# Critical-Infrastructure-Systems-Lab/ldsr

Hardware: NVIDIA B200
Metric: EM fits/sec (T~400, restarts x CV folds) (higher is better)
Workload: dtype f64

## Files before the change

### ldsr_b200/csrc/em_split_kernel.cuh

```cuda
#pragma once
#include "em_kernel.cuh"

namespace ldsr {

constexpr int SPLIT_NCH = 10;

template <int PQ> __host__ __device__ constexpr int split_nstat() { return 11 + 3 * PQ; }

__host__ __device__ constexpr bool split_w_in_smem(int pq) { return pq <= 4; }
__host__ __device__ inline size_t split_smem_bytes(int pq, int nw, int max_units, int max_uunits) {
    size_t b = 0;
    b += (size_t)max_units * 3 * 32 * 8;
    b += (size_t)2 * nw * 4 * 32 * 8;
    const bool pair = nw % 2 == 0 && nw * (11 + 3 * pq) > 2 * nw * SPLIT_NCH;
    const size_t ch = (size_t)2 * nw * SPLIT_NCH * 32 * 8, st = (size_t)(pair ? nw / 2 : nw) * (11 + 3 * pq) * 32 * 8;
    b += ch > st ? ch : st;
    b += ((size_t)max_units * 4 + 15) & ~size_t(15);
    b += 128;
    b += (size_t)8 * 32 * 8;
    if (split_w_in_smem(pq)) b += (size_t)max_uunits * pq * 32 * 8;
    if (theta_bd_in_smem(pq)) b += (size_t)2 * pq * 32 * 8;
    return b;
}

constexpr int UNIT_M = 1 << 30, UNIT_M1 = 1 << 29, UNIT_US = 1 << 28, UNIT_T0 = UNIT_US - 1;

template <class F> __host__ __device__ inline void split_window_units(int t0, int T, int mseg, int uw, F f) {
    const int end = T < t0 + uw ? T : t0 + uw;
    int t = t0;
    while (t < end) {
        if (t + mseg <= T - 1 && t + mseg <= end) {
            f(t, false);
            t += mseg;
        } else {
            f(t, true);
            t += 1;
        }
    }
}

inline int split_units_upper_bound(const double *y, int T, int mseg, int uw) {
    int n = 0;
    for (int t0 = 0; t0 < T; t0 += uw) {
        bool any = false;
        for (int t = t0; t < T && t < t0 + uw; t++) any = any || (y[t] == y[t]);
        const bool inside = t0 + uw <= T - 1;
        if (!any && inside)
            n += 1;
        else
            split_window_units(t0, T, mseg, uw, [&](int, bool) { n++; });
    }
    return n;
}

template <int N> __device__ __forceinline__ void load_vec(const double *__restrict__ p, double (&dst)[N]) {
    if constexpr (N % 2 == 0) {
        const double2 *__restrict__ p2 = reinterpret_cast<const double2 *>(p);
#pragma unroll
        for (int i = 0; i < N / 2; i++) {
            const double2 t = p2[i];
            dst[2 * i] = t.x;
            dst[2 * i + 1] = t.y;
        }
    } else {
#pragma unroll
        for (int i = 0; i < N; i++) dst[i] = p[i];
    }
}

__device__ __forceinline__ void rescale4(double &a, double &b, double &c, double &d) {
    const int e = ((__double2hiint(a + b + c + d) >> 20) & 0x7ff) - 1023;
    const double sc = __hiloint2double((1023 - e) << 20, 0);
    a *= sc;
    b *= sc;
    c *= sc;
    d *= sc;
}

template <int PQ, int UW> struct SplitConst {
    static_assert(UW == 16 || UW == 32, "U unit is 16 or 32 steps");
    double A, A2, Q;
    double A8, A16;
    double aVW, bVW;
    MixedConst<PQ> mc;
    __device__ __forceinline__ double AW() const { return UW == 32 ? A16 * A16 : A16; }
    __device__ __forceinline__ void set(const Theta<PQ> &th) {
        A = th.A;
        A2 = A * A;
        Q = th.Q;
        const double A4 = A2 * A2;
        A8 = A4 * A4;
        A16 = A8 * A8;
        const double aw = AW();
        aVW = aw * aw;
        const double sv = ((1.0 + A2) * (1.0 + A4)) * (1.0 + A8);
        double s = sv * (1.0 + A16);
        if (UW == 32) s *= 1.0 + A16 * A16;
        bVW = Q * s;
        mc.set(th, A2);
    }
};

template <int PQ, int UW, int N>
__device__ __forceinline__ void compose_var_unit(const Theta<PQ> &th, const SplitConst<PQ, UW> &k, unsigned bits,
                                                 double &m11, double &m12, double &m21, double &m22) {
#pragma unroll
    for (int j = 0; j < N; j++) {
        const bool obs = (bits >> j) & 1u;
        const double s11 = obs ? k.mc.a11 : k.A2, s12 = obs ? k.mc.a12 : k.Q;
        const double s21 = obs ? k.mc.C2 : 0.0, s22 = obs ? th.R : 1.0;
        const double n11 = fma(s11, m11, s12 * m21), n12 = fma(s11, m12, s12 * m22);
        const double n21 = fma(s21, m11, s22 * m21), n22 = fma(s21, m12, s22 * m22);
        m11 = n11;
        m12 = n12;
        m21 = n21;
        m22 = n22;
    }
    rescale4(m11, m12, m21, m22);
}

template <int N> struct UnitGains {
    double K[N], rS[N], alpha[N], J[N], L[N];
    double Vnext;
    double dend;
};
template <int PQ, int UW, int N>
__device__ __forceinline__ void unit_gains(const Theta<PQ> &th, const SplitConst<PQ, UW> &k, unsigned bits, double Vq,
                                           UnitGains<N> &G) {
    double nj[N], dj[N], nn[N], dd[N];
    double n = Vq, d = 1.0;
#pragma unroll
    for (int j = 0; j < N; j++) {
        const bool obs = (bits >> j) & 1u;
        const double m11 = obs ? k.mc.a11 : k.A2, m12 = obs ? k.mc.a12 : k.Q;
        const double m21 = obs ? k.mc.C2 : 0.0, m22 = obs ? th.R : 1.0;
        nj[j] = n;
        dj[j] = d;
        nn[j] = fma(m11, n, m12 * d);
        dd[j] = fma(m21, n, m22 * d);
        n = nn[j];
        d = dd[j];
    }
    double rho[N], rn[N];
#pragma unroll
    for (int j = 0; j < N; j++) {
        rho[j] = fast_rcp(dd[j]);
        rn[j] = fast_rcp(nn[j]);
    }
#pragma unroll
    for (int j = 0; j < N; j++) {
        const bool obs = (bits >> j) & 1u;
        const double K = obs ? th.C * nj[j] * rho[j] : 0.0;
        const double nu = obs ? th.R * nj[j] : nj[j];
        const double vu = nu * rho[j];
        const double J = k.A * nu * rn[j];
        G.K[j] = K;
        G.rS[j] = obs ? dj[j] * rho[j] : 0.0;
        G.alpha[j] = fma(-k.mc.AC, K, k.A);
        G.J[j] = J;
        G.L[j] = vu * fma(-k.A, J, 1.0);
    }
    G.Vnext = nn[N - 1] * rho[N - 1];
    G.dend = d;
}

template <int PQ, int N>
__device__ __forceinline__ void unit_inputs(const Theta<PQ> &th, unsigned bits, const double *__restrict__ yseg,
                                            const double *__restrict__ useg, const double *__restrict__ vseg,
                                            double (&Bu)[N], double (&ymd)[N], double (&yo)[N],
                                            double (&ur)[N * PQ], double (&vr)[N * PQ]) {
    double yr[N];
    load_vec<N * PQ>(useg, ur);
    load_vec<N * PQ>(vseg, vr);
    load_vec<N>(yseg, yr);
#pragma unroll
    for (int j = 0; j < N; j++) {
        double b = 0.0, dv = 0.0;
#pragma unroll
        for (int i = 0; i < PQ; i++) {
            b = fma(th.b(i), ur[j * PQ + i], b);
            dv = fma(th.d(i), vr[j * PQ + i], dv);
        }
        const bool obs = (bits >> j) & 1u;
        yo[j] = obs ? yr[j] : 0.0;
        Bu[j] = b;
        ymd[j] = yo[j] - dv;
    }
}

struct PieceFwd {
    double Vq, P, q;
    double l0, l1, l2;
    double dprod;
    int shift;
    double PJ, PJ2, G0, GG, Lc;
};

template <int PQ, int UW, int N>
__device__ __forceinline__ void forward_unit_basis(const Theta<PQ> &th, const SplitConst<PQ, UW> &k, unsigned bits,
                                                   const double *__restrict__ yseg, const double *__restrict__ useg,
                                                   const double *__restrict__ vseg, PieceFwd &c) {
    double Bu[N], ymd[N], yo[N];
    {
        double ur[N * PQ], vr[N * PQ];
        unit_inputs<PQ, N>(th, bits, yseg, useg, vseg, Bu, ymd, yo, ur, vr);
    }
    UnitGains<N> G;
    unit_gains<PQ, UW, N>(th, k, bits, c.Vq, G);
    double q[N + 1], P[N + 1];
    q[0] = c.q;
    P[0] = c.P;
#pragma unroll
    for (int j = 0; j < N; j++) {
        const double beta = fma(k.A * G.K[j], ymd[j], Bu[j]);
        q[j + 1] = fma(G.alpha[j], q[j], beta);
        P[j + 1] = G.alpha[j] * P[j];
    }
    double g0[N], gP[N];
#pragma unroll
    for (int j = 0; j < N; j++) {
        const double d0 = fma(-th.C, q[j], ymd[j]);
        const double w0 = G.rS[j] * d0;
        c.l0 = fma(w0, d0, c.l0);
        c.l1 = fma(w0, P[j], c.l1);
        c.l2 = fma(G.rS[j] * P[j], P[j], c.l2);
        const double xu0 = fma(G.K[j], d0, q[j]);
        const double xuP = P[j] * fma(-G.K[j], th.C, 1.0);
        g0[j] = fma(-G.J[j], q[j + 1], xu0);
        gP[j] = fma(-G.J[j], P[j + 1], xuP);
    }
    double pj = c.PJ, pj2 = c.PJ2;
#pragma unroll
    for (int j = 0; j < N; j++) {
        c.G0 = fma(pj, g0[j], c.G0);
        c.GG = fma(pj, gP[j], c.GG);
        c.Lc = fma(pj2, G.L[j], c.Lc);
        pj *= G.J[j];
        pj2 *= G.J[j] * G.J[j];
    }
    c.PJ = pj;
    c.PJ2 = pj2;
    c.q = q[N];
    c.P = P[N];
    c.Vq = G.Vnext;
    c.dprod *= G.dend;
    {
        const int e = ((__double2hiint(c.dprod) >> 20) & 0x7ff) - 1023;
        c.dprod *= __hiloint2double((1023 - e) << 20, 0);
        c.shift += e;
    }
}

template <int PQ, int UW>
__device__ __forceinline__ void forward_word_basis(const Theta<PQ> &th, const SplitConst<PQ, UW> &k,
                                                   const double *__restrict__ useg, double *__restrict__ wk,
                                                   PieceFwd &c) {
    constexpr bool KEEP_W = split_w_in_smem(PQ);
    const double A4 = k.A2 * k.A2;
    double hh = 0.0;
    double W[KEEP_W ? PQ : 1];
    if (KEEP_W) {
#pragma unroll
        for (int i = 0; i < PQ; i++) W[i] = 0.0;
    }
#pragma unroll 1
    for (int b = 0; b < UW / 8; b++) {
        double ur[8 * PQ];
        load_vec<8 * PQ>(useg + b * 8 * PQ, ur);
        if (KEEP_W) {
#pragma unroll
            for (int i = 0; i < PQ; i++) {
                double lo = ur[i], hi = ur[4 * PQ + i];
#pragma unroll
                for (int j = 1; j < 4; j++) {
                    lo = fma(k.A, lo, ur[j * PQ + i]);
                    hi = fma(k.A, hi, ur[(4 + j) * PQ + i]);
                }
                W[i] = fma(W[i], k.A8, fma(lo, A4, hi));
            }
        } else {
            double Bu[8];
#pragma unroll
            for (int j = 0; j < 8; j++) {
                double acc = 0.0;
#pragma unroll
                for (int i = 0; i < PQ; i++) acc = fma(th.b(i), ur[j * PQ + i], acc);
                Bu[j] = acc;
            }
            double lo = Bu[0], hi = Bu[4];
#pragma unroll
            for (int j = 1; j < 4; j++) {
                lo = fma(k.A, lo, Bu[j]);
                hi = fma(k.A, hi, Bu[4 + j]);
            }
            hh = fma(hh, k.A8, fma(lo, A4, hi));
        }
    }
    if (KEEP_W) {
#pragma unroll
        for (int i = 0; i < PQ; i++) {
            hh = fma(th.b(i), W[i], hh);
            wk[i * 32] = W[i];
        }
    }
    const double AW = k.AW();
    const double qn = fma(AW, c.q, hh);
    const double Pn = AW * c.P;
    const double Vn = fma(k.aVW, c.Vq, k.bVW);
    const double Jc = AW * c.Vq * fast_rcp(Vn);
    const double g0 = fma(-Jc, qn, c.q);
    const double gP = fma(-Jc, Pn, c.P);
    const double L = c.Vq * fma(-AW, Jc, 1.0);
    c.G0 = fma(c.PJ, g0, c.G0);
    c.GG = fma(c.PJ, gP, c.GG);
    c.Lc = fma(c.PJ2, L, c.Lc);
    c.PJ *= Jc;
    c.PJ2 *= Jc * Jc;
    c.q = qn;
    c.P = Pn;
    c.Vq = Vn;
}

template <int PQ, int UW, int N>
__device__ __forceinline__ void smooth_unit(const Theta<PQ> &th, const SplitConst<PQ, UW> &k, unsigned bits, bool last,
                                            const double *__restrict__ yseg, const double *__restrict__ useg,
                                            const double *__restrict__ vseg, double Xq, double Vq, double &Xs1,
                                            double &Vs1, Stats<PQ> &st) {
    constexpr bool KEEP_ROWS = N * PQ <= 16;
    double Bu[N], ymd[N], yo[N];
    double ur[N * PQ], vr[N * PQ];
    unit_inputs<PQ, N>(th, bits, yseg, useg, vseg, Bu, ymd, yo, ur, vr);
    UnitGains<N> G;
    unit_gains<PQ, UW, N>(th, k, bits, Vq, G);
    double xq[N + 1], g[N];
    xq[0] = Xq;
#pragma unroll
    for (int j = 0; j < N; j++) xq[j + 1] = fma(G.alpha[j], xq[j], fma(k.A * G.K[j], ymd[j], Bu[j]));
#pragma unroll
    for (int j = 0; j < N; j++) {
        const double delta = fma(-th.C, xq[j], ymd[j]);
        const double xu = fma(G.K[j], delta, xq[j]);
        g[j] = fma(-G.J[j], xq[j + 1], xu);
    }
    double Xs[N + 1], Vs[N + 1];
    Xs[N] = Xs1;
    Vs[N] = Vs1;
#pragma unroll
    for (int j = N - 1; j >= 0; j--) {
        Xs[j] = fma(G.J[j], Xs[j + 1], g[j]);
        Vs[j] = fma(G.J[j] * G.J[j], Vs[j + 1], G.L[j]);
    }
    if (!KEEP_ROWS) {
        load_vec<N * PQ>(useg, ur);
        load_vec<N * PQ>(vseg, vr);
    }
#pragma unroll
    for (int j = 0; j < N; j++) {
        if (N == 1 && last) {
            st.XT = Xs[j];
            st.VT = Vs[j];
        } else {
            st.Tx1x = fma(Xs[j + 1], Xs[j], st.Tx1x);
            st.Tx1xv = fma(Vs[j + 1], G.J[j], st.Tx1xv);
            st.Txx = fma(Xs[j], Xs[j], st.Txx);
            st.Txxv += Vs[j];
#pragma unroll
            for (int i = 0; i < PQ; i++) {
                st.Tx1u[i] = fma(Xs[j + 1], ur[j * PQ + i], st.Tx1u[i]);
                st.Tux[i] = fma(ur[j * PQ + i], Xs[j], st.Tux[i]);
            }
        }
        const bool obs = (bits >> j) & 1u;
        const double xo = obs ? Xs[j] : 0.0;
        st.Syx = fma(yo[j], xo, st.Syx);
        st.Sxx = fma(xo, xo, st.Sxx);
        st.Sxxv += obs ? Vs[j] : 0.0;
#pragma unroll
        for (int i = 0; i < PQ; i++) st.Sxv[i] = fma(xo, vr[j * PQ + i], st.Sxv[i]);
    }
    Xs1 = Xs[0];
    Vs1 = Vs[0];
}

template <int N> struct ShortConst {
    double AN, aV, bV;
    __device__ __forceinline__ ShortConst(double A, double A2, double Q) {
        double an = 1.0, av = 1.0, sv = 0.0;
#pragma unroll
        for (int j = 0; j < N; j++) {
            an *= A;
            sv = fma(sv, A2, 1.0);
            av *= A2;
        }
        AN = an;
        aV = av;
        bV = Q * sv;
    }
};
template <int PQ, int N>
__device__ __forceinline__ void forward_short_basis(const Theta<PQ> &th, double A, double A2, double Q,
                                                    const double *__restrict__ useg, PieceFwd &c) {
    const ShortConst<N> sc(A, A2, Q);
    double hh = 0.0;
#pragma unroll
    for (int j = 0; j < N; j++) {
        double bu = 0.0;
#pragma unroll
        for (int i = 0; i < PQ; i++) bu = fma(th.b(i), useg[j * PQ + i], bu);
        hh = fma(A, hh, bu);
    }
    const double qn = fma(sc.AN, c.q, hh), Pn = sc.AN * c.P, Vn = fma(sc.aV, c.Vq, sc.bV);
    const double Jc = sc.AN * c.Vq * fast_rcp(Vn);
    const double g0 = fma(-Jc, qn, c.q), gP = fma(-Jc, Pn, c.P), L = c.Vq * fma(-sc.AN, Jc, 1.0);
    c.G0 = fma(c.PJ, g0, c.G0);
    c.GG = fma(c.PJ, gP, c.GG);
    c.Lc = fma(c.PJ2, L, c.Lc);
    c.PJ *= Jc;
    c.PJ2 *= Jc * Jc;
    c.q = qn;
    c.P = Pn;
    c.Vq = Vn;
}
template <int PQ, int N>
__device__ __forceinline__ void smooth_short(const Theta<PQ> &th, double A, double A2, double Q,
                                             const double *__restrict__ useg, double Xq, double Vq, double &cG,
                                             double &cH, double &Xs1, double &Vs1, Stats<PQ> &st) {
    double Gs[N], Hs[N];
    Gs[N - 1] = Q * cG;
    Hs[N - 1] = cH;
#pragma unroll
    for (int j = N - 2; j >= 0; j--) {
        Gs[j] = A * Gs[j + 1];
        Hs[j] = A2 * Hs[j + 1];
    }
    const ShortConst<N> sc(A, A2, Q);
    const double G0 = sc.AN * cG, H0 = sc.aV * cH;
    double Xn[N + 1], vp[N + 1], Vn[N + 1];
    Xn[0] = fma(Vq, G0, Xq);
    vp[0] = Vq;
    Vn[0] = fma(Vq, Vq * H0, Vq);
    double tv = 0.0;
#pragma unroll
    for (int j = 0; j < N; j++) {
        double inp = Gs[j];
#pragma unroll
        for (int i = 0; i < PQ; i++) inp = fma(th.b(i), useg[j * PQ + i], inp);
        Xn[j + 1] = fma(A, Xn[j], inp);
        vp[j + 1] = fma(A2, vp[j], Q);
        const double t1 = vp[j + 1] * Hs[j];
        Vn[j + 1] = fma(vp[j + 1], t1, vp[j + 1]);
        st.Tx1x = fma(Xn[j + 1], Xn[j], st.Tx1x);
        st.Txx = fma(Xn[j], Xn[j], st.Txx);
        st.Txxv += Vn[j];
        tv = fma(vp[j], 1.0 + t1, tv);
#pragma unroll
        for (int i = 0; i < PQ; i++) {
            st.Tx1u[i] = fma(Xn[j + 1], useg[j * PQ + i], st.Tx1u[i]);
            st.Tux[i] = fma(useg[j * PQ + i], Xn[j], st.Tux[i]);
        }
    }
    st.Tx1xv = fma(A, tv, st.Tx1xv);
    Xs1 = Xn[0];
    Vs1 = Vn[0];
    cG = G0;
    cH = H0;
}

constexpr int SPLIT_NUV = 7;
template <int UW> __device__ __forceinline__ void uvar_constants(double a, double Q, double aW, double *o) {
    double sig = 0.0, b1 = 0.0, W = 0.0, Z = 0.0, pw = 1.0, pw_prev = 1.0;
#pragma unroll 4
    for (int s = 0; s < UW; s++) {
        const double sn = fma(a, sig, 1.0);
        b1 += sig;
        W = fma(a, W, sig * sig);
        Z = fma(a, Z, sig * sn);
        sig = sn;
        pw_prev = pw;
        pw *= a;
    }
    const double Q2 = Q * Q;
    o[0 * 32] = sig;
    o[1 * 32] = Q * b1;
    o[2 * 32] = aW * sig;
    o[3 * 32] = 2.0 * Q * aW * b1;
    o[4 * 32] = Q2 * (a * W);
    o[5 * 32] = Q * fma(pw_prev, b1 + sig, aW * b1);
    o[6 * 32] = Q2 * Z;
}

template <int PQ, int UW>
__device__ __forceinline__ void smooth_word(const Theta<PQ> &th, const SplitConst<PQ, UW> &k,
                                            const double *__restrict__ useg, const double *__restrict__ uv,
                                            const double *__restrict__ wk, const double *__restrict__ tuu_w,
                                            double Xq, double Vq, double &cG, double &cH, double &Xs1, double &Vs1,
                                            Stats<PQ> &st) {
    constexpr int NB = UW / 8;
    constexpr bool KEEP_W = split_w_in_smem(PQ);
    const double qg0 = k.Q * cG;
    const double g1 = k.A8 * qg0, g2 = k.A16 * qg0, g3 = k.A8 * g2;
    const double G0 = (NB == 4 ? k.A8 * k.A16 * k.A8 : k.A16) * cG;
    const double H0 = k.aVW * cH;
    const double Xfirst = fma(Vq, G0, Xq), Vfirst = fma(Vq, Vq * H0, Vq);
    {
        const double sumVp = fma(uv[0 * 32], Vq, uv[1 * 32]);
        const double qa = uv[2 * 32] * Vq;
        st.Txxv += fma(cH, fma(Vq, qa + uv[3 * 32], uv[4 * 32]), sumVp);
        st.Tx1xv = fma(k.A, fma(cH, fma(Vq, qa + uv[5 * 32], uv[6 * 32]), sumVp), st.Tx1xv);
    }
    double Xs = Xfirst;
    double tux[KEEP_W ? PQ : 1];
    if (KEEP_W) {
#pragma unroll
        for (int i = 0; i < PQ; i++) tux[i] = 0.0;
    }
#pragma unroll 1
    for (int b = 0; b < NB; b++) {
        const int r = NB - 1 - b;
        const double Gb = r == 0 ? qg0 : (r == 1 ? g1 : (r == 2 ? g2 : g3));
        const double *__restrict__ blk = useg + b * 8 * PQ;
        constexpr bool KEEP_U = PQ <= 4;
        double uk[8 * PQ];
        load_vec<8 * PQ>(blk, uk);
        double Gs[8];
        Gs[7] = Gb;
#pragma unroll
        for (int j = 6; j >= 0; j--) Gs[j] = k.A * Gs[j + 1];
        double inp[8];
#pragma unroll
        for (int j = 0; j < 8; j++) {
            double acc = Gs[j];
#pragma unroll
            for (int i = 0; i < PQ; i++) acc = fma(th.b(i), uk[j * PQ + i], acc);
            inp[j] = acc;
        }
        double Xn[9];
        Xn[0] = Xs;
#pragma unroll
        for (int j = 0; j < 8; j++) Xn[j + 1] = fma(k.A, Xn[j], inp[j]);
        if (!KEEP_U) load_vec<8 * PQ>(blk, uk);
#pragma unroll
        for (int j = 0; j < 8; j++) {
            st.Tx1x = fma(Xn[j + 1], Xn[j], st.Tx1x);
            st.Txx = fma(Xn[j], Xn[j], st.Txx);
#pragma unroll
            for (int i = 0; i < PQ; i++) {
                if (KEEP_W) {
                    tux[i] = fma(uk[j * PQ + i], Xn[j], tux[i]);
                } else {
                    st.Tx1u[i] = fma(Xn[j + 1], uk[j * PQ + i], st.Tx1u[i]);
                    st.Tux[i] = fma(uk[j * PQ + i], Xn[j], st.Tux[i]);
                }
            }
        }
        Xs = Xn[8];
    }
    if (KEEP_W) {
#pragma unroll
        for (int i = 0; i < PQ; i++) {
            double acc = fma(qg0, wk[i * 32], k.A * tux[i]);
#pragma unroll
            for (int j = 0; j < PQ; j++) acc = fma(th.b(j), tuu_w[j * PQ + i], acc);
            st.Tx1u[i] += acc;
            st.Tux[i] += tux[i];
        }
    }
    Xs1 = Xfirst;
    Vs1 = Vfirst;
    cG = G0;
    cH = H0;
}

template <int PQ> __device__ __forceinline__ void stats_store(const Stats<PQ> &st, double *o) {
    o[0 * 32] = st.Syx;
    o[1 * 32] = st.Sxx;
    o[2 * 32] = st.Sxxv;
    o[3 * 32] = st.Tx1x;
    o[4 * 32] = st.Tx1xv;
    o[5 * 32] = st.Txx;
    o[6 * 32] = st.Txxv;
    o[7 * 32] = st.X0;
    o[8 * 32] = st.V0;
    o[9 * 32] = st.XT;
    o[10 * 32] = st.VT;
#pragma unroll
    for (int i = 0; i < PQ; i++) {
        o[(11 + i) * 32] = st.Sxv[i];
        o[(11 + PQ + i) * 32] = st.Tx1u[i];
        o[(11 + 2 * PQ + i) * 32] = st.Tux[i];
    }
}
template <int PQ> __device__ __forceinline__ void stats_add(Stats<PQ> &st, const double *o) {
    st.Syx += o[0 * 32];
    st.Sxx += o[1 * 32];
    st.Sxxv += o[2 * 32];
    st.Tx1x += o[3 * 32];
    st.Tx1xv += o[4 * 32];
    st.Txx += o[5 * 32];
    st.Txxv += o[6 * 32];
    st.X0 += o[7 * 32];
    st.V0 += o[8 * 32];
    st.XT += o[9 * 32];
    st.VT += o[10 * 32];
#pragma unroll
    for (int i = 0; i < PQ; i++) {
        st.Sxv[i] += o[(11 + i) * 32];
        st.Tx1u[i] += o[(11 + PQ + i) * 32];
        st.Tux[i] += o[(11 + 2 * PQ + i) * 32];
    }
}
template <int PQ, int NW> __host__ __device__ constexpr bool split_pairwise() {
    return NW % 2 == 0 && NW * (11 + 3 * PQ) > 2 * NW * SPLIT_NCH;
}
template <int PQ, int NW> __host__ __device__ constexpr int split_st_slots() {
    return split_pairwise<PQ, NW>() ? NW / 2 : NW;
}

struct SplitParams {
    EmParams em;
    int max_units;
    int max_uunits;
    int blob_smem;
    int cost_u, cost_m;
    int *flags;
    int epoch;
    int *ctl;
    const int *order;
    int n_sm;
#ifdef LDSR_PHASE_CLOCKS
    long long *clk;
#endif
};
#ifdef LDSR_PHASE_CLOCKS
#define LDSR_PHASE_MARK(kk)                       \
    do {                                          \
        const long long c_ = clock64();           \
        pc[kk] += c_ - tprev;                     \
        tprev = c_;                               \
    } while (0)
#define LDSR_UNIT_BEGIN() const long long ub_ = clock64()
#define LDSR_UNIT_END(base, u0) pc[(base) + (((u0) & UNIT_M) ? 1 : ((u0) & UNIT_M1) ? 2 : ((u0) & UNIT_US) ? 3 : 0)] += clock64() - ub_
#else
#define LDSR_PHASE_MARK(kk) \
    do {                    \
    } while (0)
#define LDSR_UNIT_BEGIN() \
    do {                  \
    } while (0)
#define LDSR_UNIT_END(base, u0) \
    do {                        \
    } while (0)
#endif

__device__ __forceinline__ int unit_cost(int u, int cost_u, int cost_m, int mseg) {
    if (u & UNIT_US) return cost_m / 5;
    return (u & UNIT_M) ? cost_m : ((u & UNIT_M1) ? (3 * cost_m) / (2 * mseg) : cost_u);
}
template <int NW>
__device__ inline void split_range(const int *units, int a, int b, int cost_u, int cost_m, int mseg, int *bounds) {
    long long total = 0;
    for (int i = a; i < b; ++i) total += unit_cost(units[i], cost_u, cost_m, mseg);
    bounds[0] = a;
    long long acc = 0;
    int kq = a;
    for (int w = 1; w < NW; ++w) {
        const long long target = (total * w + NW / 2) / NW;
        while (kq < b) {
            const int cu = unit_cost(units[kq], cost_u, cost_m, mseg);
            if (acc + cu / 2 >= target) break;
            acc += cu;
            kq++;
        }
        bounds[w] = kq;
    }
    bounds[NW] = b;
}

template <int PQ, int NW, int MINB, int MSEG, int UW>
__global__ void __launch_bounds__(NW * 32, MINB) em_split_kernel(const SplitParams SP) {
    static_assert(MSEG == 4 || MSEG == 8, "M unit is 4 or 8 steps");
    const EmParams &P = SP.em;
    LDSR_DYN_SMEM(smem_raw);
    LDSR_STATIC_SMEM(__align__(8) uint64_t, bar);
    constexpr int NST = split_nstat<PQ>();
    constexpr int NP = 2 * NW;
    constexpr bool PAIR = split_pairwise<PQ, NW>();
    constexpr int ST_SLOTS = split_st_slots<PQ, NW>();
    constexpr size_t CH_DOUBLES = (size_t)NP * SPLIT_NCH * 32, ST_DOUBLES = (size_t)ST_SLOTS * NST * 32;

    const int lane = threadIdx.x & 31, warp = threadIdx.x >> 5;
    if (threadIdx.x == 0) {
        mbar_init(&bar, 1);
        fence_mbar_init();
    }
    __syncthreads();
    const int n_tasks = *P.n_tasks;
    unsigned phase = 0;
    int w_lo = 0;
    const auto slot_len = [&]() -> int {
        const int W = n_tasks * P.chunk, M = (W + (int)gridDim.x - 1) / (int)gridDim.x;
        return M < P.chunk ? P.chunk : M;
    };
    if (SP.flags) w_lo = (int)blockIdx.x * slot_len();
    const bool ranked = SP.ctl != nullptr && n_tasks <= (int)gridDim.x;
    LDSR_STATIC_SMEM(int, s_ti);
    LDSR_STATIC_SMEM(int, s_more);
    LDSR_STATIC_SMEM(int, s_on_sm);
    for (int seg = 0;; ++seg, phase ^= 1u) {
    int ti, n_it = P.chunk;
    bool wait_first = false;
    if (ranked) {
        if (seg > 0) break;
        if (threadIdx.x == 0) {
            const unsigned sm = sm_id(2);
            if (sm >= (unsigned)SHARE_MAX_SMID) share_trap();
            const int local = atomicAdd(SP.ctl + SHARE_CTL_SLOT + sm, 1);
            int r;
            if (local == 0) {
                r = atomicAdd(SP.ctl + SHARE_CTL_SMS, 1);
                flag_raise(SP.ctl + SHARE_CTL_RANK + sm, r + 1);
            } else {
                while ((r = ld_acquire(SP.ctl + SHARE_CTL_RANK + sm)) == 0) {
                }
                r -= 1;
            }
            if (local >= 2 || r >= SP.n_sm) share_trap();
            const int x = n_tasks > SP.n_sm ? n_tasks - SP.n_sm : 0;
            int qi = -1;
            if (local < 2 && r < SP.n_sm) qi = r < x ? 2 * r + local : (local == 0 ? x + r : -1);
            s_ti = (qi >= 0 && qi < n_tasks) ? SP.order[qi] : -1;
            s_on_sm = r < x ? 2 : 1;
            s_more = 1;
        }
        __syncthreads();
        ti = s_ti;
        if (ti < 0) break;
    } else if (SP.flags) {
        const int W = n_tasks * P.chunk, hi = ((int)blockIdx.x + 1) * slot_len(), w_hi = hi < W ? hi : W;
        if (w_lo >= w_hi) break;
        ti = w_lo / P.chunk;
        const int t_end = (ti + 1) * P.chunk, end = t_end < w_hi ? t_end : w_hi;
        n_it = end - w_lo;
        wait_first = w_lo == ti * P.chunk && end < t_end;
    } else {
        ti = (int)blockIdx.x + seg * (int)gridDim.x;
        if (ti >= n_tasks) break;
    }
    LDSR_CHECK(ti >= 0 && ti < n_tasks && n_it >= 1 && n_it <= P.chunk);
    if (seg > 0) __syncthreads();
    if (wait_first) {
        if (threadIdx.x == 0) flag_wait(SP.flags + ti, SP.epoch);
        __syncthreads();
    }
    const int4 task = P.tasks[ti];
    const SeriesDev S = P.series[task.x];
    const int T = S.T;
    if (threadIdx.x == 0) stage_blob(smem_raw, P.blobs + S.blob_off, (unsigned)S.blob_doubles * 8u, &bar);

    const double *__restrict__ ser = reinterpret_cast<const double *>(smem_raw);
    const double *__restrict__ ys = ser + S.y_off;
    const double *__restrict__ us = ser + S.u_off;
    const double *__restrict__ vs = ser + S.v_off;
    double *const ck = reinterpret_cast<double *>(smem_raw + SP.blob_smem) + lane;
    double *const MC = ck + (size_t)SP.max_units * 96;
    double *const CH = MC + (size_t)NP * 4 * 32;
    double *const ST = CH;
    int *const units =
        reinterpret_cast<int *>(CH - lane + (CH_DOUBLES > ST_DOUBLES ? CH_DOUBLES : ST_DOUBLES));
    int *const pbound = units + ((SP.max_units + 3) & ~3);
    double *const UV = reinterpret_cast<double *>(pbound + 32) + lane;
    double *const WK = UV + 8 * 32;
    double *const TB = WK + (split_w_in_smem(PQ) ? (size_t)SP.max_uunits * PQ * 32 : 0);
    double *const TD = TB + PQ * 32;
    constexpr bool BD_SMEM = theta_bd_in_smem(PQ);

    const bool valid = lane < task.z;
    const int fit = P.active[task.y + (valid ? lane : 0)];
    const int grp = P.f_group[fit];
    const unsigned *__restrict__ mw = P.masks + P.g_mask_off[grp];
    const double *__restrict__ gc = P.gconst + (size_t)grp * gconst_stride(PQ);
    const double *__restrict__ tuu_inv = P.sconst + S.sconst_off;
    const double n_obs = gc[1], inv_n_obs = 1.0 / n_obs;
    constexpr int TL = theta_pad_len<PQ>();
    Theta<PQ> th;
    {
        double g[TL];
#pragma unroll
        for (int i = 0; i < TL; i++) g[i] = ld_l2(P.theta + (size_t)fit * TL + i);
        load_theta<PQ>(th, g);
    }
    th.sb = TB;
    th.sd = TD;
    if (BD_SMEM && warp == 0) {
#pragma unroll
        for (int i = 0; i < PQ; i++) {
            TB[i * 32] = th.B[i];
            TD[i * 32] = th.D[i];
        }
    }
    double l1 = ld_l2(P.l1 + fit), l2 = ld_l2(P.l2 + fit), lik = ld_l2(P.lik + fit);
    int ne = ld_l2(P.ne + fit);
    bool live = valid && (ld_l2(P.done + fit) == 0);
    if (live && P.g_status[grp] != 0) {
        live = false;
        lik = __longlong_as_double(0x7ff8000000000000ULL);
    }

    if (warp == 0) {
        mbar_wait(&bar, phase);
        auto any_finite = [&](int t0, int n) -> bool {
            const int t = t0 + lane;
            const double yt = (lane < n && t < T) ? ys[t] : __longlong_as_double(0x7ff8000000000000ULL);
            return __any_sync(FULL, yt == yt);
        };
        int nu = 0;
        for (int t0 = 0; t0 < T; t0 += UW) {
            const bool any = any_finite(t0, UW);
            const bool inside = t0 + UW <= T - 1;
            if (!any && inside) {
                if (lane == 0) units[nu] = t0;
                nu++;
            } else {
                split_window_units(t0, T, MSEG, UW, [&](int t, bool single) {
                    int type = single ? UNIT_M1 : UNIT_M;
#ifndef LDSR_NO_US
                    if (!single && !any_finite(t, MSEG)) type = UNIT_US;
#endif
                    if (lane == 0) units[nu] = t | type;
                    nu++;
                });
            }
        }
        __syncwarp();
        if (lane == 0) {
            int nM = 0;
            for (int i = 0; i < nu; ++i) nM += (units[i] & (UNIT_M | UNIT_M1)) ? 1 : 0;
            int best = nu / 2, best_mis = 1 << 30, mb = 0;
            for (int s = 0; s <= nu; ++s) {
                const int ub = s - mb, ma = nM - mb, uaft = (nu - s) - ma;
                int mis = min(mb + uaft, ub + ma);
                if (s == 0 || s == nu) mis = 1 << 29;
                if (mis < best_mis || (mis == best_mis && abs(2 * s - nu) < abs(2 * best - nu))) {
                    best_mis = mis;
                    best = s;
                }
                if (s < nu && (units[s] & (UNIT_M | UNIT_M1))) mb++;
            }
            split_range<NW>(units, 0, best, SP.cost_u, SP.cost_m, MSEG, pbound);
            split_range<NW>(units, best, nu, SP.cost_u, SP.cost_m, MSEG, pbound + NW);
            LDSR_CHECK(nu <= SP.max_units && (T + UW - 1) / UW <= SP.max_uunits);
            for (int w = 0; w < 2 * NW; ++w) LDSR_CHECK(pbound[w] >= 0 && pbound[w] <= pbound[w + 1] && pbound[w + 1] <= nu);
        }
    }
    mbar_wait(&bar, phase);
    __syncthreads();

#ifdef LDSR_PHASE_CLOCKS
    long long pc[21] = {0, 0, 0, 0, 0, 0, 0, 0, 0, 0, 0, 0, 0, 0, 0, 0, 0, 0, 0, 0, 0}, tprev = clock64();
#endif
    bool counted = false;
    for (int it = 0;; ++it) {
        if (it >= n_it) {
            if (!ranked) break;
            if (!counted) {
                if (threadIdx.x == 0) {
                    atomicAdd(SP.ctl + SHARE_CTL_FINISHED, 1);
                    if (atomicAdd(SP.ctl + SHARE_CTL_DONE + sm_id(2), 1) + 1 < s_on_sm) s_more = 0;
                }
                counted = true;
                __syncthreads();
            }
            if (!s_more) break;
        }
        if (!__any_sync(FULL, live)) break;
        SplitConst<PQ, UW> k;
        k.set(th);

        if (warp == NW - 1) uvar_constants<UW>(k.A2, k.Q, k.aVW, UV);
        LDSR_PHASE_MARK(9);
#pragma unroll 1
        for (int h = 0; h < 2; ++h) {
            const int pj = h * NW + warp;
            if (pj == NP - 1) break;
            double m11 = 1.0, m12 = 0.0, m21 = 0.0, m22 = 1.0;
            const int ua = pbound[pj], ue = pbound[pj + 1];
            for (int un = ua; un < ue; ++un) {
                const int u0 = units[un];
                const int t0 = u0 & UNIT_T0;
                if (u0 & UNIT_M) {
                    compose_var_unit<PQ, UW, MSEG>(th, k, seg_bits(mw, t0, MSEG), m11, m12, m21, m22);
                } else if (u0 & UNIT_M1) {
                    compose_var_unit<PQ, UW, 1>(th, k, seg_bits(mw, t0, 1), m11, m12, m21, m22);
                } else if (u0 & UNIT_US) {
                    const ShortConst<MSEG> sc(k.A, k.A2, k.Q);
                    m11 = fma(sc.aV, m11, sc.bV * m21);
                    m12 = fma(sc.aV, m12, sc.bV * m22);
                } else {
                    m11 = fma(k.aVW, m11, k.bVW * m21);
                    m12 = fma(k.aVW, m12, k.bVW * m22);
                }
            }
            MC[(pj * 4 + 0) * 32] = m11;
            MC[(pj * 4 + 1) * 32] = m12;
            MC[(pj * 4 + 2) * 32] = m21;
            MC[(pj * 4 + 3) * 32] = m22;
        }
        LDSR_PHASE_MARK(0);
        __syncthreads();
        LDSR_PHASE_MARK(1);
        double VinA = th.V1, VinB = th.V1;
        {
            double n = th.V1, d = 1.0;
#pragma unroll
            for (int pj = 0; pj < NP - 1; ++pj) {
                const double m11 = MC[(pj * 4 + 0) * 32], m12 = MC[(pj * 4 + 1) * 32];
                const double m21 = MC[(pj * 4 + 2) * 32], m22 = MC[(pj * 4 + 3) * 32];
                const double nn = fma(m11, n, m12 * d), dd = fma(m21, n, m22 * d);
                n = nn;
                d = dd;
                if (pj + 1 == warp) VinA = n * fast_rcp(d);
                if (pj + 1 == NW + warp) VinB = n * fast_rcp(d);
            }
        }

        LDSR_PHASE_MARK(10);
#pragma unroll 1
        for (int h = 0; h < 2; ++h) {
            const int pj = h * NW + warp;
            const int ua = pbound[pj], ue = pbound[pj + 1];
            PieceFwd c;
            c.Vq = h ? VinB : VinA;
            c.P = 1.0;
            c.q = 0.0;
            c.l0 = c.l1 = c.l2 = 0.0;
            c.dprod = 1.0;
            c.shift = 0;
            c.PJ = c.PJ2 = 1.0;
            c.G0 = c.GG = c.Lc = 0.0;
            bool any_m = false;
            for (int un = ua; un < ue; ++un) {
                const int u0 = units[un];
                const int t0 = u0 & UNIT_T0;
                ck[(un * 3 + 0) * 32] = c.Vq;
                ck[(un * 3 + 1) * 32] = c.q;
                ck[(un * 3 + 2) * 32] = c.P;
                LDSR_UNIT_BEGIN();
                if (u0 & UNIT_M) {
                    any_m = true;
                    forward_unit_basis<PQ, UW, MSEG>(th, k, seg_bits(mw, t0, MSEG), ys + t0, us + t0 * PQ,
                                                     vs + t0 * PQ, c);
                } else if (u0 & UNIT_M1) {
                    any_m = true;
                    forward_unit_basis<PQ, UW, 1>(th, k, seg_bits(mw, t0, 1), ys + t0, us + t0 * PQ, vs + t0 * PQ, c);
                } else if (u0 & UNIT_US) {
                    forward_short_basis<PQ, MSEG>(th, k.A, k.A2, k.Q, us + t0 * PQ, c);
                } else {
                    forward_word_basis<PQ, UW>(th, k, us + t0 * PQ, WK + (size_t)(t0 / UW) * PQ * 32, c);
                }
                LDSR_UNIT_END(13, u0);
            }
            double ld = 0.0;
            if (any_m) ld = fma((double)c.shift, 0.693147180559945309417, log(c.dprod));
            double *o = CH + (size_t)pj * SPLIT_NCH * 32;
            o[0 * 32] = c.P;
            o[1 * 32] = c.q;
            o[2 * 32] = c.l0 + ld;
            o[3 * 32] = c.l1;
            o[4 * 32] = c.l2;
            o[5 * 32] = c.PJ;
            o[6 * 32] = c.G0;
            o[7 * 32] = c.GG;
            o[8 * 32] = c.Lc;
            o[9 * 32] = c.Vq;
        }
        LDSR_PHASE_MARK(2);
        __syncthreads();
        LDSR_PHASE_MARK(3);

        double gk[NP];
        double xinA = 0.0, xinB = 0.0;
        double XrA = 0.0, XrB = 0.0, VrA = 0.0, VrB = 0.0;
        double acc = 0.0;
        double x = th.mu1;
        double vend = th.V1;
        {
#pragma unroll
            for (int pj = 0; pj < NP; ++pj) {
                const double *o = CH + (size_t)pj * SPLIT_NCH * 32;
                if (pj == warp) xinA = x;
                if (pj == NW + warp) xinB = x;
                gk[pj] = fma(o[7 * 32], x, o[6 * 32]);
                const double tC = th.C * x;
                acc += fma(tC, fma(tC, o[4 * 32], -2.0 * o[3 * 32]), o[2 * 32]);
                x = fma(o[0 * 32], x, o[1 * 32]);
                vend = o[9 * 32];
                if (pj == warp) {
                    XrA = x;
                    VrA = vend;
                }
                if (pj == NW + warp) {
                    XrB = x;
                    VrB = vend;
                }
            }
        }
        const double lik_new = (-0.5 * n_obs * LOG_2PI - 0.5 * acc) * inv_n_obs;

        if (live) {
            lik = lik_new;
            ne += 1;
            if (warp == 0 && P.liks) P.liks[(size_t)P.f_user[fit] * P.niter + (ne - 1)] = lik_new;
            const bool conv = (ne >= 3) && (fabs(lik_new - l1) < P.tol) && (fabs(l1 - l2) < P.tol);
            if (conv || ne >= P.niter) live = false;
        }
        if (!__any_sync(FULL, live)) break;

        double Xs1A = 0.0, Vs1A = 0.0, Xs1B = 0.0, Vs1B = 0.0;
        {
            double Xs = x, Vs = vend;
#pragma unroll
            for (int pj = NP - 1; pj >= 0; --pj) {
                if (pj == NW + warp) {
                    Xs1B = Xs;
                    Vs1B = Vs;
                }
                if (pj == warp) {
                    Xs1A = Xs;
                    Vs1A = Vs;
                }
                const double *o = CH + (size_t)pj * SPLIT_NCH * 32;
                const double pjv = o[5 * 32];
                Xs = fma(pjv, Xs, gk[pj]);
                Vs = fma(pjv * pjv, Vs, o[8 * 32]);
            }
        }
        LDSR_PHASE_MARK(4);
        __syncthreads();
        LDSR_PHASE_MARK(5);

        Stats<PQ> st;
        st.zero();
#pragma unroll 1
        for (int h = 1; h >= 0; --h) {
            const int pj = h * NW + warp;
            const int ua = pbound[pj], ue = pbound[pj + 1];
            const double xin = h ? xinB : xinA;
            double Xs1 = h ? Xs1B : Xs1A, Vs1 = h ? Vs1B : Vs1A;
            double Xr = h ? XrB : XrA, Vr = h ? VrB : VrA;
            double cG = 0.0, cH = 0.0;
            bool in_run = false;
            for (int un = ue - 1; un >= ua; --un) {
                const int u0 = units[un];
                const int t0 = u0 & UNIT_T0;
                const double Vq = ck[(un * 3 + 0) * 32];
                const double Xq = fma(ck[(un * 3 + 2) * 32], xin, ck[(un * 3 + 1) * 32]);
                LDSR_UNIT_BEGIN();
                if (u0 & UNIT_M) {
                    smooth_unit<PQ, UW, MSEG>(th, k, seg_bits(mw, t0, MSEG), false, ys + t0, us + t0 * PQ,
                                              vs + t0 * PQ, Xq, Vq, Xs1, Vs1, st);
                    in_run = false;
                } else if (u0 & UNIT_M1) {
                    smooth_unit<PQ, UW, 1>(th, k, seg_bits(mw, t0, 1), t0 == T - 1, ys + t0, us + t0 * PQ,
                                           vs + t0 * PQ, Xq, Vq, Xs1, Vs1, st);
                    in_run = false;
                } else {
                    if (!in_run) {
                        const double rv = fast_rcp(Vr);
                        cG = (Xs1 - Xr) * rv;
                        cH = (Vs1 - Vr) * rv * rv;
                        in_run = true;
                    }
                    if (u0 & UNIT_US)
                        smooth_short<PQ, MSEG>(th, k.A, k.A2, k.Q, us + t0 * PQ, Xq, Vq, cG, cH, Xs1, Vs1, st);
                    else
                    smooth_word<PQ, UW>(th, k, us + t0 * PQ, UV, WK + (size_t)(t0 / UW) * PQ * 32,
                                        P.uwin + S.uwin_off + (size_t)(t0 / UW) * PQ * PQ, Xq, Vq, cG, cH, Xs1, Vs1, st);
                }
                LDSR_UNIT_END(17, u0);
                Xr = Xq;
                Vr = Vq;
            }
            if (ua == 0 && ue > 0) {
                st.X0 = Xs1;
                st.V0 = Vs1;
            }
        }
        LDSR_PHASE_MARK(6);
        if (ranked && it + 1 >= n_it && threadIdx.x == 0)
            s_more = ld_relaxed(SP.ctl + SHARE_CTL_FINISHED) + (counted ? 0 : 1) < n_tasks;
        if (!PAIR) {
            stats_store<PQ>(st, ST + (size_t)warp * NST * 32);
            __syncthreads();
            LDSR_PHASE_MARK(7);
            st.zero();
#pragma unroll
            for (int w = 0; w < NW; ++w) stats_add<PQ>(st, ST + (size_t)w * NST * 32);
        } else {
            if (warp >= NW / 2) stats_store<PQ>(st, ST + (size_t)(warp - NW / 2) * NST * 32);
            __syncthreads();
            if (warp < NW / 2) {
                stats_add<PQ>(st, ST + (size_t)warp * NST * 32);
                stats_store<PQ>(st, ST + (size_t)warp * NST * 32);
            }
            __syncthreads();
            if (warp == 0) {
                st.zero();
#pragma unroll
                for (int w = 0; w < NW / 2; ++w) stats_add<PQ>(st, ST + (size_t)w * NST * 32);
            }
        }
        LDSR_PHASE_MARK(11);
        if (!PAIR) {
            if (live) mstep_from_stats<PQ, true>(st, gc, tuu_inv, T, th);
        } else {
            double g[TL];
            if (warp == 0) {
                if (BD_SMEM) {
#pragma unroll
                    for (int i = 0; i < PQ; i++) {
                        th.B[i] = TB[i * 32];
                        th.D[i] = TD[i * 32];
                    }
                }
                if (live) mstep_from_stats<PQ, true>(st, gc, tuu_inv, T, th);
                if (BD_SMEM) {
#pragma unroll
                    for (int i = 0; i < PQ; i++) {
                        TB[i * 32] = th.B[i];
                        TD[i * 32] = th.D[i];
                    }
                }
                store_theta<PQ>(th, g);
#pragma unroll
                for (int i = 0; i < TL; i++) ST[i * 32] = g[i];
            }
            __syncthreads();
            if (warp != 0) {
#pragma unroll
                for (int i = 0; i < TL; i++) g[i] = ST[i * 32];
                load_theta<PQ>(th, g);
            }
        }
        if (live) {
            l2 = l1;
            l1 = lik;
        }
        LDSR_PHASE_MARK(8);
    }
#ifdef LDSR_PHASE_CLOCKS
    if (lane == 0 && SP.clk)
        for (int i = 0; i < 21; i++) SP.clk[((size_t)blockIdx.x * NW + warp) * 21 + i] = pc[i];
#endif

    if (ranked && !counted && threadIdx.x == 0) {
        atomicAdd(SP.ctl + SHARE_CTL_FINISHED, 1);
        atomicAdd(SP.ctl + SHARE_CTL_DONE + sm_id(2), 1);
    }
    if (BD_SMEM && warp == 0) {
#pragma unroll
        for (int i = 0; i < PQ; i++) {
            th.B[i] = TB[i * 32];
            th.D[i] = TD[i * 32];
        }
    }
    if (warp == 0 && valid) {
        store_theta<PQ>(th, P.theta + (size_t)fit * TL);
        P.l1[fit] = l1;
        P.l2[fit] = l2;
        P.lik[fit] = lik;
        P.ne[fit] = ne;
        P.done[fit] = live ? 0 : 1;
    }
    if (SP.flags) {
        if (w_lo % P.chunk != 0 && warp == 0) {
            __threadfence();
            __syncwarp();
            if (lane == 0) flag_raise(SP.flags + w_lo / P.chunk, SP.epoch);
        }
        w_lo += n_it;
    }
    }
}

}
```

### ldsr_b200/csrc/ldsr_abi.cu

```cuda
#include "../../include/ldsr_b200.h"
#include "generic_kernels.cuh"
#include "kernel_table.h"
#include "r_rng.cuh"
#include "scan_kernels.cuh"

#include <algorithm>
#include <atomic>
#include <chrono>
#include <condition_variable>
#include <cmath>
#include <cstdarg>
#include <cstdio>
#include <cstdlib>
#include <cstring>
#include <memory>
#include <mutex>
#include <numeric>
#include <string>
#include <thread>
#include <vector>

namespace ldsr {

#define LDSR_DECL(n) const KernelTable *kernel_table_pq##n() __attribute__((weak));
#define LDSR_PQ_LIST(X) X(1) X(2) X(3) X(4) X(5) X(6) X(7) X(8) X(10) X(12) X(16) X(24) X(32)
LDSR_PQ_LIST(LDSR_DECL)
const KernelTable *kernel_table_for(int need) {
#define LDSR_PICK(n) \
    if (need <= n && kernel_table_pq##n) return kernel_table_pq##n();
    LDSR_PQ_LIST(LDSR_PICK)
    return nullptr;
}

struct Err {
    int code = LDSR_OK;
    std::string msg;
    bool ok() const { return code == LDSR_OK; }
};
static Err fail(int code, const char *fmt, ...) {
    char buf[512];
    va_list ap;
    va_start(ap, fmt);
    vsnprintf(buf, sizeof buf, fmt, ap);
    va_end(ap);
    Err e;
    e.code = code;
    e.msg = buf;
    return e;
}
static int report(const Err &e, char *errbuf, int errlen) {
    if (errbuf && errlen > 0) snprintf(errbuf, errlen, "%s", e.msg.c_str());
    return e.code;
}
#define CU(call)                                                                                    \
    do {                                                                                            \
        cudaError_t _e = (call);                                                                    \
        if (_e != cudaSuccess) return fail(LDSR_ERR_CUDA, "%s: %s", #call, cudaGetErrorString(_e)); \
    } while (0)

class DevicePool {
  public:
    explicit DevicePool(int device) : device_(device) {}
    ~DevicePool() {
        cudaSetDevice(device_);
        for (auto &b : blocks_) cudaFree(b.ptr);
        for (auto &b : pinned_) cudaFreeHost(b.ptr);
        for (cudaStream_t s : streams_) cudaStreamDestroy(s);
    }
    cudaError_t alloc_pinned(size_t bytes, void **out) {
        bytes = std::max<size_t>((bytes + 255) & ~size_t(255), 256);
        std::lock_guard<std::mutex> lk(mu_);
        for (auto &b : pinned_)
            if (!b.used && b.size >= bytes) {
                b.used = true;
                *out = b.ptr;
                return cudaSuccess;
            }
        void *p = nullptr;
        cudaError_t e = cudaMallocHost(&p, bytes);
        if (e != cudaSuccess) return e;
        pinned_.push_back({p, bytes, true});
        *out = p;
        return cudaSuccess;
    }
    void release_pinned(void *p) {
        std::lock_guard<std::mutex> lk(mu_);
        for (auto &b : pinned_)
            if (b.ptr == p) b.used = false;
    }
    cudaError_t get_stream(cudaStream_t *out) {
        std::lock_guard<std::mutex> lk(mu_);
        if (!streams_.empty()) {
            *out = streams_.back();
            streams_.pop_back();
            return cudaSuccess;
        }
        return cudaStreamCreateWithFlags(out, cudaStreamNonBlocking);
    }
    void put_stream(cudaStream_t s) {
        std::lock_guard<std::mutex> lk(mu_);
        streams_.push_back(s);
    }
    cudaError_t alloc(size_t bytes, void **out) {
        bytes = std::max<size_t>((bytes + 255) & ~size_t(255), 256);
        std::lock_guard<std::mutex> lk(mu_);
        int best = -1;
        for (int i = 0; i < (int)blocks_.size(); i++)
            if (!blocks_[i].used && blocks_[i].size >= bytes && blocks_[i].size <= 2 * bytes + 4096 &&
                (best < 0 || blocks_[i].size < blocks_[best].size))
                best = i;
        if (best >= 0) {
            blocks_[best].used = true;
            *out = blocks_[best].ptr;
            return cudaSuccess;
        }
        void *p = nullptr;
        cudaError_t e = cudaMalloc(&p, bytes);
        if (e == cudaErrorMemoryAllocation) {
            cudaGetLastError();
            trim_locked();
            e = cudaMalloc(&p, bytes);
        }
        if (e != cudaSuccess) return e;
        blocks_.push_back({p, bytes, true});
        *out = p;
        return cudaSuccess;
    }
    void release(void *p) {
        std::lock_guard<std::mutex> lk(mu_);
        for (auto &b : blocks_)
            if (b.ptr == p) b.used = false;
    }
    size_t trim() {
        std::lock_guard<std::mutex> lk(mu_);
        return trim_locked();
    }
    size_t cached_bytes() {
        std::lock_guard<std::mutex> lk(mu_);
        size_t n = 0;
        for (auto &b : blocks_) n += b.size;
        return n;
    }
    int device() const { return device_; }

  private:
    struct Block {
        void *ptr;
        size_t size;
        bool used;
    };
    size_t trim_locked() {
        int prev = -1;
        cudaGetDevice(&prev);
        cudaSetDevice(device_);
        size_t freed = 0;
        auto drop = [&](std::vector<Block> &v, bool pinned) {
            size_t keep = 0;
            for (auto &b : v) {
                if (b.used) {
                    v[keep++] = b;
                    continue;
                }
                if (pinned)
                    cudaFreeHost(b.ptr);
                else {
                    cudaFree(b.ptr);
                    freed += b.size;
                }
            }
            v.resize(keep);
        };
        drop(blocks_, false);
        drop(pinned_, true);
        if (prev >= 0) cudaSetDevice(prev);
        return freed;
    }
    int device_;
    std::mutex mu_;
    std::vector<Block> blocks_, pinned_;
    std::vector<cudaStream_t> streams_;
};

}

using namespace ldsr;

struct ldsr_ctx {
    std::vector<int> devices;
    std::vector<std::unique_ptr<DevicePool>> pools;
};

constexpr int SCAN_MAX_FITS = 1500;
inline int scan_auto_fits(int pq) { return pq <= 4 ? 1200 : 900; }
constexpr size_t COUNTS_CAP = 256;
struct ldsr_plan {
    int device = 0;
    int n_sm = 148;
    DevicePool *pool = nullptr;
    std::unique_ptr<DevicePool> own_pool;
    cudaStream_t stream = nullptr;
    const KernelTable *kt = nullptr;
    int PQ = 0, TL = 0;
    int n_series = 0, n_groups = 0, n_fits = 0, theta_stride = 0;
    int max_T = 0, max_seg = 0;
    int max_units = 0;
    int wide_units = 0, wide_msteps = 0;
    size_t max_blob_bytes = 0;
    bool blob_in_smem = true;
    int last_niter = 0;
    std::vector<SeriesDev> h_series;
    std::vector<int> g_user, f_user, h_g_series, h_g_fit_ptr, h_f_group;
    std::vector<int> s_p, s_q, s_T;
    std::vector<int> user_fit_series;
    std::vector<long long> h_traj_ptr_user;
    long long traj_total = 0;
    std::vector<void *> allocs;
    SeriesDev *d_series = nullptr;
    double *d_blobs = nullptr, *d_sconst = nullptr, *d_gconst = nullptr, *d_uwin = nullptr;
    int *d_g_series = nullptr, *d_g_status = nullptr, *d_g_nobs = nullptr, *d_g_fit_ptr = nullptr;
    int *d_held_ptr = nullptr, *d_held_idx = nullptr;
    unsigned *d_masks = nullptr;
    long long *d_g_mask_off = nullptr;
    int *d_f_group = nullptr, *d_f_user = nullptr;
    double *d_theta0 = nullptr, *d_theta = nullptr, *d_l1 = nullptr, *d_l2 = nullptr, *d_lik = nullptr;
    int *d_ne = nullptr, *d_done = nullptr, *d_status = nullptr;
    double *d_liks = nullptr;
    size_t liks_cap = 0;
    int *d_active = nullptr, *d_task_off = nullptr, *d_n_live = nullptr, *d_counts = nullptr;
    size_t counts_cap = COUNTS_CAP;
    int4 *d_tasks = nullptr;
    int max_tasks = 0;
    unsigned long long *d_sum = nullptr;
    unsigned *d_ticket = nullptr;
    int *d_share_flags = nullptr;
    int *d_share_ctl = nullptr, *d_share_order = nullptr, *d_share_key = nullptr;
    int share_epoch = 0;
    double *d_ckpt = nullptr;
    size_t ckpt_cap = 0;
    int *d_best = nullptr;
    double *d_X = nullptr, *d_Y = nullptr, *d_V = nullptr, *d_J = nullptr;
    double *d_res = nullptr, *h_res = nullptr;
    size_t res_head = 0, res_total = 0;
    int *d_g_user = nullptr;
    bool same_width = true;
    int *d_job_group = nullptr, *d_job_theta = nullptr;
    long long *d_job_row = nullptr;
    int *h_counts = nullptr;
    bool em_done = false;

    template <class T> Err dalloc(T **out, size_t n) {
        void *p = nullptr;
        cudaError_t e = pool->alloc(std::max<size_t>(n, 1) * sizeof(T), &p);
        if (e != cudaSuccess) return fail(LDSR_ERR_CUDA, "device allocation of %zu bytes failed: %s", n * sizeof(T),
                                          cudaGetErrorString(e));
        allocs.push_back(p);
        *out = static_cast<T *>(p);
        return Err();
    }
    template <class T> Err drealloc(T **ptr, size_t n) {
        if (*ptr) {
            allocs.erase(std::remove(allocs.begin(), allocs.end(), static_cast<void *>(*ptr)), allocs.end());
            pool->release(*ptr);
            *ptr = nullptr;
        }
        return dalloc(ptr, n);
    }
    template <class T> Err upload(T **out, const std::vector<T> &h) {
        Err e = dalloc(out, h.size());
        if (!e.ok()) return e;
        if (!h.empty()) CU(cudaMemcpyAsync(*out, h.data(), h.size() * sizeof(T), cudaMemcpyHostToDevice, stream));
        return Err();
    }
    ~ldsr_plan() {
        cudaSetDevice(device);
        if (stream) cudaStreamSynchronize(stream);
        for (void *p : allocs) pool->release(p);
        if (h_counts) pool->release_pinned(h_counts);
        if (h_res) pool->release_pinned(h_res);
        if (stream) pool->put_stream(stream);
    }
};

namespace ldsr {

static void pad_theta(const double *src, int p, int q, bool has_u, bool has_v, int PQ, double *dst) {
    std::fill(dst, dst + 2 * PQ + 6, 0.0);
    dst[0] = src[0];
    if (has_u)
        for (int j = 0; j < p; j++) dst[1 + j] = src[1 + j];
    dst[1 + PQ] = src[1 + p];
    if (has_v)
        for (int j = 0; j < q; j++) dst[2 + PQ + j] = src[2 + p + j];
    for (int k = 0; k < 4; k++) dst[2 + 2 * PQ + k] = src[2 + p + q + k];
}
static void unpad_theta(const double *src, int p, int q, bool has_u, bool has_v, int PQ, double *dst) {
    dst[0] = src[0];
    for (int j = 0; j < p; j++) dst[1 + j] = has_u ? src[1 + j] : 0.0;
    dst[1 + p] = src[1 + PQ];
    for (int j = 0; j < q; j++) dst[2 + p + j] = has_v ? src[2 + PQ + j] : 0.0;
    for (int k = 0; k < 4; k++) dst[2 + p + q + k] = src[2 + 2 * PQ + k];
}

static Err validate(const ldsr_batch *b) {
    if (!b) return fail(LDSR_ERR_ARG, "batch is NULL");
    if (b->n_series < 1 || b->n_groups < 1 || b->n_fits < 1)
        return fail(LDSR_ERR_ARG, "n_series, n_groups and n_fits must all be >= 1");
    if (!b->T || !b->p || !b->q || !b->y || !b->group_series || !b->fit_group || !b->theta0)
        return fail(LDSR_ERR_ARG, "a required table pointer is NULL");
    for (int s = 0; s < b->n_series; s++) {
        if (b->T[s] < 2) return fail(LDSR_ERR_ARG, "series %d: T=%d, need T >= 2", s, b->T[s]);
        if (b->p[s] < 0 || b->q[s] < 0) return fail(LDSR_ERR_ARG, "series %d: negative p or q", s);
        if (b->p[s] > LDSR_MAX_PQ || b->q[s] > LDSR_MAX_PQ)
            return fail(LDSR_ERR_UNSUPPORTED, "series %d: p=%d q=%d exceeds LDSR_MAX_PQ=%d", s, b->p[s], b->q[s],
                        LDSR_MAX_PQ);
        if (!b->y[s]) return fail(LDSR_ERR_ARG, "series %d: y is NULL", s);
        if (b->u && b->u[s] && b->p[s] < 1) return fail(LDSR_ERR_ARG, "series %d: u given but p=0", s);
        if (b->v && b->v[s] && b->q[s] < 1) return fail(LDSR_ERR_ARG, "series %d: v given but q=0", s);
        if (b->theta_stride < b->p[s] + b->q[s] + 6)
            return fail(LDSR_ERR_ARG, "theta_stride=%d < p+q+6=%d (series %d)", b->theta_stride,
                        b->p[s] + b->q[s] + 6, s);
        for (int t = 0; t < b->T[s]; t++)
            if (std::isinf(b->y[s][t])) return fail(LDSR_ERR_ARG, "series %d: y[%d] is +-Inf", s, t);
    }
    for (int g = 0; g < b->n_groups; g++) {
        const int s = b->group_series[g];
        if (s < 0 || s >= b->n_series) return fail(LDSR_ERR_ARG, "group %d: series id %d out of range", g, s);
        if (b->held_ptr) {
            if (b->held_ptr[g + 1] < b->held_ptr[g]) return fail(LDSR_ERR_ARG, "held_ptr not monotone at group %d", g);
            for (int k = b->held_ptr[g]; k < b->held_ptr[g + 1]; k++)
                if (b->held_idx[k] < 0 || b->held_idx[k] >= b->T[s])
                    return fail(LDSR_ERR_ARG, "group %d: held-out step %d outside 0..%d", g, b->held_idx[k],
                                b->T[s] - 1);
        }
    }
    for (int f = 0; f < b->n_fits; f++) {
        const int g = b->fit_group[f];
        if (g < 0 || g >= b->n_groups) return fail(LDSR_ERR_ARG, "fit %d: group id %d out of range", f, g);
        if (f > 0 && g < b->fit_group[f - 1])
            return fail(LDSR_ERR_ARG, "fit_group must be non-decreasing (fit %d)", f);
    }
    return Err();
}

static Err plan_build(const ldsr_batch *b, int device, DevicePool *pool, ldsr_plan **out) {
    Err e = validate(b);
    if (!e.ok()) return e;
    int ndev = 0;
    if (cudaGetDeviceCount(&ndev) != cudaSuccess || ndev < 1)
        return fail(LDSR_ERR_CUDA, "no CUDA device available (this library has no CPU path)");
    if (device < 0 || device >= ndev) return fail(LDSR_ERR_ARG, "device %d out of range (have %d)", device, ndev);
    CU(cudaSetDevice(device));

    std::unique_ptr<ldsr_plan> P(new ldsr_plan());
    P->device = device;
    if (pool)
        P->pool = pool;
    else {
        P->own_pool.reset(new DevicePool(device));
        P->pool = P->own_pool.get();
    }
    CU(P->pool->get_stream(&P->stream));
    {
        void *hp = nullptr;
        CU(P->pool->alloc_pinned(COUNTS_CAP * sizeof(int), &hp));
        P->h_counts = static_cast<int *>(hp);
    }
    CU(cudaDeviceGetAttribute(&P->n_sm, cudaDevAttrMultiProcessorCount, device));

    const int ns = b->n_series, ng = b->n_groups, nf = b->n_fits;
    P->n_series = ns;
    P->n_groups = ng;
    P->n_fits = nf;
    P->theta_stride = b->theta_stride;
    int need = 1;
    for (int s = 0; s < ns; s++) {
        const bool hu = b->u && b->u[s], hv = b->v && b->v[s];
        if (hu) need = std::max(need, b->p[s]);
        if (hv) need = std::max(need, b->q[s]);
    }
    P->kt = kernel_table_for(need);
    if (!P->kt) return fail(LDSR_ERR_UNSUPPORTED, "input width %d has no kernel instantiation", need);
    const int PQ = P->PQ = P->kt->pq;
    P->TL = 2 * PQ + 6;
    P->s_p.assign(b->p, b->p + ns);
    P->s_q.assign(b->q, b->q + ns);
    P->s_T.assign(b->T, b->T + ns);

    std::vector<int> fit_lo(ng, -1), fit_hi(ng, -1);
    for (int f = 0; f < nf; f++) {
        const int g = b->fit_group[f];
        if (fit_lo[g] < 0) fit_lo[g] = f;
        fit_hi[g] = f + 1;
    }
    P->g_user.resize(ng);
    std::iota(P->g_user.begin(), P->g_user.end(), 0);
    std::stable_sort(P->g_user.begin(), P->g_user.end(),
                     [&](int a, int c) { return b->group_series[a] < b->group_series[c]; });
    P->h_g_series.resize(ng);
    P->h_g_fit_ptr.assign(ng + 1, 0);
    P->f_user.clear();
    P->h_f_group.clear();
    for (int gi = 0; gi < ng; gi++) {
        const int gu = P->g_user[gi];
        P->h_g_series[gi] = b->group_series[gu];
        P->h_g_fit_ptr[gi] = (int)P->f_user.size();
        if (fit_lo[gu] >= 0)
            for (int f = fit_lo[gu]; f < fit_hi[gu]; f++) {
                P->f_user.push_back(f);
                P->h_f_group.push_back(gi);
            }
    }
    P->h_g_fit_ptr[ng] = (int)P->f_user.size();

    P->h_series.resize(ns);
    std::vector<double> blobs, uwin;
    long long sconst_off = 0;
    for (int s = 0; s < ns; s++) {
        SeriesDev &S = P->h_series[s];
        std::memset(&S, 0, sizeof S);
        const int T = b->T[s], p = b->p[s], q = b->q[s];
        const double *u = b->u ? b->u[s] : nullptr, *v = b->v ? b->v[s] : nullptr;
        S.T = T;
        S.p = p;
        S.q = q;
        S.has_u = u != nullptr;
        S.has_v = v != nullptr;
        S.same_uv = (u && v && p == q && (u == v || std::memcmp(u, v, sizeof(double) * (size_t)p * T) == 0)) ||
                    (!u && !v);
        const int Ty = (T + 1) & ~1;
        const int nuv = T * PQ;
        S.y_off = 0;
        S.u_off = Ty;
        S.v_off = S.same_uv ? S.u_off : ((S.u_off + nuv + 1) & ~1);
        S.blob_doubles = ((S.v_off + nuv) + 1) & ~1;
        S.blob_off = (long long)blobs.size();
        S.sconst_off = sconst_off;
        sconst_off += PQ * PQ + 1;
        blobs.resize(blobs.size() + S.blob_doubles, 0.0);
        double *B = blobs.data() + S.blob_off;
        for (int t = 0; t < T; t++) {
            B[t] = b->y[s][t];
            if (u)
                for (int j = 0; j < p; j++) B[S.u_off + (size_t)t * PQ + j] = u[(size_t)t * p + j];
            if (v && !S.same_uv)
                for (int j = 0; j < q; j++) B[S.v_off + (size_t)t * PQ + j] = v[(size_t)t * q + j];
        }
        P->max_T = std::max(P->max_T, T);
        P->max_units = std::max(P->max_units, split_units_upper_bound(b->y[s], T, P->kt->split_mseg, P->kt->split_uw));
        if (P->kt->wide_nw > 0) {
            int nu = 0, nm = 0;
            wide_count_units(b->y[s], T, P->kt->wide_mseg, P->kt->split_uw, &nu, &nm);
            P->wide_units = std::max(P->wide_units, nu);
            P->wide_msteps = std::max(P->wide_msteps, nm);
        }
        {
            const int UWn = P->kt->split_uw, nwin = (T + UWn - 1) / UWn;
            S.uwin_off = (int)uwin.size();
            uwin.resize(uwin.size() + (size_t)nwin * PQ * PQ, 0.0);
            if (u)
                for (int t = 0; t < T; t++) {
                    double *G = uwin.data() + S.uwin_off + (size_t)(t / UWn) * PQ * PQ;
                    for (int a = 0; a < p; a++)
                        for (int c = 0; c < p; c++) G[a * PQ + c] += u[(size_t)t * p + a] * u[(size_t)t * p + c];
                }
        }
        P->max_blob_bytes = std::max(P->max_blob_bytes, (size_t)S.blob_doubles * 8);
    }
    {
        int f = 0;
        for (int s = 0; s < ns; s++) {
            P->h_series[s].fit_begin = f;
            while (f < (int)P->h_f_group.size() && P->h_g_series[P->h_f_group[f]] == s) f++;
            P->h_series[s].fit_end = f;
        }
    }
    P->max_seg = (P->max_T + EM_SEG - 1) / EM_SEG;
    P->blob_in_smem = P->max_blob_bytes <= 200 * 1024;

    std::vector<long long> mask_off(ng);
    long long nwords = 0;
    std::vector<int> held_ptr(ng + 1, 0), held_idx;
    for (int gi = 0; gi < ng; gi++) {
        const int gu = P->g_user[gi];
        mask_off[gi] = nwords;
        nwords += (b->T[P->h_g_series[gi]] + 31) / 32;
        if (b->held_ptr)
            for (int k = b->held_ptr[gu]; k < b->held_ptr[gu + 1]; k++) held_idx.push_back(b->held_idx[k]);
        held_ptr[gi + 1] = (int)held_idx.size();
    }
    P->h_traj_ptr_user.resize(ng + 1);
    P->h_traj_ptr_user[0] = 0;
    for (int g = 0; g < ng; g++) P->h_traj_ptr_user[g + 1] = P->h_traj_ptr_user[g] + b->T[b->group_series[g]];
    P->traj_total = P->h_traj_ptr_user[ng];

    std::vector<double> th0((size_t)nf * P->TL);
    for (int fi = 0; fi < nf; fi++) {
        const int s = P->h_g_series[P->h_f_group[fi]];
        pad_theta(b->theta0 + (size_t)P->f_user[fi] * b->theta_stride, b->p[s], b->q[s], P->h_series[s].has_u != 0,
                  P->h_series[s].has_v != 0, PQ, &th0[(size_t)fi * P->TL]);
    }

    if (!(e = P->upload(&P->d_series, P->h_series)).ok()) return e;
    if (!(e = P->upload(&P->d_blobs, blobs)).ok()) return e;
    if (uwin.empty()) uwin.push_back(0.0);
    if (!(e = P->upload(&P->d_uwin, uwin)).ok()) return e;
    if (!(e = P->upload(&P->d_g_series, P->h_g_series)).ok()) return e;
    if (!(e = P->upload(&P->d_g_fit_ptr, P->h_g_fit_ptr)).ok()) return e;
    if (!(e = P->upload(&P->d_g_mask_off, mask_off)).ok()) return e;
    if (!(e = P->upload(&P->d_held_ptr, held_ptr)).ok()) return e;
    if (held_idx.empty()) held_idx.push_back(0);
    if (!(e = P->upload(&P->d_held_idx, held_idx)).ok()) return e;
    if (!(e = P->upload(&P->d_f_group, P->h_f_group)).ok()) return e;
    if (!(e = P->upload(&P->d_f_user, P->f_user)).ok()) return e;
    if (!(e = P->upload(&P->d_g_user, P->g_user)).ok()) return e;
    for (int s = 0; s < ns; s++) P->same_width = P->same_width && b->p[s] + b->q[s] + 6 == b->theta_stride;
    if (!P->same_width) {
        P->user_fit_series.resize(nf);
        for (int f = 0; f < nf; f++) P->user_fit_series[f] = b->group_series[b->fit_group[f]];
    }
    P->res_head = (size_t)nf * b->theta_stride + nf + ((size_t)2 * nf + ng + 1) / 2;
    P->res_total = P->res_head + 4 * (size_t)P->traj_total;
    if (!(e = P->upload(&P->d_theta0, th0)).ok()) return e;
    if (!(e = P->dalloc(&P->d_masks, (size_t)nwords)).ok()) return e;
    if (!(e = P->dalloc(&P->d_sconst, (size_t)sconst_off)).ok()) return e;
    if (!(e = P->dalloc(&P->d_gconst, (size_t)ng * gconst_stride(PQ))).ok()) return e;
    if (!(e = P->dalloc(&P->d_g_status, ng)).ok()) return e;
    if (!(e = P->dalloc(&P->d_g_nobs, ng)).ok()) return e;
    if (!(e = P->dalloc(&P->d_theta, (size_t)nf * P->TL)).ok()) return e;
    if (!(e = P->dalloc(&P->d_l1, nf)).ok()) return e;
    if (!(e = P->dalloc(&P->d_l2, nf)).ok()) return e;
    if (!(e = P->dalloc(&P->d_lik, nf)).ok()) return e;
    if (!(e = P->dalloc(&P->d_ne, nf)).ok()) return e;
    if (!(e = P->dalloc(&P->d_done, nf)).ok()) return e;
    if (!(e = P->dalloc(&P->d_status, nf)).ok()) return e;
    if (!(e = P->dalloc(&P->d_active, nf)).ok()) return e;
    if (!(e = P->dalloc(&P->d_n_live, ns)).ok()) return e;
    if (!(e = P->dalloc(&P->d_task_off, ns + 1)).ok()) return e;
    if (!(e = P->dalloc(&P->d_counts, COUNTS_CAP)).ok()) return e;
    if (!(e = P->dalloc(&P->d_sum, 1)).ok()) return e;
    if (!(e = P->dalloc(&P->d_ticket, 1)).ok()) return e;
    CU(cudaMemsetAsync(P->d_ticket, 0, sizeof(unsigned), P->stream));
    P->max_tasks = std::max(nf / 32, std::min(nf, SCAN_MAX_FITS)) + ns + 1;
    if (!(e = P->dalloc(&P->d_tasks, P->max_tasks)).ok()) return e;
    if (!(e = P->dalloc(&P->d_share_flags, P->max_tasks)).ok()) return e;
    CU(cudaMemsetAsync(P->d_share_flags, 0, (size_t)P->max_tasks * sizeof(int), P->stream));
    if (!(e = P->dalloc(&P->d_share_ctl, SHARE_CTL_LEN)).ok()) return e;
    if (!(e = P->dalloc(&P->d_share_order, P->max_tasks)).ok()) return e;
    if (!(e = P->dalloc(&P->d_share_key, P->max_tasks)).ok()) return e;
    if (!(e = P->dalloc(&P->d_best, ng)).ok()) return e;

    SetupParams sp;
    sp.series = P->d_series;
    sp.blobs = P->d_blobs;
    sp.n_series = ns;
    sp.n_groups = ng;
    sp.g_series = P->d_g_series;
    sp.held_ptr = P->d_held_ptr;
    sp.held_idx = P->d_held_idx;
    sp.masks = P->d_masks;
    sp.g_mask_off = P->d_g_mask_off;
    sp.gconst = P->d_gconst;
    sp.sconst = P->d_sconst;
    sp.g_status = P->d_g_status;
    sp.g_nobs = P->d_g_nobs;
    sp.pq = PQ;
    const size_t sh = (size_t)(2 * PQ * PQ + 2 * PQ + 4) * sizeof(double);
    setup_kernel<<<ng + ns, 128, sh, P->stream>>>(sp);
    CU(cudaGetLastError());
    merge_status_kernel<<<(ng + 127) / 128, 128, 0, P->stream>>>(P->d_series, P->d_sconst, P->d_g_series, ng, PQ,
                                                                 P->d_g_status);
    CU(cudaGetLastError());
    *out = P.release();
    return Err();
}

#ifdef LDSR_PHASE_CLOCKS
static long long *sp_clk_last = nullptr;
#endif
static Err plan_em(ldsr_plan *P, int niter, double tol, const ldsr_options *opt, cudaStream_t st, bool want_liks,
                   std::atomic<int> *abort_flag, long long *stats) {
    if (niter < 2) return fail(LDSR_ERR_ARG, "niter=%d: the reference requires niter >= 2 (EM.cpp:247,256)", niter);
    if (!(tol == tol)) return fail(LDSR_ERR_ARG, "tol is NaN");
    CU(cudaSetDevice(P->device));
    if (!st) st = P->stream;
    if (st != P->stream) {
        cudaEvent_t ready = nullptr;
        CU(cudaEventCreateWithFlags(&ready, cudaEventDisableTiming));
        cudaError_t e1 = cudaEventRecord(ready, P->stream);
        if (e1 == cudaSuccess) e1 = cudaStreamWaitEvent(st, ready, 0);
        cudaEventDestroy(ready);
        CU(e1);
    }
    const int nf = P->n_fits, ns = P->n_series, ng = P->n_groups;
    int chunk = (opt && opt->chunk_iters > 0) ? opt->chunk_iters : 100;
    long long launches = 0, chunks = 0;
    double em_ms = 0.0;
    P->last_niter = niter;
    P->em_done = false;

    if (want_liks) {
        const size_t need = (size_t)nf * niter;
        if (P->liks_cap < need) {
            P->liks_cap = 0;
            Err e = P->drealloc(&P->d_liks, need);
            if (!e.ok()) return e;
            P->liks_cap = need;
        }
        fill_nan_kernel<<<(unsigned)((need + 255) / 256), 256, 0, st>>>(P->d_liks, need);
        launches++;
    }
    {
        const int n = nf * P->TL;
        init_state_kernel<<<(n + 255) / 256, 256, 0, st>>>(nf, P->TL, P->d_theta0, P->d_theta, P->d_l1, P->d_l2,
                                                           P->d_lik, P->d_ne, P->d_done);
        CU(cudaGetLastError());
        launches++;
    }
    const size_t blob_sm = (P->max_blob_bytes + 127) & ~size_t(127);
    const size_t ck_sm = (size_t)EM_WARPS * P->max_seg * 64 * sizeof(double);
    int mode = 0;
    size_t smem = 0;
    if (P->blob_in_smem) {
        mode = 1;
        smem = blob_sm;
        if (blob_sm + ck_sm <= 220 * 1024 && !(opt && opt->variant == 1)) {
            mode = 2;
            smem = blob_sm + ck_sm;
        }
    }
    const bool no_scan = opt && opt->variant == 6;
    const int variant = (opt && !no_scan) ? opt->variant : 0;
    const int max_uunits = (P->max_T + P->kt->split_uw - 1) / P->kt->split_uw;
    const size_t split_sm = blob_sm + split_smem_bytes(P->PQ, P->kt->split_nw, P->max_units, max_uunits);
    const size_t wide_blob_sm = wide_blob_smem(P->max_blob_bytes, P->max_T);
    const size_t wide_sm = P->kt->wide_nw > 0
                               ? wide_blob_sm + wide_smem_bytes(P->PQ, P->kt->wide_nw, P->max_T, P->wide_units, P->wide_msteps)
                               : ~size_t(0);
    const bool use_wide = P->kt->wide_nw > 0 && P->blob_in_smem && wide_sm <= 227 * 1024 && (variant == 0 || variant == 4);
    if (variant == 4 && !use_wide)
        return fail(LDSR_ERR_UNSUPPORTED, "variant 4 (wide-input kernel) needs width >= 5 and %zu bytes of shared memory",
                    wide_sm);
    int scan_steps = P->PQ <= 4 ? 4 : 2;
    if (const char *ev = std::getenv("LDSR_SCAN_L"))
        if (std::atoi(ev) == 2 && P->max_T <= 2 * 32 * SCAN_MAX_WARPS) scan_steps = 2;
    bool scan_uv_ok = true;
    if (P->PQ >= SCAN_SHARE_UV_FROM)
        for (const SeriesDev &S : P->h_series) scan_uv_ok = scan_uv_ok && S.same_uv != 0 && S.has_u != 0;
    const bool scan_ok = P->kt->scan_l > 0 && scan_uv_ok && P->max_T <= scan_steps * 32 * SCAN_MAX_WARPS;
    const bool use_scan = scan_ok && !no_scan &&
                          ((variant == 0 && nf <= scan_auto_fits(P->PQ)) || (variant == 5 && nf <= SCAN_MAX_FITS));
    if (variant == 5 && !use_scan)
        return fail(LDSR_ERR_UNSUPPORTED,
                    "variant 5 (scan kernel) needs input width <= %d, T <= %d (%d and v == u for width > 4) and at most %d fits",
                    SCAN_MAX_PQ, 32 * SCAN_L * SCAN_MAX_WARPS, 32 * 2 * SCAN_MAX_WARPS, SCAN_MAX_FITS);
    bool use_split = !use_scan && !use_wide && P->blob_in_smem && split_sm <= 227 * 1024 && (variant == 0 || variant == 3);
    if (variant == 3 && !use_split)
        return fail(LDSR_ERR_UNSUPPORTED, "variant 3 (time-split kernel) needs %zu bytes of shared memory", split_sm);
    if (use_scan) {
        smem = 0;
    } else if (use_wide) {
        smem = wide_sm;
        CU(P->kt->em_wide_prepare(smem));
    } else if (use_split) {
        smem = split_sm;
        CU(P->kt->em_split_prepare(smem));
    } else {
        CU(P->kt->em_prepare(std::max<size_t>(smem, 1024)));
    }
    const int fits_per_cta = use_scan ? 1 : ((use_split || use_wide) ? 32 : 32 * EM_WARPS);

    EmParams ep;
    ep.series = P->d_series;
    ep.blobs = P->d_blobs;
    ep.sconst = P->d_sconst;
    ep.uwin = P->d_uwin;
    ep.g_series = P->d_g_series;
    ep.masks = P->d_masks;
    ep.g_mask_off = P->d_g_mask_off;
    ep.gconst = P->d_gconst;
    ep.g_status = P->d_g_status;
    ep.f_group = P->d_f_group;
    ep.theta = P->d_theta;
    ep.l1 = P->d_l1;
    ep.l2 = P->d_l2;
    ep.lik = P->d_lik;
    ep.ne = P->d_ne;
    ep.done = P->d_done;
    ep.liks = want_liks ? P->d_liks : nullptr;
    ep.f_user = P->d_f_user;
    ep.active = P->d_active;
    ep.tasks = P->d_tasks;
    ep.max_seg = P->max_seg;
    ep.niter = niter;
    if (use_scan && !(opt && opt->chunk_iters > 0) && !(opt && opt->poll) && abort_flag == nullptr) chunk = niter;
    ep.chunk = chunk;
    ep.tol = tol;
    ep.mode = mode;
    ep.ckpt_smem_off = (int)blob_sm;
    ep.ckpt = nullptr;

    const int max_chunks = (niter + chunk - 1) / chunk;
    const bool sync_each = (opt && opt->poll) || abort_flag != nullptr;
    int grid0 = 0;
    for (int s = 0; s < ns; s++)
        grid0 += (P->h_series[s].fit_end - P->h_series[s].fit_begin + fits_per_cta - 1) / fits_per_cta;
    int share_slots = 0;
    bool share_ranked = false;
    if (use_split && P->kt->em_split_resident) {
        static const bool no_share = std::getenv("LDSR_NO_SHARE") != nullptr;
        int coop = 0, dev = 0;
        CU(cudaGetDevice(&dev));
        CU(cudaDeviceGetAttribute(&coop, cudaDevAttrCooperativeLaunch, dev));
        const int slots = P->kt->em_split_resident(smem) * P->n_sm;
        if (!no_share && !std::getenv("LDSR_MAX_GRID") && coop && slots > 0 && grid0 > P->n_sm && grid0 <= 4 * slots &&
            (long long)(grid0 + 1) * chunk < (1ll << 31))
            share_slots = slots;
        static const bool no_rank = std::getenv("LDSR_NO_RANK") != nullptr;
        share_ranked = share_slots == 2 * P->n_sm && share_slots <= 1024 && !no_rank;
    }
    if ((int)P->counts_cap < 2 * max_chunks) {
        Err e = P->drealloc(&P->d_counts, (size_t)2 * max_chunks);
        if (!e.ok()) return e;
        P->counts_cap = 2 * max_chunks;
        if (P->h_counts) P->pool->release_pinned(P->h_counts);
        P->h_counts = nullptr;
        void *hp = nullptr;
        CU(P->pool->alloc_pinned((size_t)2 * max_chunks * sizeof(int), &hp));
        P->h_counts = static_cast<int *>(hp);
    }
    const size_t ck_need = (mode == 2 || use_split || use_wide || use_scan) ? 0 : (size_t)grid0 * EM_WARPS * P->max_seg * 64;
    if (P->ckpt_cap < ck_need) {
        P->ckpt_cap = 0;
        Err e = P->drealloc(&P->d_ckpt, ck_need);
        if (!e.ok()) return e;
        P->ckpt_cap = ck_need;
    }
    ep.ckpt = P->d_ckpt;
    std::vector<cudaEvent_t> evs;
    struct EvVecGuard {
        std::vector<cudaEvent_t> &v;
        ~EvVecGuard() {
            for (cudaEvent_t e : v) cudaEventDestroy(e);
        }
    } evs_guard{evs};
    int enq = 0;
    for (int c = 0; c < max_chunks; ++c) {
        int *cnt = P->d_counts + 2 * c;
        compact_kernel<<<ns, 1024, 0, st>>>(P->d_series, ns, P->d_done, P->d_active, P->d_n_live, fits_per_cta,
                                            P->d_tasks, P->d_task_off, cnt, P->d_ticket, P->d_ne,
                                            share_ranked ? P->d_share_ctl : nullptr, P->d_share_order, P->d_share_key);
        launches++;
        int grid = (c == 0 || grid0 > 3 * P->n_sm) ? grid0 : std::min(grid0, 2 * P->n_sm);
        if (use_wide || use_scan) grid = grid0;
        int plain_grid = grid;
        if (share_slots > 0) grid = share_slots;
        static const int grid_cap = std::getenv("LDSR_MAX_GRID") ? std::atoi(std::getenv("LDSR_MAX_GRID")) : 0;
        if (grid_cap > 0) grid = std::min(grid, grid_cap);
        if (sync_each) {
            CU(cudaMemcpyAsync(P->h_counts + 2 * c, cnt, 2 * sizeof(int), cudaMemcpyDeviceToHost, st));
            CU(cudaStreamSynchronize(st));
            grid = plain_grid = std::max(1, P->h_counts[2 * c]);
            if (share_slots > 0) grid = share_ranked ? share_slots : std::min(grid, share_slots);
            if (P->h_counts[2 * c + 1] == 0) break;
            if (abort_flag) {
                if (abort_flag->load()) return fail(LDSR_ERR_INTERRUPTED, "interrupted");
            } else if (opt->poll(opt->poll_arg)) {
                return fail(LDSR_ERR_INTERRUPTED, "interrupted by the poll callback");
            }
        }
        ep.n_tasks = cnt;
        if (stats) {
            cudaEvent_t a = nullptr, b = nullptr;
            CU(cudaEventCreate(&a));
            evs.push_back(a);
            CU(cudaEventCreate(&b));
            evs.push_back(b);
            CU(cudaEventRecord(a, st));
        }
        if (use_scan) {
            ep.max_seg = P->max_T;
            ep.mode = nf > 2 * P->n_sm ? 1 : 0;
            CU(P->kt->em_scan(ep, grid, scan_steps, st));
        } else if (use_wide) {
            WideParams wp;
            wp.em = ep;
            wp.max_units = P->wide_units;
            wp.max_msteps = P->wide_msteps;
            wp.max_T = P->max_T;
            wp.blob_smem = (int)wide_blob_sm;
            wp.cost_u = P->kt->split_uw * 17 / 2;
            wp.cost_m = P->kt->wide_mseg * 90;
            if (const char *ev = std::getenv("LDSR_WIDE_COST_M")) wp.cost_m = std::atoi(ev);
#ifdef LDSR_PHASE_CLOCKS
            if (!sp_clk_last) cudaMalloc(&sp_clk_last, sizeof(long long) * 4096 * 21 * 8);
            wp.clk = (c == 1 && grid <= 2048) ? sp_clk_last : nullptr;
#endif
            CU(P->kt->em_wide(wp, grid, smem, st));
#ifdef LDSR_PHASE_CLOCKS
            if (c == 1 && grid <= 2048) {
                const int nw = P->kt->wide_nw;
                std::vector<long long> h((size_t)grid * nw * 21);
                cudaStreamSynchronize(st);
                cudaMemcpy(h.data(), sp_clk_last, h.size() * sizeof(long long), cudaMemcpyDeviceToHost);
                static const char *names[21] = {"P1", "B1 wait", "prefix+P2", "B2 wait", "P4", "B3 wait", "-",
                                                "B4 wait", "store sums", "B5 wait", "totals", "B5b wait", "matvec rows",
                                                "B5c wait", "M-step scalars", "B6 wait", "phase A", "chain+stop", "phase C", "-", "-"};
                std::fprintf(stderr, "[ldsr] wide kernel, phase clocks of launch 1 (cycles per iteration, mean over %d CTAs), per warp:\n", grid);
                for (int i = 0; i < 19; i++) {
                    std::fprintf(stderr, "[ldsr]   %-14s", names[i]);
                    for (int w = 0; w < nw; w++) {
                        double sum = 0;
                        for (int b = 0; b < grid; b++) sum += (double)h[((size_t)b * nw + w) * 21 + i];
                        std::fprintf(stderr, " %8.0f", sum / grid / chunk);
                    }
                    std::fprintf(stderr, "\n");
                }
            }
#endif
        } else if (use_split) {
            SplitParams sp;
            sp.em = ep;
            sp.max_units = P->max_units;
            sp.max_uunits = max_uunits;
            sp.blob_smem = (int)blob_sm;
            sp.cost_u = P->kt->split_uw * 22;
            sp.cost_m = P->kt->split_mseg * 168;
#ifdef LDSR_PHASE_CLOCKS
            if (!sp_clk_last) cudaMalloc(&sp_clk_last, sizeof(long long) * 4096 * 21 * 8);
            sp.clk = (c == 1 && grid <= 4096) ? sp_clk_last : nullptr;
#endif
            sp.flags = share_slots > 0 ? P->d_share_flags : nullptr;
            sp.epoch = ++P->share_epoch;
            sp.ctl = share_ranked ? P->d_share_ctl : nullptr;
            sp.order = P->d_share_order;
            sp.n_sm = P->n_sm;
            cudaError_t le = (grid <= 2 * P->n_sm || sp.flags) ? P->kt->em_split_wide(sp, grid, smem, st)
                                                               : P->kt->em_split(sp, grid, smem, st);
            if (le == cudaErrorCooperativeLaunchTooLarge && sp.flags) {
                cudaGetLastError();
                share_slots = 0;
                share_ranked = false;
                sp.flags = nullptr;
                sp.ctl = nullptr;
                grid = plain_grid;
                le = grid <= 2 * P->n_sm ? P->kt->em_split_wide(sp, grid, smem, st) : P->kt->em_split(sp, grid, smem, st);
            }
            CU(le);
        } else {
            CU(P->kt->em_chunk(ep, grid, smem, st));
        }
        if (stats) CU(cudaEventRecord(evs.back(), st));
#ifdef LDSR_PHASE_CLOCKS
        if (use_split && c == 1 && grid <= 4096) {
            const int nw = P->kt->split_nw;
            std::vector<long long> h((size_t)grid * nw * 21);
            cudaStreamSynchronize(st);
            cudaMemcpy(h.data(), sp_clk_last, h.size() * sizeof(long long), cudaMemcpyDeviceToHost);
            static const char *names[21] = {"P1 loops", "B1 wait", "P2", "B2 wait", "chain+stop", "B2' wait",
                                            "P4", "B3 wait", "M-step", "constants", "prefix", "reduce",
                                            "-", "P2 U words", "P2 M units", "P2 M1 units",
                                            "P2 US units", "P4 U words", "P4 M units", "P4 M1 units", "P4 US units"};
            std::fprintf(stderr, "[ldsr] phase clocks of launch 1 (cycles per iteration, mean over %d CTAs), per warp:\n", grid);
            for (int i = 0; i < 21; i++) {
                std::fprintf(stderr, "[ldsr]   %-14s", names[i]);
                for (int w = 0; w < nw; w++) {
                    double sum = 0;
                    for (int b = 0; b < grid; b++) sum += (double)h[((size_t)b * nw + w) * 21 + i];
                    std::fprintf(stderr, " %9.0f", sum / grid / chunk);
                }
                std::fprintf(stderr, "\n");
            }
        }
#endif
        launches++;
        enq++;
    }
    if (!sync_each) {
        CU(cudaMemcpyAsync(P->h_counts, P->d_counts, (size_t)2 * max_chunks * sizeof(int), cudaMemcpyDeviceToHost, st));
        CU(cudaStreamSynchronize(st));
        if (abort_flag && abort_flag->load()) return fail(LDSR_ERR_INTERRUPTED, "interrupted");
    } else {
        CU(cudaStreamSynchronize(st));
    }
    static const bool trace_chunks = std::getenv("LDSR_TIMING") != nullptr;
    for (int c = 0; c < enq; ++c) {
        if (P->h_counts[2 * c + 1] > 0) chunks++;
        if (stats) {
            float ms = 0.f;
            CU(cudaEventElapsedTime(&ms, evs[2 * c], evs[2 * c + 1]));
            if (P->h_counts[2 * c + 1] > 0) em_ms += ms;
            if (trace_chunks)
                std::fprintf(stderr, "[ldsr] chunk %d: %d tasks, %d live fits, %.3f ms\n", c, P->h_counts[2 * c],
                             P->h_counts[2 * c + 1], ms);
        }
    }
    cudaEvent_t tail_a = nullptr, tail_b = nullptr;
    if (trace_chunks && stats) {
        cudaEventCreate(&tail_a);
        cudaEventCreate(&tail_b);
        cudaEventRecord(tail_a, st);
    }
    select_kernel<<<(ng + 3) / 4, 128, 0, st>>>(ng, P->d_g_fit_ptr, P->d_theta, P->TL, 1 + P->PQ, P->d_lik,
                                                    P->d_g_status, P->d_best, P->d_status);
    CU(cudaGetLastError());
    launches++;
    if (!P->d_X) {
        Err e;
        if (!(e = P->dalloc(&P->d_res, P->res_total)).ok()) return e;
        P->d_X = P->d_res + P->res_head;
        P->d_Y = P->d_X + P->traj_total;
        P->d_V = P->d_Y + P->traj_total;
        P->d_J = P->d_V + P->traj_total;
        std::vector<int> jg(ng);
        std::vector<long long> jr(ng);
        for (int gi = 0; gi < ng; gi++) {
            jg[gi] = gi;
            jr[gi] = P->h_traj_ptr_user[P->g_user[gi]];
        }
        cudaStream_t keep = P->stream;
        P->stream = st;
        if (!(e = P->upload(&P->d_job_group, jg)).ok()) return e;
        if (!(e = P->upload(&P->d_job_row, jr)).ok()) return e;
        P->stream = keep;
    }
    SmootherParams sp;
    sp.series = P->d_series;
    sp.blobs = P->d_blobs;
    sp.g_series = P->d_g_series;
    sp.masks = P->d_masks;
    sp.g_mask_off = P->d_g_mask_off;
    sp.g_nobs = P->d_g_nobs;
    sp.n_jobs = ng;
    sp.job_group = P->d_job_group;
    sp.job_theta = P->d_best;
    sp.job_row = P->d_job_row;
    sp.theta = P->d_theta;
    sp.X = P->d_X;
    sp.Y = P->d_Y;
    sp.V = P->d_V;
    sp.J = P->d_J;
    sp.lik = nullptr;
    sp.stdlik = 1;
    sp.aux = nullptr;
    static const bool seq_traj = std::getenv("LDSR_SEQ_TRAJ") != nullptr;
    if (scan_ok && !seq_traj) {
        EmParams tp = ep;
        tp.max_seg = P->max_T;
        tp.n_jobs = ng;
        tp.job_group = sp.job_group;
        tp.job_theta = sp.job_theta;
        tp.job_row = sp.job_row;
        tp.tX = sp.X;
        tp.tY = sp.Y;
        tp.tV = sp.V;
        tp.tJ = sp.J;
        CU(P->kt->em_scan_traj(tp, scan_steps, st));
    } else {
        CU(P->kt->smoother(sp, st));
    }
    launches++;
    if (tail_a) cudaEventRecord(tail_b, st);
    CU(cudaMemsetAsync(P->d_sum, 0, sizeof(unsigned long long), st));
    sum_int_kernel<<<64, 256, 0, st>>>(P->d_ne, nf, P->d_sum);
    launches++;
    unsigned long long total = 0;
    CU(cudaMemcpyAsync(&total, P->d_sum, sizeof total, cudaMemcpyDeviceToHost, st));
    CU(cudaStreamSynchronize(st));
    CU(cudaGetLastError());
    P->em_done = true;
    if (tail_a) {
        float ms = 0.f, all = 0.f;
        cudaEventElapsedTime(&ms, tail_a, tail_b);
        if (!evs.empty()) cudaEventElapsedTime(&all, evs.front(), tail_b);
        std::fprintf(stderr, "[ldsr] selection + winners' smoother %.3f ms; first chunk start -> end %.3f ms\n", ms, all);
        cudaEventDestroy(tail_a);
        cudaEventDestroy(tail_b);
    }
    if (stats) {
        stats[0] = launches;
        stats[1] = chunks;
        stats[2] = (long long)total;
        stats[3] = (long long)(em_ms * 1e6);
        stats[4] = use_scan ? 3 : (use_wide ? 2 : (use_split ? 1 : 0));
        stats[5] = share_slots;
        stats[6] = stats[7] = 0;
    }
    return Err();
}

struct FetchMap {
    const int *fits, *groups;
    const long long *traj_ptr;
    int niter;
};

static Err plan_fetch(ldsr_plan *P, ldsr_em_result *out, const FetchMap *map = nullptr) {
    if (!P->em_done) return fail(LDSR_ERR_ARG, "ldsr_plan_fetch before a successful ldsr_plan_em");
    if (!out) return fail(LDSR_ERR_ARG, "result struct is NULL");
    CU(cudaSetDevice(P->device));
    const int nf = P->n_fits, ng = P->n_groups, stride = P->theta_stride;
    cudaStream_t st = P->stream;
    double *d_theta_u = P->d_res, *d_lik_u = d_theta_u + (size_t)nf * stride;
    int *d_int = reinterpret_cast<int *>(d_lik_u + nf);
    PackParams pk;
    pk.n_fits = nf;
    pk.n_groups = ng;
    pk.theta_len = P->TL;
    pk.pq = P->PQ;
    pk.stride = stride;
    pk.series = P->d_series;
    pk.g_series = P->d_g_series;
    pk.f_group = P->d_f_group;
    pk.f_user = P->d_f_user;
    pk.g_user = P->d_g_user;
    pk.theta = P->d_theta;
    pk.lik = P->d_lik;
    pk.iters = P->d_ne;
    pk.status = P->d_status;
    pk.best = P->d_best;
    pk.theta_u = d_theta_u;
    pk.lik_u = d_lik_u;
    pk.iters_u = d_int;
    pk.status_u = d_int + nf;
    pk.best_u = d_int + 2 * (size_t)nf;
    pack_results_kernel<<<(std::max(nf, ng) + 255) / 256, 256, 0, st>>>(pk);
    CU(cudaGetLastError());
    if (!P->h_res) {
        void *hp = nullptr;
        CU(P->pool->alloc_pinned(P->res_total * sizeof(double), &hp));
        P->h_res = static_cast<double *>(hp);
    }
    const bool traj = out->X || out->Y || out->V || out->J;
    CU(cudaMemcpyAsync(P->h_res, P->d_res, (traj ? P->res_total : P->res_head) * sizeof(double),
                       cudaMemcpyDeviceToHost, st));
    std::vector<double> liks_tmp;
    if (out->liks) {
        if (!P->d_liks) return fail(LDSR_ERR_ARG, "liks requested at fetch but not at ldsr_plan_em time");
        double *dst = out->liks;
        if (map) {
            liks_tmp.resize((size_t)nf * P->last_niter);
            dst = liks_tmp.data();
        }
        CU(cudaMemcpyAsync(dst, P->d_liks, (size_t)nf * P->last_niter * sizeof(double), cudaMemcpyDeviceToHost, st));
    }
    CU(cudaStreamSynchronize(st));
    const double *h_theta = P->h_res, *h_lik = h_theta + (size_t)nf * stride;
    const int *h_int = reinterpret_cast<const int *>(h_lik + nf);
    if (map) {
        const int *h_it = h_int, *h_st = h_int + nf, *h_best = h_int + 2 * (size_t)nf;
        for (int i = 0; i < nf; i++) {
            const int f = map->fits[i];
            if (out->theta) {
                int w = stride;
                if (!P->same_width) {
                    const int s = P->user_fit_series[i];
                    w = P->s_p[s] + P->s_q[s] + 6;
                }
                std::memcpy(out->theta + (size_t)f * stride, h_theta + (size_t)i * stride, sizeof(double) * w);
            }
            if (out->lik) out->lik[f] = h_lik[i];
            if (out->iters) out->iters[f] = h_it[i];
            if (out->status) out->status[f] = h_st[i];
            if (out->liks)
                std::memcpy(out->liks + (size_t)f * map->niter, &liks_tmp[(size_t)i * P->last_niter],
                            sizeof(double) * P->last_niter);
        }
        const size_t tt = (size_t)P->traj_total;
        const double *h_traj = P->h_res + P->res_head;
        for (int gl = 0; gl < ng; gl++) {
            const int g = map->groups[gl];
            if (out->best) out->best[g] = h_best[gl] < 0 ? -1 : map->fits[h_best[gl]];
            const size_t n = (size_t)(P->h_traj_ptr_user[gl + 1] - P->h_traj_ptr_user[gl]) * sizeof(double);
            const size_t src = (size_t)P->h_traj_ptr_user[gl], dst = (size_t)map->traj_ptr[g];
            if (out->X) std::memcpy(out->X + dst, h_traj + src, n);
            if (out->Y) std::memcpy(out->Y + dst, h_traj + tt + src, n);
            if (out->V) std::memcpy(out->V + dst, h_traj + 2 * tt + src, n);
            if (out->J) std::memcpy(out->J + dst, h_traj + 3 * tt + src, n);
        }
        return Err();
    }
    if (out->theta) {
        if (P->same_width)
            std::memcpy(out->theta, h_theta, sizeof(double) * (size_t)nf * stride);
        else
            for (int fi = 0; fi < nf; fi++) {
                const int s = P->h_g_series[P->h_f_group[fi]];
                const size_t row = (size_t)P->f_user[fi] * stride;
                std::memcpy(out->theta + row, h_theta + row, sizeof(double) * (P->s_p[s] + P->s_q[s] + 6));
            }
    }
    if (out->lik) std::memcpy(out->lik, h_lik, sizeof(double) * nf);
    if (out->iters) std::memcpy(out->iters, h_int, sizeof(int) * nf);
    if (out->status) std::memcpy(out->status, h_int + nf, sizeof(int) * nf);
    if (out->best) std::memcpy(out->best, h_int + 2 * (size_t)nf, sizeof(int) * ng);
    const size_t tt = (size_t)P->traj_total, tb = tt * sizeof(double);
    const double *h_traj = P->h_res + P->res_head;
    if (out->X) std::memcpy(out->X, h_traj, tb);
    if (out->Y) std::memcpy(out->Y, h_traj + tt, tb);
    if (out->V) std::memcpy(out->V, h_traj + 2 * tt, tb);
    if (out->J) std::memcpy(out->J, h_traj + 3 * tt, tb);
    return Err();
}

struct SubBatch {
    ldsr_batch b;
    std::vector<int> groups;
    std::vector<int> group_series, held_ptr, held_idx, fit_group, fits;
    std::vector<double> theta0;
    std::vector<long long> traj_ptr;
};

static void make_sub(const ldsr_batch *b, const std::vector<int> &groups, const std::vector<int> &fit_lo,
                     const std::vector<int> &fit_hi, SubBatch &sb) {
    sb.groups = groups;
    sb.b = *b;
    sb.held_ptr.assign(1, 0);
    sb.traj_ptr.assign(1, 0);
    for (int gl = 0; gl < (int)groups.size(); gl++) {
        const int g = groups[gl];
        sb.group_series.push_back(b->group_series[g]);
        if (b->held_ptr)
            for (int k = b->held_ptr[g]; k < b->held_ptr[g + 1]; k++) sb.held_idx.push_back(b->held_idx[k]);
        sb.held_ptr.push_back((int)sb.held_idx.size());
        sb.traj_ptr.push_back(sb.traj_ptr.back() + b->T[b->group_series[g]]);
        for (int f = fit_lo[g]; f >= 0 && f < fit_hi[g]; f++) {
            sb.fits.push_back(f);
            sb.fit_group.push_back(gl);
        }
    }
    sb.theta0.resize(sb.fits.size() * (size_t)b->theta_stride);
    for (size_t i = 0; i < sb.fits.size(); i++)
        std::memcpy(&sb.theta0[i * b->theta_stride], b->theta0 + (size_t)sb.fits[i] * b->theta_stride,
                    sizeof(double) * b->theta_stride);
    if (sb.held_idx.empty()) sb.held_idx.push_back(0);
    sb.b.n_groups = (int)groups.size();
    sb.b.group_series = sb.group_series.data();
    sb.b.held_ptr = sb.held_ptr.data();
    sb.b.held_idx = sb.held_idx.data();
    sb.b.n_fits = (int)sb.fits.size();
    sb.b.fit_group = sb.fit_group.data();
    sb.b.theta0 = sb.theta0.data();
}

static void shard_groups(const ldsr_batch *b, int n_shards, int *group_shard) {
    const int ng = b->n_groups;
    std::vector<double> cost(ng, 0.0);
    for (int f = 0; f < b->n_fits; f++) {
        const int g = b->fit_group[f], s = b->group_series[g];
        cost[g] += (double)b->T[s] * (b->p[s] + b->q[s] + 8);
    }
    std::vector<int> order(ng);
    std::iota(order.begin(), order.end(), 0);
    std::stable_sort(order.begin(), order.end(), [&](int a, int c) { return cost[a] > cost[c]; });
    std::vector<double> load(n_shards, 0.0);
    for (int g : order) {
        const int d = (int)(std::min_element(load.begin(), load.end()) - load.begin());
        group_shard[g] = d;
        load[d] += cost[g];
    }
}

static Err em_batch(ldsr_ctx *ctx, const ldsr_batch *b, int niter, double tol, const ldsr_options *opt,
                    ldsr_em_result *out) {
    Err e = validate(b);
    if (!e.ok()) return e;
    if (!out) return fail(LDSR_ERR_ARG, "result struct is NULL");
    std::unique_ptr<ldsr_ctx> tmp_ctx;
    if (!ctx) {
        ldsr_ctx *c = nullptr;
        char buf[256];
        int rc = ldsr_ctx_create(opt ? opt->n_devices : 0, opt ? opt->devices : nullptr, &c, buf, sizeof buf);
        if (rc != LDSR_OK) return fail(rc, "%s", buf);
        tmp_ctx.reset(c);
        ctx = c;
    }
    int nd = (int)ctx->devices.size();
    if (opt && opt->n_devices > 0) nd = std::min(nd, opt->n_devices);
    nd = std::max(1, std::min(nd, b->n_groups));
    const bool want_liks = out->liks != nullptr;

    if (nd == 1) {
        static const bool timing = std::getenv("LDSR_TIMING") != nullptr;
        auto now = [] { return std::chrono::steady_clock::now(); };
        auto ms = [](std::chrono::steady_clock::time_point a, std::chrono::steady_clock::time_point c) {
            return std::chrono::duration<double, std::milli>(c - a).count();
        };
        const auto t0 = now();
        ldsr_plan *P = nullptr;
        e = plan_build(b, ctx->devices[0], ctx->pools[0].get(), &P);
        if (!e.ok()) return e;
        const auto t1 = now();
        {
            std::unique_ptr<ldsr_plan> guard(P);
            e = plan_em(P, niter, tol, opt, nullptr, want_liks, nullptr, nullptr);
            if (!e.ok()) return e;
            const auto t2 = now();
            e = plan_fetch(P, out);
            const auto t3 = now();
            guard.reset();
            if (timing)
                std::fprintf(stderr, "ldsr_em_batch: build %.3f ms, em %.3f ms, fetch %.3f ms, destroy %.3f ms\n",
                             ms(t0, t1), ms(t1, t2), ms(t2, t3), ms(t3, now()));
        }
        return e;
    }

    const int ng = b->n_groups;
    std::vector<int> fit_lo(ng, -1), fit_hi(ng, -1);
    for (int f = 0; f < b->n_fits; f++) {
        const int g = b->fit_group[f];
        if (fit_lo[g] < 0) fit_lo[g] = f;
        fit_hi[g] = f + 1;
    }
    {
        int nonempty = 0;
        for (int g = 0; g < ng; g++) nonempty += fit_lo[g] >= 0 ? 1 : 0;
        nd = std::max(1, std::min(nd, nonempty));
    }
    std::vector<int> shard(ng);
    shard_groups(b, nd, shard.data());
    std::vector<std::vector<int>> dev_groups(nd);
    for (int g = 0; g < ng; g++) dev_groups[shard[g]].push_back(g);
    std::vector<long long> traj_ptr(ng + 1, 0);
    for (int g = 0; g < ng; g++) traj_ptr[g + 1] = traj_ptr[g] + b->T[b->group_series[g]];

    ldsr_options wopt;
    std::memset(&wopt, 0, sizeof wopt);
    if (opt) wopt = *opt;
    wopt.poll = nullptr;
    wopt.poll_arg = nullptr;
    if (wopt.variant == 0) {
        int width = 1;
        for (int s = 0; s < b->n_series; s++) {
            if (b->u && b->u[s]) width = std::max(width, b->p[s]);
            if (b->v && b->v[s]) width = std::max(width, b->q[s]);
        }
        const KernelTable *kt_all = kernel_table_for(width);
        if (kt_all && b->n_fits > scan_auto_fits(kt_all->pq)) wopt.variant = 6;
    }
    const bool caller_polls = opt && opt->poll;
    std::vector<SubBatch> subs(nd);
    std::vector<Err> errs(nd);
    std::atomic<int> abort_flag(0);
    std::mutex mu;
    std::condition_variable cv;
    int running = nd;
    static const bool timing = std::getenv("LDSR_TIMING") != nullptr;
    std::vector<double> dev_ms(nd, 0.0);
    std::vector<std::thread> workers;
    for (int d = 0; d < nd; d++) {
        workers.emplace_back([&, d]() {
            const auto t0 = std::chrono::steady_clock::now();
            SubBatch &sb = subs[d];
            make_sub(b, dev_groups[d], fit_lo, fit_hi, sb);
            Err er;
            if (sb.fits.empty()) {
                const double nan = std::nan("");
                for (int g : sb.groups) {
                    if (out->best) out->best[g] = -1;
                    for (double *rowp : {out->X, out->Y, out->V, out->J})
                        if (rowp) std::fill(rowp + traj_ptr[g], rowp + traj_ptr[g + 1], nan);
                }
            } else {
                ldsr_plan *P = nullptr;
                er = plan_build(&sb.b, ctx->devices[d], ctx->pools[d].get(), &P);
                if (er.ok()) {
                    std::unique_ptr<ldsr_plan> guard(P);
                    er = plan_em(P, niter, tol, &wopt, nullptr, want_liks, caller_polls ? &abort_flag : nullptr, nullptr);
                    if (er.ok()) {
                        FetchMap map{sb.fits.data(), sb.groups.data(), traj_ptr.data(), niter};
                        er = plan_fetch(P, out, &map);
                    }
                }
            }
            if (!er.ok()) abort_flag.store(1);
            errs[d] = er;
            dev_ms[d] = std::chrono::duration<double, std::milli>(std::chrono::steady_clock::now() - t0).count();
            {
                std::lock_guard<std::mutex> lk(mu);
                running--;
            }
            cv.notify_all();
        });
    }
    bool interrupted = false;
    {
        std::unique_lock<std::mutex> lk(mu);
        while (running > 0) {
            if (!caller_polls) {
                cv.wait(lk);
                continue;
            }
            cv.wait_for(lk, std::chrono::milliseconds(20));
            if (running > 0 && !interrupted) {
                lk.unlock();
                const bool stop = opt->poll(opt->poll_arg) != 0;
                lk.lock();
                if (stop) {
                    interrupted = true;
                    abort_flag.store(1);
                }
            }
        }
    }
    for (auto &w : workers) w.join();
    if (timing)
        for (int d = 0; d < nd; d++)
            std::fprintf(stderr, "ldsr_em_batch: device %d: %zu groups, %zu fits, %.3f ms\n", ctx->devices[d],
                         subs[d].groups.size(), subs[d].fits.size(), dev_ms[d]);
    if (interrupted) return fail(LDSR_ERR_INTERRUPTED, "interrupted by the poll callback");
    for (int d = 0; d < nd; d++)
        if (!errs[d].ok() && errs[d].code != LDSR_ERR_INTERRUPTED) return errs[d];
    for (int d = 0; d < nd; d++)
        if (!errs[d].ok()) return errs[d];
    return Err();
}

static thread_local double g_last_device_ms = 0.0;

enum class StepKind { Smoother, Propagate };

static Err step_batch(ldsr_ctx *ctx, const ldsr_batch *b, StepKind kind, int stdlik, double *X, double *Y, double *V,
                      double *J, double *lik, double *aux = nullptr, bool rows_to_host = true) {
    std::unique_ptr<ldsr_ctx> tmp_ctx;
    if (!ctx) {
        ldsr_ctx *c = nullptr;
        char buf[256];
        int rc = ldsr_ctx_create(1, nullptr, &c, buf, sizeof buf);
        if (rc != LDSR_OK) return fail(rc, "%s", buf);
        tmp_ctx.reset(c);
        ctx = c;
    }
    if (rows_to_host && (!X || !Y || !V)) return fail(LDSR_ERR_ARG, "X, Y and V outputs are required");
    ldsr_plan *P = nullptr;
    Err e = plan_build(b, ctx->devices[0], ctx->pools[0].get(), &P);
    if (!e.ok()) return e;
    std::unique_ptr<ldsr_plan> guard(P);
    const int nf = P->n_fits;
    std::vector<long long> row_user(nf + 1, 0);
    for (int f = 0; f < nf; f++) row_user[f + 1] = row_user[f] + b->T[b->group_series[b->fit_group[f]]];
    std::vector<long long> jr(nf);
    std::vector<int> jt(nf);
    for (int fi = 0; fi < nf; fi++) {
        jr[fi] = row_user[P->f_user[fi]];
        jt[fi] = fi;
    }
    const size_t tot = (size_t)row_user[nf];
    double *dX, *dY, *dV, *dJ = nullptr, *dlik, *daux = nullptr;
    int *d_jt;
    long long *d_jr;
    if (!(e = P->dalloc(&dX, tot)).ok()) return e;
    if (!(e = P->dalloc(&dY, tot)).ok()) return e;
    if (!(e = P->dalloc(&dV, tot)).ok()) return e;
    if (J && !(e = P->dalloc(&dJ, tot)).ok()) return e;
    if (!(e = P->dalloc(&dlik, nf)).ok()) return e;
    if (aux && !(e = P->dalloc(&daux, nf)).ok()) return e;
    if (!(e = P->upload(&d_jt, jt)).ok()) return e;
    if (!(e = P->upload(&d_jr, jr)).ok()) return e;
    SmootherParams sp;
    sp.series = P->d_series;
    sp.blobs = P->d_blobs;
    sp.g_series = P->d_g_series;
    sp.masks = P->d_masks;
    sp.g_mask_off = P->d_g_mask_off;
    sp.g_nobs = P->d_g_nobs;
    sp.n_jobs = nf;
    sp.job_group = P->d_f_group;
    sp.job_theta = d_jt;
    sp.job_row = d_jr;
    sp.theta = P->d_theta0;
    sp.X = dX;
    sp.Y = dY;
    sp.V = dV;
    sp.J = dJ;
    sp.lik = dlik;
    sp.stdlik = stdlik;
    sp.aux = daux;
    CU(kind == StepKind::Smoother ? P->kt->smoother(sp, P->stream) : P->kt->propagate(sp, P->stream));
    CU(cudaStreamSynchronize(P->stream));
    if (rows_to_host) {
        CU(cudaMemcpy(X, dX, tot * sizeof(double), cudaMemcpyDeviceToHost));
        CU(cudaMemcpy(Y, dY, tot * sizeof(double), cudaMemcpyDeviceToHost));
        CU(cudaMemcpy(V, dV, tot * sizeof(double), cudaMemcpyDeviceToHost));
        if (J) CU(cudaMemcpy(J, dJ, tot * sizeof(double), cudaMemcpyDeviceToHost));
    }
    if (aux) {
        std::vector<double> a(nf);
        CU(cudaMemcpy(a.data(), daux, nf * sizeof(double), cudaMemcpyDeviceToHost));
        for (int fi = 0; fi < nf; fi++) aux[P->f_user[fi]] = a[fi];
    }
    if (lik) {
        std::vector<double> l(nf);
        CU(cudaMemcpy(l.data(), dlik, nf * sizeof(double), cudaMemcpyDeviceToHost));
        for (int fi = 0; fi < nf; fi++) lik[P->f_user[fi]] = l[fi];
    }
    return Err();
}

static Err mstep_batch(ldsr_ctx *ctx, const ldsr_batch *b, const double *X, const double *V, const double *J,
                       double *theta_out, int *status) {
    std::unique_ptr<ldsr_ctx> tmp_ctx;
    if (!ctx) {
        ldsr_ctx *c = nullptr;
        char buf[256];
        int rc = ldsr_ctx_create(1, nullptr, &c, buf, sizeof buf);
        if (rc != LDSR_OK) return fail(rc, "%s", buf);
        tmp_ctx.reset(c);
        ctx = c;
    }
    if (!X || !V || !J || !theta_out) return fail(LDSR_ERR_ARG, "X, V, J and theta_out are required");
    ldsr_plan *P = nullptr;
    Err e = plan_build(b, ctx->devices[0], ctx->pools[0].get(), &P);
    if (!e.ok()) return e;
    std::unique_ptr<ldsr_plan> guard(P);
    const int nf = P->n_fits;
    std::vector<long long> row_user(nf + 1, 0);
    for (int f = 0; f < nf; f++) row_user[f + 1] = row_user[f] + b->T[b->group_series[b->fit_group[f]]];
    std::vector<long long> fr(nf);
    for (int fi = 0; fi < nf; fi++) fr[fi] = row_user[P->f_user[fi]];
    const size_t tot = (size_t)row_user[nf];
    double *dX, *dV, *dJ, *dth;
    int *dst;
    long long *d_fr;
    if (!(e = P->dalloc(&dX, tot)).ok()) return e;
    if (!(e = P->dalloc(&dV, tot)).ok()) return e;
    if (!(e = P->dalloc(&dJ, tot)).ok()) return e;
    if (!(e = P->dalloc(&dth, (size_t)nf * P->TL)).ok()) return e;
    if (!(e = P->dalloc(&dst, nf)).ok()) return e;
    if (!(e = P->upload(&d_fr, fr)).ok()) return e;
    CU(cudaMemcpyAsync(dX, X, tot * sizeof(double), cudaMemcpyHostToDevice, P->stream));
    CU(cudaMemcpyAsync(dV, V, tot * sizeof(double), cudaMemcpyHostToDevice, P->stream));
    CU(cudaMemcpyAsync(dJ, J, tot * sizeof(double), cudaMemcpyHostToDevice, P->stream));
    MstepParams mp;
    mp.series = P->d_series;
    mp.blobs = P->d_blobs;
    mp.sconst = P->d_sconst;
    mp.g_series = P->d_g_series;
    mp.masks = P->d_masks;
    mp.g_mask_off = P->d_g_mask_off;
    mp.gconst = P->d_gconst;
    mp.g_status = P->d_g_status;
    mp.n_fits = nf;
    mp.f_group = P->d_f_group;
    mp.f_row = d_fr;
    mp.X = dX;
    mp.V = dV;
    mp.J = dJ;
    mp.theta_out = dth;
    mp.status = dst;
    CU(P->kt->mstep(mp, P->stream));
    CU(cudaStreamSynchronize(P->stream));
    std::vector<double> th((size_t)nf * P->TL);
    std::vector<int> stt(nf);
    CU(cudaMemcpy(th.data(), dth, th.size() * sizeof(double), cudaMemcpyDeviceToHost));
    CU(cudaMemcpy(stt.data(), dst, nf * sizeof(int), cudaMemcpyDeviceToHost));
    for (int fi = 0; fi < nf; fi++) {
        const int s = P->h_g_series[P->h_f_group[fi]];
        unpad_theta(&th[(size_t)fi * P->TL], P->s_p[s], P->s_q[s], P->h_series[s].has_u != 0,
                    P->h_series[s].has_v != 0, P->PQ, theta_out + (size_t)P->f_user[fi] * P->theta_stride);
        if (status) status[P->f_user[fi]] = stt[fi];
    }
    return Err();
}

static Err rep_batch(ldsr_ctx *ctx, const double *theta, const double *u, const double *v, int n, int p, int q,
                     int n_reps, const double *z, unsigned long long seed, double mu, int exp_trans, double *simX,
                     double *simY, double *simQ, const unsigned *r_seed = nullptr) {
    if (!theta || n < 1 || n_reps < 1 || p < 0 || q < 0) return fail(LDSR_ERR_ARG, "bad theta/n/n_reps/p/q");
    if (p > LDSR_MAX_PQ || q > LDSR_MAX_PQ) return fail(LDSR_ERR_UNSUPPORTED, "p or q exceeds LDSR_MAX_PQ");
    std::unique_ptr<ldsr_ctx> tmp_ctx;
    if (!ctx) {
        ldsr_ctx *c = nullptr;
        char buf[256];
        int rc = ldsr_ctx_create(1, nullptr, &c, buf, sizeof buf);
        if (rc != LDSR_OK) return fail(rc, "%s", buf);
        tmp_ctx.reset(c);
        ctx = c;
    }
    CU(cudaSetDevice(ctx->devices[0]));
    DevicePool *pool = ctx->pools[0].get();
    const int need = std::max(1, std::max(u ? p : 0, v ? q : 0));
    const KernelTable *kt = kernel_table_for(need);
    if (!kt) return fail(LDSR_ERR_UNSUPPORTED, "no kernel for width %d", need);
    const int PQ = kt->pq;
    std::vector<double> th(2 * PQ + 6), up((size_t)n * PQ, 0.0), vp((size_t)n * PQ, 0.0);
    pad_theta(theta, p, q, u != nullptr, v != nullptr, PQ, th.data());
    for (int t = 0; t < n; t++) {
        if (u)
            for (int j = 0; j < p; j++) up[(size_t)t * PQ + j] = u[(size_t)t * p + j];
        if (v)
            for (int j = 0; j < q; j++) vp[(size_t)t * PQ + j] = v[(size_t)t * q + j];
    }
    std::vector<void *> held;
    auto dal = [&](size_t bytes, void **pp) -> cudaError_t {
        cudaError_t e = pool->alloc(bytes, pp);
        if (e == cudaSuccess) held.push_back(*pp);
        return e;
    };
    struct Rel {
        DevicePool *pool;
        std::vector<void *> *h;
        ~Rel() {
            for (void *p : *h) pool->release(p);
        }
    } rel{pool, &held};
    double *dth, *du, *dv, *dz_all = nullptr;
    CU(dal(th.size() * 8, (void **)&dth));
    CU(dal(up.size() * 8, (void **)&du));
    CU(dal(vp.size() * 8, (void **)&dv));
    CU(cudaMemcpy(dth, th.data(), th.size() * 8, cudaMemcpyHostToDevice));
    CU(cudaMemcpy(du, up.data(), up.size() * 8, cudaMemcpyHostToDevice));
    CU(cudaMemcpy(dv, vp.data(), vp.size() * 8, cudaMemcpyHostToDevice));
    const size_t zrow = 1 + 2 * (size_t)n;
    if (r_seed) {
        const long long nz = (long long)n_reps * (long long)zrow;
        CU(dal((size_t)nz * 8, (void **)&dz_all));
        CU(r_rnorm_device(*r_seed, nz, dz_all, 0));
    }
    double *outs[3] = {simX, simY, simQ};
    int n_out = 0;
    for (double *o : outs) n_out += o ? 1 : 0;
    g_last_device_ms = 0.0;
    if (n_out == 0) return Err();
    int chunk = (int)std::max<size_t>(128, ((size_t)48 << 20) / ((size_t)n * 8));
    chunk = std::min(n_reps, (chunk + 127) / 128 * 128);
    const int n_chunks = (n_reps + chunk - 1) / chunk;
    const size_t slot_doubles = (size_t)n_out * chunk * n;
    const size_t tot = (size_t)n * n_reps;
    static const bool force_chunked = std::getenv("LDSR_REP_CHUNKED") != nullptr;
    const bool whole =
        !force_chunked && (size_t)n_out * tot * 8 + (z ? (size_t)n_reps * zrow * 8 : 0) <= ((size_t)8 << 30);
    double *d_whole = nullptr;
    constexpr int SLOTS = 2;
    double *d_out[SLOTS] = {nullptr, nullptr}, *h_out[SLOTS] = {nullptr, nullptr}, *d_z[SLOTS] = {nullptr, nullptr};
    cudaEvent_t ev_k[SLOTS] = {nullptr, nullptr}, ev_c[SLOTS] = {nullptr, nullptr};
    std::vector<cudaEvent_t> ev_t;
    cudaStream_t sk = nullptr, sc = nullptr;
    struct Cleanup {
        DevicePool *pool;
        double **h;
        cudaEvent_t *a, *b;
        std::vector<cudaEvent_t> *t;
        cudaStream_t *sk, *sc;
        ~Cleanup() {
            if (*sk) cudaStreamSynchronize(*sk);
            if (*sc) cudaStreamSynchronize(*sc);
            for (int i = 0; i < SLOTS; i++) {
                if (h[i]) pool->release_pinned(h[i]);
                if (a[i]) cudaEventDestroy(a[i]);
                if (b[i]) cudaEventDestroy(b[i]);
            }
            for (cudaEvent_t e : *t) cudaEventDestroy(e);
            if (*sk) pool->put_stream(*sk);
            if (*sc) pool->put_stream(*sc);
        }
    } cleanup{pool, h_out, ev_k, ev_c, &ev_t, &sk, &sc};
    CU(pool->get_stream(&sk));
    CU(pool->get_stream(&sc));
    for (int i = 0; i < SLOTS && i < n_chunks; i++) {
        if (!whole) CU(dal(slot_doubles * 8, (void **)&d_out[i]));
        void *hp = nullptr;
        CU(pool->alloc_pinned(slot_doubles * 8, &hp));
        h_out[i] = static_cast<double *>(hp);
        if (z && !whole) CU(dal((size_t)chunk * zrow * 8, (void **)&d_z[i]));
        CU(cudaEventCreateWithFlags(&ev_k[i], cudaEventDisableTiming));
        CU(cudaEventCreateWithFlags(&ev_c[i], cudaEventDisableTiming));
    }
    auto copy_out = [&](int c) {
        const int slot = c % SLOTS, r0 = c * chunk, nr = std::min(chunk, n_reps - r0);
        const size_t bytes = (size_t)nr * n * 8;
        std::vector<std::thread> th;
        int k = 0;
        for (int o = 0; o < 3; o++) {
            if (!outs[o]) continue;
            const char *src = reinterpret_cast<const char *>(h_out[slot] + (size_t)k * chunk * n);
            char *dst = reinterpret_cast<char *>(outs[o] + (size_t)r0 * n);
            const int parts = bytes > ((size_t)4 << 20) ? 2 : 1;
            for (int pi = 0; pi < parts; pi++) {
                const size_t lo = bytes * pi / parts, hi = bytes * (pi + 1) / parts;
                th.emplace_back([=] { std::memcpy(dst + lo, src + lo, hi - lo); });
            }
            k++;
        }
        for (auto &t : th) t.join();
    };
    auto launch = [&](int r0, int nr, const double *zdev, double *base, size_t out_stride) -> Err {
        RepParams rp;
        rp.theta = dth;
        rp.u = du;
        rp.v = dv;
        rp.z = zdev;
        rp.seed = seed;
        rp.n = n;
        rp.n_reps = nr;
        rp.rep0 = r0;
        rp.mu = mu;
        rp.exp_trans = exp_trans;
        int k = 0;
        double *o3[3] = {nullptr, nullptr, nullptr};
        for (int o = 0; o < 3; o++)
            if (outs[o]) o3[o] = base + (size_t)(k++) * out_stride;
        rp.simX = o3[0];
        rp.simY = o3[1];
        rp.simQ = o3[2];
        cudaEvent_t ta = nullptr, tb = nullptr;
        CU(cudaEventCreate(&ta));
        ev_t.push_back(ta);
        CU(cudaEventCreate(&tb));
        ev_t.push_back(tb);
        CU(cudaEventRecord(ta, sk));
        CU(kt->rep(rp, sk));
        CU(cudaEventRecord(tb, sk));
        return Err();
    };
    if (whole) {
        CU(dal((size_t)n_out * tot * 8, (void **)&d_whole));
        const double *zdev = dz_all;
        if (z) {
            double *dzw = nullptr;
            CU(dal((size_t)n_reps * zrow * 8, (void **)&dzw));
            CU(cudaMemcpyAsync(dzw, z, (size_t)n_reps * zrow * 8, cudaMemcpyHostToDevice, sk));
            zdev = dzw;
        }
        Err e = launch(0, n_reps, zdev, d_whole, tot);
        if (!e.ok()) return e;
        CU(cudaEventRecord(ev_k[0], sk));
        CU(cudaStreamWaitEvent(sc, ev_k[0], 0));
    }
    for (int c = 0; c < n_chunks; c++) {
        const int slot = c % SLOTS, r0 = c * chunk, nr = std::min(chunk, n_reps - r0);
        if (c >= SLOTS) {
            CU(cudaEventSynchronize(ev_c[slot]));
            copy_out(c - SLOTS);
        }
        if (whole) {
            for (int k = 0; k < n_out; k++)
                CU(cudaMemcpyAsync(h_out[slot] + (size_t)k * chunk * n, d_whole + (size_t)k * tot + (size_t)r0 * n,
                                   (size_t)nr * n * 8, cudaMemcpyDeviceToHost, sc));
            CU(cudaEventRecord(ev_c[slot], sc));
            continue;
        }
        RepParams rp;
        rp.theta = dth;
        rp.u = du;
        rp.v = dv;
        rp.z = nullptr;
        if (z) {
            CU(cudaMemcpyAsync(d_z[slot], z + (size_t)r0 * zrow, (size_t)nr * zrow * 8, cudaMemcpyHostToDevice, sk));
            rp.z = d_z[slot];
        } else if (dz_all) {
            rp.z = dz_all + (size_t)r0 * zrow;
        }
        rp.seed = seed;
        rp.n = n;
        rp.n_reps = nr;
        rp.rep0 = r0;
        rp.mu = mu;
        rp.exp_trans = exp_trans;
        int k = 0;
        double *slot_out[3] = {nullptr, nullptr, nullptr};
        for (int o = 0; o < 3; o++)
            if (outs[o]) slot_out[o] = d_out[slot] + (size_t)(k++) * chunk * n;
        rp.simX = slot_out[0];
        rp.simY = slot_out[1];
        rp.simQ = slot_out[2];
        cudaEvent_t ta = nullptr, tb = nullptr;
        CU(cudaEventCreate(&ta));
        ev_t.push_back(ta);
        CU(cudaEventCreate(&tb));
        ev_t.push_back(tb);
        CU(cudaEventRecord(ta, sk));
        CU(kt->rep(rp, sk));
        CU(cudaEventRecord(tb, sk));
        CU(cudaEventRecord(ev_k[slot], sk));
        CU(cudaStreamWaitEvent(sc, ev_k[slot], 0));
        CU(cudaMemcpyAsync(h_out[slot], d_out[slot], slot_doubles * 8, cudaMemcpyDeviceToHost, sc));
        CU(cudaEventRecord(ev_c[slot], sc));
    }
    for (int c = std::max(0, n_chunks - SLOTS); c < n_chunks; c++) {
        CU(cudaEventSynchronize(ev_c[c % SLOTS]));
        copy_out(c);
    }
    CU(cudaStreamSynchronize(sk));
    for (size_t i = 0; i + 1 < ev_t.size(); i += 2) {
        float ms = 0.f;
        CU(cudaEventElapsedTime(&ms, ev_t[i], ev_t[i + 1]));
        g_last_device_ms += ms;
    }
    return Err();
}

}

extern "C" {

int ldsr_abi_version(void) { return LDSR_ABI_VERSION; }

int ldsr_device_count(void) {
    int n = 0;
    if (cudaGetDeviceCount(&n) != cudaSuccess) {
        cudaGetLastError();
        return 0;
    }
    return n;
}

int ldsr_ctx_create(int n_devices, const int *devices, ldsr_ctx **out, char *errbuf, int errlen) {
    if (!out) return report(fail(LDSR_ERR_ARG, "out is NULL"), errbuf, errlen);
    const int have = ldsr_device_count();
    if (have < 1)
        return report(fail(LDSR_ERR_CUDA, "no CUDA device available (this library has no CPU path)"), errbuf, errlen);
    if (n_devices <= 0) n_devices = have;
    std::unique_ptr<ldsr_ctx> c(new ldsr_ctx());
    for (int i = 0; i < n_devices; i++) {
        const int d = devices ? devices[i] : i;
        if (d < 0 || d >= have)
            return report(fail(LDSR_ERR_ARG, "device %d out of range (have %d)", d, have), errbuf, errlen);
        c->devices.push_back(d);
        c->pools.emplace_back(new DevicePool(d));
    }
    *out = c.release();
    return LDSR_OK;
}

void ldsr_ctx_destroy(ldsr_ctx *ctx) { delete ctx; }

long long ldsr_ctx_trim(ldsr_ctx *ctx, long long *cached_bytes) {
    long long freed = 0, kept = 0;
    if (ctx)
        for (auto &p : ctx->pools) {
            freed += (long long)p->trim();
            kept += (long long)p->cached_bytes();
        }
    if (cached_bytes) *cached_bytes = kept;
    return freed;
}

int ldsr_em_batch(ldsr_ctx *ctx, const ldsr_batch *batch, int niter, double tol, const ldsr_options *opt,
                  ldsr_em_result *out, char *errbuf, int errlen) {
    return report(em_batch(ctx, batch, niter, tol, opt, out), errbuf, errlen);
}

int ldsr_plan_create(const ldsr_batch *batch, int device, ldsr_plan **out, char *errbuf, int errlen) {
    if (!out) return report(fail(LDSR_ERR_ARG, "out is NULL"), errbuf, errlen);
    return report(plan_build(batch, device, nullptr, out), errbuf, errlen);
}

int ldsr_plan_em(ldsr_plan *plan, int niter, double tol, const ldsr_options *opt, void *stream, long long *stats,
                 char *errbuf, int errlen) {
    if (!plan) return report(fail(LDSR_ERR_ARG, "plan is NULL"), errbuf, errlen);
    return report(plan_em(plan, niter, tol, opt, (cudaStream_t)stream, opt && opt->trace_liks != 0, nullptr, stats),
                  errbuf, errlen);
}

int ldsr_plan_set_theta0(ldsr_plan *plan, const double *theta0_host, char *errbuf, int errlen) {
    if (!plan || !theta0_host) return report(fail(LDSR_ERR_ARG, "plan or theta0 is NULL"), errbuf, errlen);
    cudaSetDevice(plan->device);
    std::vector<double> th0((size_t)plan->n_fits * plan->TL);
    for (int fi = 0; fi < plan->n_fits; fi++) {
        const int s = plan->h_g_series[plan->h_f_group[fi]];
        pad_theta(theta0_host + (size_t)plan->f_user[fi] * plan->theta_stride, plan->s_p[s], plan->s_q[s],
                  plan->h_series[s].has_u != 0, plan->h_series[s].has_v != 0, plan->PQ, &th0[(size_t)fi * plan->TL]);
    }
    cudaError_t e = cudaMemcpy(plan->d_theta0, th0.data(), th0.size() * sizeof(double), cudaMemcpyHostToDevice);
    if (e != cudaSuccess) return report(fail(LDSR_ERR_CUDA, "theta0 upload: %s", cudaGetErrorString(e)), errbuf, errlen);
    return LDSR_OK;
}

int ldsr_plan_fetch(ldsr_plan *plan, ldsr_em_result *out, char *errbuf, int errlen) {
    if (!plan) return report(fail(LDSR_ERR_ARG, "plan is NULL"), errbuf, errlen);
    return report(plan_fetch(plan, out), errbuf, errlen);
}

void ldsr_plan_destroy(ldsr_plan *plan) { delete plan; }

int ldsr_smoother_batch(ldsr_ctx *ctx, const ldsr_batch *batch, int stdlik, double *X, double *Y, double *V, double *J,
                        double *lik, char *errbuf, int errlen) {
    return report(step_batch(ctx, batch, StepKind::Smoother, stdlik, X, Y, V, J, lik), errbuf, errlen);
}

int ldsr_mstep_batch(ldsr_ctx *ctx, const ldsr_batch *batch, const double *X, const double *V, const double *J,
                     double *theta_out, int *status, char *errbuf, int errlen) {
    return report(mstep_batch(ctx, batch, X, V, J, theta_out, status), errbuf, errlen);
}

int ldsr_propagate_batch(ldsr_ctx *ctx, const ldsr_batch *batch, int stdlik, double *X, double *Y, double *V,
                         double *lik, char *errbuf, int errlen) {
    return report(step_batch(ctx, batch, StepKind::Propagate, stdlik, X, Y, V, nullptr, lik), errbuf, errlen);
}

int ldsr_rep_batch(ldsr_ctx *ctx, const double *theta, const double *u, const double *v, int n, int p, int q,
                   int n_reps, const double *z, unsigned long long seed, double mu, int exp_trans, double *simX,
                   double *simY, double *simQ, char *errbuf, int errlen) {
    return report(rep_batch(ctx, theta, u, v, n, p, q, n_reps, z, seed, mu, exp_trans, simX, simY, simQ), errbuf,
                  errlen);
}

int ldsr_rep_batch_r(ldsr_ctx *ctx, const double *theta, const double *u, const double *v, int n, int p, int q,
                     int n_reps, unsigned int r_seed, double mu, int exp_trans, double *simX, double *simY,
                     double *simQ, char *errbuf, int errlen) {
    return report(rep_batch(ctx, theta, u, v, n, p, q, n_reps, nullptr, 0ull, mu, exp_trans, simX, simY, simQ, &r_seed),
                  errbuf, errlen);
}

struct ldsr_r_rng {
    ldsr::RMersenne g;
    explicit ldsr_r_rng(unsigned seed) : g(seed) {}
};

double ldsr_last_device_ms(void) { return g_last_device_ms; }

int ldsr_r_rng_create(unsigned int seed, ldsr_r_rng **out, char *errbuf, int errlen) {
    if (!out) return report(fail(LDSR_ERR_ARG, "out is NULL"), errbuf, errlen);
    *out = new (std::nothrow) ldsr_r_rng(seed);
    if (!*out) return report(fail(LDSR_ERR_ARG, "out of memory"), errbuf, errlen);
    return LDSR_OK;
}
int ldsr_r_rng_unif(ldsr_r_rng *rng, int n, double a, double b, double *out, char *errbuf, int errlen) {
    if (!rng || n < 0 || (n > 0 && !out)) return report(fail(LDSR_ERR_ARG, "rng / out is NULL or n < 0"), errbuf, errlen);
    for (int i = 0; i < n; i++) out[i] = a + (b - a) * rng->g.unif();
    return LDSR_OK;
}
int ldsr_r_rng_norm(ldsr_r_rng *rng, int n, double *out, char *errbuf, int errlen) {
    if (!rng || n < 0 || (n > 0 && !out)) return report(fail(LDSR_ERR_ARG, "rng / out is NULL or n < 0"), errbuf, errlen);
    for (int i = 0; i < n; i++) out[i] = rng->g.norm();
    return LDSR_OK;
}
int ldsr_r_rng_sample(ldsr_r_rng *rng, int n, int k, int *out, char *errbuf, int errlen) {
    if (!rng || n < 1 || k < 0 || k > n || (k > 0 && !out))
        return report(fail(LDSR_ERR_ARG, "need rng, 0 <= k <= n, n >= 1 and out"), errbuf, errlen);
    rng->g.sample_int(n, k, out);
    return LDSR_OK;
}
void ldsr_r_rng_destroy(ldsr_r_rng *rng) { delete rng; }

int ldsr_r_rnorm_device(int device, unsigned int seed, long long n, double *out, char *errbuf, int errlen) {
    auto run = [&]() -> Err {
        if (n < 1 || !out) return fail(LDSR_ERR_ARG, "need n >= 1 and out");
        if (ldsr_device_count() < 1) return fail(LDSR_ERR_CUDA, "no CUDA device available (this library has no CPU path)");
        CU(cudaSetDevice(device));
        double *d = nullptr;
        struct Guard {
            double *&p;
            ~Guard() { cudaFree(p); }
        } guard{d};
        CU(cudaMalloc(&d, sizeof(double) * (size_t)n));
        CU(r_rnorm_device(seed, n, d, 0));
        CU(cudaMemcpy(out, d, sizeof(double) * (size_t)n, cudaMemcpyDeviceToHost));
        return Err();
    };
    return report(run(), errbuf, errlen);
}

int ldsr_shard_groups(const ldsr_batch *batch, int n_shards, int *group_shard, char *errbuf, int errlen) {
    Err e = validate(batch);
    if (e.ok() && (n_shards < 1 || !group_shard)) e = fail(LDSR_ERR_ARG, "n_shards < 1 or group_shard is NULL");
    if (e.ok()) shard_groups(batch, n_shards, group_shard);
    return report(e, errbuf, errlen);
}

int ldsr_objective_batch(ldsr_ctx *ctx, const ldsr_batch *batch, int kind, double lambda, double *values, char *errbuf,
                         int errlen) {
    auto run = [&]() -> Err {
        if (!values) return fail(LDSR_ERR_ARG, "values is NULL");
        if (kind < 0 || kind > 2) return fail(LDSR_ERR_ARG, "kind must be 0 (penalized_likelihood), 1 (negLogLik) or 2 (ssqTrain)");
        if (!batch) return fail(LDSR_ERR_ARG, "batch is NULL");
        const int nf = batch->n_fits;
        std::vector<double> lik(std::max(nf, 1)), aux(std::max(nf, 1));
        Err e = step_batch(ctx, batch, kind == 0 ? StepKind::Smoother : StepKind::Propagate, kind == 0 ? 0 : 1, nullptr,
                           nullptr, nullptr, nullptr, lik.data(), aux.data(), false);
        if (!e.ok()) return e;
        for (int f = 0; f < nf; f++)
            values[f] = kind == 0 ? lik[f] - lambda * aux[f] : (kind == 1 ? -lik[f] : aux[f]);
        return Err();
    };
    return report(run(), errbuf, errlen);
}

static Err construct_rec_stations(int device, int n_stations, const int *T, const int *member_ptr, const double *X,
                                  const double *V, const double *Y, const double *C, const double *R, const double *mu,
                                  const double *lambda, int transform, double *out, double *mean) {
    if (n_stations < 1) return fail(LDSR_ERR_ARG, "need n_stations >= 1");
    if (!T || !member_ptr || !X || !V || !Y || !C || !R || !mu || !out) return fail(LDSR_ERR_ARG, "a required pointer is NULL");
    if (transform < 0 || transform > 2) return fail(LDSR_ERR_ARG, "transform must be 0 (none), 1 (log) or 2 (boxcox)");
    if (transform == 2 && !lambda) return fail(LDSR_ERR_ARG, "lambda is required with transform 2 (boxcox)");
    if (member_ptr[0] != 0) return fail(LDSR_ERR_ARG, "member_ptr[0] must be 0");
    std::vector<long long> row_off(n_stations), t_off(n_stations);
    std::vector<double> lam(n_stations, 0.0);
    long long rows = 0, years = 0;
    int max_T = 0;
    for (int s = 0; s < n_stations; s++) {
        if (T[s] < 1) return fail(LDSR_ERR_ARG, "station %d: need T >= 1", s);
        if (member_ptr[s + 1] <= member_ptr[s]) return fail(LDSR_ERR_ARG, "station %d: member_ptr not increasing (every station needs a member)", s);
        row_off[s] = rows;
        t_off[s] = years;
        rows += (long long)(member_ptr[s + 1] - member_ptr[s]) * T[s];
        years += T[s];
        max_T = std::max(max_T, T[s]);
        if (lambda) lam[s] = lambda[s];
    }
    const int n = member_ptr[n_stations];
    if (ldsr_device_count() < 1) return fail(LDSR_ERR_CUDA, "no CUDA device available (this library has no CPU path)");
    CU(cudaSetDevice(device));
    const size_t nT = (size_t)rows, S = (size_t)n_stations;
    double *d = nullptr;
    struct Guard {
        double *&p;
        ~Guard() { cudaFree(p); }
    } guard{d};
    const size_t n_dbl = 3 * nT + 2 * (size_t)n + 2 * S + 6 * nT + 2 * (size_t)years + 2 * S;
    CU(cudaMalloc(&d, sizeof(double) * n_dbl + sizeof(int) * (2 * S + 1)));
    double *dX = d, *dV = dX + nT, *dY = dV + nT, *dC = dY + nT, *dR = dC + n, *dmu = dR + n, *dlam = dmu + S;
    double *dO = dlam + S, *dM = dO + 6 * nT;
    long long *d_roff = reinterpret_cast<long long *>(dM + 2 * years), *d_toff = d_roff + S;
    int *d_T = reinterpret_cast<int *>(d_toff + S), *d_mp = d_T + S;
    CU(cudaMemcpy(dX, X, sizeof(double) * nT, cudaMemcpyHostToDevice));
    CU(cudaMemcpy(dV, V, sizeof(double) * nT, cudaMemcpyHostToDevice));
    CU(cudaMemcpy(dY, Y, sizeof(double) * nT, cudaMemcpyHostToDevice));
    CU(cudaMemcpy(dC, C, sizeof(double) * n, cudaMemcpyHostToDevice));
    CU(cudaMemcpy(dR, R, sizeof(double) * n, cudaMemcpyHostToDevice));
    CU(cudaMemcpy(dmu, mu, sizeof(double) * S, cudaMemcpyHostToDevice));
    CU(cudaMemcpy(dlam, lam.data(), sizeof(double) * S, cudaMemcpyHostToDevice));
    CU(cudaMemcpy(d_roff, row_off.data(), sizeof(long long) * S, cudaMemcpyHostToDevice));
    CU(cudaMemcpy(d_toff, t_off.data(), sizeof(long long) * S, cudaMemcpyHostToDevice));
    CU(cudaMemcpy(d_T, T, sizeof(int) * S, cudaMemcpyHostToDevice));
    CU(cudaMemcpy(d_mp, member_ptr, sizeof(int) * (S + 1), cudaMemcpyHostToDevice));
    const dim3 grid((max_T + 127) / 128, std::min(n_stations, 65535));
    construct_rec_kernel<<<grid, 128>>>(n_stations, d_T, d_mp, d_roff, d_toff, dX, dV, dY, dC, dR, dmu, dlam, transform,
                                        dO, mean ? dM : nullptr);
    CU(cudaGetLastError());
    CU(cudaMemcpy(out, dO, sizeof(double) * 6 * nT, cudaMemcpyDeviceToHost));
    if (mean) CU(cudaMemcpy(mean, dM, sizeof(double) * 2 * (size_t)years, cudaMemcpyDeviceToHost));
    return Err();
}

int ldsr_construct_rec_stations(int device, int n_stations, const int *T, const int *member_ptr, const double *X,
                                const double *V, const double *Y, const double *C, const double *R, const double *mu,
                                const double *lambda, int transform, double *out, double *mean, char *errbuf,
                                int errlen) {
    return report(construct_rec_stations(device, n_stations, T, member_ptr, X, V, Y, C, R, mu, lambda, transform, out,
                                         mean),
                  errbuf, errlen);
}

int ldsr_construct_rec_batch(int device, int n, int T, const double *X, const double *V, const double *Y,
                             const double *C, const double *R, double mu, int transform, double lambda, double *out,
                             double *mean, char *errbuf, int errlen) {
    const int member_ptr[2] = {0, n};
    return report(construct_rec_stations(device, 1, &T, member_ptr, X, V, Y, C, R, &mu, &lambda, transform, out, mean),
                  errbuf, errlen);
}

static Err cv_metrics_stations(int device, int n_stations, const int *n, const int *fold_ptr, const double *sim,
                               const double *obs, const int *z_ptr, const int *z_idx, int exp_trans, double *out) {
    if (n_stations < 1) return fail(LDSR_ERR_ARG, "need n_stations >= 1");
    if (!n || !fold_ptr || !sim || !obs || !z_ptr || !z_idx || !out) return fail(LDSR_ERR_ARG, "a required pointer is NULL");
    if (fold_ptr[0] != 0) return fail(LDSR_ERR_ARG, "fold_ptr[0] must be 0");
    for (int s = 0; s < n_stations; s++) {
        if (n[s] < 2) return fail(LDSR_ERR_ARG, "station %d: need a target of length n >= 2", s);
        if (fold_ptr[s + 1] < fold_ptr[s]) return fail(LDSR_ERR_ARG, "fold_ptr not monotone at station %d", s);
    }
    const int n_folds = fold_ptr[n_stations];
    if (n_folds < 1) return fail(LDSR_ERR_ARG, "need n_folds >= 1");
    if (z_ptr[0] < 0) return fail(LDSR_ERR_ARG, "z_ptr[0] < 0");
    std::vector<int> f_n(n_folds);
    std::vector<long long> f_obs(n_folds), f_row(n_folds);
    long long n_obs = 0, n_sim = 0;
    for (int s = 0; s < n_stations; s++) {
        for (int f = fold_ptr[s]; f < fold_ptr[s + 1]; f++) {
            f_n[f] = n[s];
            f_obs[f] = n_obs;
            f_row[f] = n_sim;
            n_sim += n[s];
        }
        n_obs += n[s];
    }
    std::vector<unsigned char> held((size_t)n_sim, 0);
    for (int f = 0; f < n_folds; f++) {
        if (z_ptr[f + 1] < z_ptr[f]) return fail(LDSR_ERR_ARG, "z_ptr not monotone at fold %d", f);
        for (int k = z_ptr[f]; k < z_ptr[f + 1]; k++) {
            const int i = z_idx[k] - 1;
            if (i < 0 || i >= f_n[f]) return fail(LDSR_ERR_ARG, "fold %d: hold-out index %d outside 1..%d", f, z_idx[k], f_n[f]);
            held[(size_t)f_row[f] + i] = 1;
        }
    }
    if (ldsr_device_count() < 1) return fail(LDSR_ERR_CUDA, "no CUDA device available (this library has no CPU path)");
    CU(cudaSetDevice(device));
    double *d_sim = nullptr, *d_obs = nullptr, *d_out = nullptr;
    unsigned char *d_held = nullptr;
    long long *d_off = nullptr;
    int *d_n = nullptr;
    struct Guard {
        double *&a, *&b, *&c;
        unsigned char *&h;
        long long *&o;
        int *&n;
        ~Guard() {
            cudaFree(a);
            cudaFree(b);
            cudaFree(c);
            cudaFree(h);
            cudaFree(o);
            cudaFree(n);
        }
    } guard{d_sim, d_obs, d_out, d_held, d_off, d_n};
    CU(cudaMalloc(&d_sim, sizeof(double) * (size_t)n_sim));
    CU(cudaMalloc(&d_obs, sizeof(double) * (size_t)n_obs));
    CU(cudaMalloc(&d_out, sizeof(double) * (size_t)n_folds * 5));
    CU(cudaMalloc(&d_held, held.size()));
    CU(cudaMalloc(&d_off, sizeof(long long) * 2 * (size_t)n_folds));
    CU(cudaMalloc(&d_n, sizeof(int) * (size_t)n_folds));
    CU(cudaMemcpy(d_sim, sim, sizeof(double) * (size_t)n_sim, cudaMemcpyHostToDevice));
    CU(cudaMemcpy(d_obs, obs, sizeof(double) * (size_t)n_obs, cudaMemcpyHostToDevice));
    CU(cudaMemcpy(d_held, held.data(), held.size(), cudaMemcpyHostToDevice));
    CU(cudaMemcpy(d_off, f_obs.data(), sizeof(long long) * n_folds, cudaMemcpyHostToDevice));
    CU(cudaMemcpy(d_off + n_folds, f_row.data(), sizeof(long long) * n_folds, cudaMemcpyHostToDevice));
    CU(cudaMemcpy(d_n, f_n.data(), sizeof(int) * n_folds, cudaMemcpyHostToDevice));
    cv_metrics_kernel<<<(n_folds + 3) / 4, 128>>>(n_folds, d_n, d_off, d_off + n_folds, d_sim, d_obs, d_held, exp_trans,
                                                  d_out);
    CU(cudaGetLastError());
    CU(cudaMemcpy(out, d_out, sizeof(double) * (size_t)n_folds * 5, cudaMemcpyDeviceToHost));
    return Err();
}

int ldsr_cv_metrics_stations(int device, int n_stations, const int *n, const int *fold_ptr, const double *sim,
                             const double *obs, const int *z_ptr, const int *z_idx, int exp_trans, double *out,
                             char *errbuf, int errlen) {
    return report(cv_metrics_stations(device, n_stations, n, fold_ptr, sim, obs, z_ptr, z_idx, exp_trans, out), errbuf,
                  errlen);
}

int ldsr_cv_metrics_batch(int device, int n, int n_folds, const double *sim, const double *obs, const int *z_ptr,
                          const int *z_idx, int exp_trans, double *out, char *errbuf, int errlen) {
    const int fold_ptr[2] = {0, n_folds};
    return report(cv_metrics_stations(device, 1, &n, fold_ptr, sim, obs, z_ptr, z_idx, exp_trans, out), errbuf, errlen);
}

int ldsr_smoother_d_batch(int device, int d, int T, int p, int q, const double *y, const double *u, const double *v,
                          int n_fits, const double *theta, int theta_stride, int stdlik, int method, int chunk,
                          double *X, double *V, double *Y, double *lik, double *kernel_ms, char *errbuf,
                          int errlen) {
    auto run = [&]() -> Err {
        if (d < 1 || d > LDSR_MAX_STATE_DIM)
            return fail(LDSR_ERR_UNSUPPORTED, "state dimension %d outside 1..%d", d, LDSR_MAX_STATE_DIM);
        if (T < 2 || p < 0 || q < 0 || n_fits < 1) return fail(LDSR_ERR_ARG, "need T >= 2, p,q >= 0, n_fits >= 1");
        if (!y || !theta || !lik) return fail(LDSR_ERR_ARG, "y, theta and lik are required");
        if ((u && p < 1) || (v && q < 1)) return fail(LDSR_ERR_ARG, "u/v given with p/q = 0");
        const int tl = 2 * d * d + d * p + d + q + 1 + d + d * d;
        if (theta_stride < tl) return fail(LDSR_ERR_ARG, "theta_stride=%d < %d", theta_stride, tl);
        if (method != 0 && method != 1) return fail(LDSR_ERR_ARG, "method must be 0 (sequential) or 1 (scan)");
        for (int t = 0; t < T; t++)
            if (std::isinf(y[t])) return fail(LDSR_ERR_ARG, "y[%d] is +-Inf", t);
        if (ldsr_device_count() < 1) return fail(LDSR_ERR_CUDA, "no CUDA device available (this library has no CPU path)");
        CU(cudaSetDevice(device));
        ScanParams P;
        std::memset(&P, 0, sizeof P);
        P.n_fits = n_fits;
        P.T = T;
        P.p = p;
        P.q = q;
        P.stdlik = stdlik;
        P.theta_len = tl;
        if (method == 0) {
            P.L = T;
        } else if (chunk > 0) {
            P.L = std::min(chunk, T);
        } else {
            int L = 8;
            while (L < 64 && (long long)L * L * 256 < T) L *= 2;
            const double want = 0.05 * std::sqrt((double)n_fits * (double)T);
            int Lg = 4;
            while (Lg < 64 && (double)Lg * 1.41421356 < want) Lg *= 2;
            if (scan_groups_for((T + Lg - 1) / Lg) > 1) L = Lg;
            P.L = L;
        }
        P.n_chunks = (T + P.L - 1) / P.L;
        std::vector<void *> bufs;
        struct Guard {
            std::vector<void *> &b;
            ~Guard() {
                for (void *p : b) cudaFree(p);
            }
        } guard{bufs};
        auto dalloc = [&](double **out, size_t n) -> cudaError_t {
            void *ptr = nullptr;
            cudaError_t e = cudaMalloc(&ptr, std::max<size_t>(n, 1) * sizeof(double));
            if (e == cudaSuccess) {
                bufs.push_back(ptr);
                *out = static_cast<double *>(ptr);
            }
            return e;
        };
        const size_t nT = (size_t)n_fits * T, D = d, nC = (size_t)n_fits * P.n_chunks;
        double *dy = nullptr, *du = nullptr, *dv_in = nullptr, *dth = nullptr;
        CU(dalloc(&dy, T));
        CU(cudaMemcpy(dy, y, sizeof(double) * T, cudaMemcpyHostToDevice));
        if (u) {
            CU(dalloc(&du, (size_t)T * p));
            CU(cudaMemcpy(du, u, sizeof(double) * (size_t)T * p, cudaMemcpyHostToDevice));
        }
        if (v) {
            CU(dalloc(&dv_in, (size_t)T * q));
            CU(cudaMemcpy(dv_in, v, sizeof(double) * (size_t)T * q, cudaMemcpyHostToDevice));
        }
        std::vector<double> th((size_t)n_fits * tl);
        for (int f = 0; f < n_fits; f++) std::memcpy(&th[(size_t)f * tl], theta + (size_t)f * theta_stride, sizeof(double) * tl);
        CU(dalloc(&dth, th.size()));
        CU(cudaMemcpy(dth, th.data(), sizeof(double) * th.size(), cudaMemcpyHostToDevice));
        P.y = dy;
        P.u = du;
        P.v = dv_in;
        P.theta = dth;
        CU(dalloc(&P.c, nT * D));
        CU(dalloc(&P.dv, nT));
        CU(dalloc(&P.Xu, nT * D));
        CU(dalloc(&P.Vu, nT * D * D));
        CU(dalloc(&P.fagg, nC * (3 * D * D + 2 * D)));
        CU(dalloc(&P.sagg, nC * (2 * D * D + D)));
        CU(dalloc(&P.pre, nC * (D + D * D)));
        CU(dalloc(&P.suf, nC * (D + D * D)));
        CU(dalloc(&P.likp, nC * 2));
        P.n_groups = scan_groups_for(P.n_chunks);
        if (const char *ev = std::getenv("LDSR_SCAN_GROUPS"))
            if (std::atoi(ev) == 1) P.n_groups = 1;
        if (P.n_groups > 1) {
            const size_t nG = (size_t)n_fits * P.n_groups;
            CU(dalloc(&P.fgagg, nG * (3 * D * D + 2 * D)));
            CU(dalloc(&P.fgpre, nG * (3 * D * D + 2 * D)));
            CU(dalloc(&P.sgagg, nG * (2 * D * D + D)));
            CU(dalloc(&P.sgsuf, nG * (2 * D * D + D)));
        }
        CU(dalloc(&P.X, nT * D));
        CU(dalloc(&P.V, nT * D * D));
        CU(dalloc(&P.Y, nT));
        CU(dalloc(&P.lik, n_fits));
        cudaEvent_t a, b;
        CU(cudaEventCreate(&a));
        CU(cudaEventCreate(&b));
        CU(cudaEventRecord(a, nullptr));
        cudaError_t le = scan_smoother_launch(d, P, nullptr);
        cudaEventRecord(b, nullptr);
        cudaError_t se = cudaEventSynchronize(b);
        float ms = 0.f;
        cudaEventElapsedTime(&ms, a, b);
        cudaEventDestroy(a);
        cudaEventDestroy(b);
        CU(le);
        CU(se);
        CU(cudaGetLastError());
        if (kernel_ms) *kernel_ms = ms;
        CU(cudaMemcpy(lik, P.lik, sizeof(double) * n_fits, cudaMemcpyDeviceToHost));
        if (X) CU(cudaMemcpy(X, P.X, sizeof(double) * nT * D, cudaMemcpyDeviceToHost));
        if (V) CU(cudaMemcpy(V, P.V, sizeof(double) * nT * D * D, cudaMemcpyDeviceToHost));
        if (Y) CU(cudaMemcpy(Y, P.Y, sizeof(double) * nT, cudaMemcpyDeviceToHost));
        return Err();
    };
    return report(run(), errbuf, errlen);
}

int ldsr_measure_fp64_peak(int device, double *tflops, char *errbuf, int errlen) {
    auto run = [&]() -> Err {
        if (!tflops) return fail(LDSR_ERR_ARG, "tflops is NULL");
        if (ldsr_device_count() < 1) return fail(LDSR_ERR_CUDA, "no CUDA device available");
        CU(cudaSetDevice(device));
        cudaDeviceProp prop;
        CU(cudaGetDeviceProperties(&prop, device));
        double *d = nullptr;
        CU(cudaMalloc(&d, 64));
        cudaEvent_t a, b;
        CU(cudaEventCreate(&a));
        CU(cudaEventCreate(&b));
        const int blocks = prop.multiProcessorCount * 2, threads = 1024, iters = 4096;
        double best = 0.0;
        for (int rep = 0; rep < 6; rep++) {
            CU(cudaEventRecord(a));
            dfma_peak_kernel<<<blocks, threads>>>(d, iters, 1.0000001, 1e-9);
            CU(cudaEventRecord(b));
            CU(cudaEventSynchronize(b));
            float ms = 0.f;
            CU(cudaEventElapsedTime(&ms, a, b));
            const double fl = 2.0 * 64.0 * iters * (double)blocks * threads;
            if (rep > 0) best = std::max(best, fl / (ms * 1e-3) / 1e12);
        }
        cudaEventDestroy(a);
        cudaEventDestroy(b);
        cudaFree(d);
        *tflops = best;
        return Err();
    };
    return report(run(), errbuf, errlen);
}

}
```

Before: 735,100.

## Interleave word and M-segment units across two pieces in split walks

```diff
diff --git a/ldsr_b200/csrc/em_split_kernel.cuh b/ldsr_b200/csrc/em_split_kernel.cuh
--- a/ldsr_b200/csrc/em_split_kernel.cuh
+++ b/ldsr_b200/csrc/em_split_kernel.cuh
@@ -4,6 +4,9 @@
 namespace ldsr {
 
 constexpr int SPLIT_NCH = 10;
+#ifndef LDSR_SPLIT_PAIR
+#define LDSR_SPLIT_PAIR 0
+#endif
 
 template <int PQ> __host__ __device__ constexpr int split_nstat() { return 11 + 3 * PQ; }
 
@@ -24,6 +27,12 @@
 }
 
 constexpr int UNIT_M = 1 << 30, UNIT_M1 = 1 << 29, UNIT_US = 1 << 28, UNIT_T0 = UNIT_US - 1;
+
+__host__ __device__ inline bool split_is_word(int u) { return u >= 0 && !(u & (UNIT_M | UNIT_M1 | UNIT_US)); }
+__host__ __device__ inline bool split_is_short(int u) { return u >= 0 && (u & (UNIT_M1 | UNIT_US)); }
+__host__ __device__ inline bool split_pairable(int ua, int ub) {
+    return (split_is_word(ua) && ub >= 0 && (ub & UNIT_M)) || (ua >= 0 && (ua & UNIT_M) && split_is_word(ub));
+}
 
 template <class F> __host__ __device__ inline void split_window_units(int t0, int T, int mseg, int uw, F f) {
     const int end = T < t0 + uw ? T : t0 + uw;
@@ -196,190 +205,239 @@
     double PJ, PJ2, G0, GG, Lc;
 };
 
+template <int PQ, int UW, int N> struct FwdUnit {
+    double Bu[N], ymd[N];
+    UnitGains<N> G;
+    double q[N + 1], P[N + 1];
+    __device__ __forceinline__ void inputs(const Theta<PQ> &th, unsigned bits, const double *__restrict__ yseg,
+                                           const double *__restrict__ useg, const double *__restrict__ vseg) {
+        double yo[N], ur[N * PQ], vr[N * PQ];
+        unit_inputs<PQ, N>(th, bits, yseg, useg, vseg, Bu, ymd, yo, ur, vr);
+    }
+    __device__ __forceinline__ void gains(const Theta<PQ> &th, const SplitConst<PQ, UW> &k, unsigned bits,
+                                          const PieceFwd &c) {
+        unit_gains<PQ, UW, N>(th, k, bits, c.Vq, G);
+    }
+    __device__ __forceinline__ void mean(const SplitConst<PQ, UW> &k, const PieceFwd &c) {
+        q[0] = c.q;
+        P[0] = c.P;
+#pragma unroll
+        for (int j = 0; j < N; j++) {
+            const double beta = fma(k.A * G.K[j], ymd[j], Bu[j]);
+            q[j + 1] = fma(G.alpha[j], q[j], beta);
+            P[j + 1] = G.alpha[j] * P[j];
+        }
+    }
+    __device__ __forceinline__ void finish(const Theta<PQ> &th, PieceFwd &c) {
+        double g0[N], gP[N];
+#pragma unroll
+        for (int j = 0; j < N; j++) {
+            const double d0 = fma(-th.C, q[j], ymd[j]);
+            const double w0 = G.rS[j] * d0;
+            c.l0 = fma(w0, d0, c.l0);
+            c.l1 = fma(w0, P[j], c.l1);
+            c.l2 = fma(G.rS[j] * P[j], P[j], c.l2);
+            const double xu0 = fma(G.K[j], d0, q[j]);
+            const double xuP = P[j] * fma(-G.K[j], th.C, 1.0);
+            g0[j] = fma(-G.J[j], q[j + 1], xu0);
+            gP[j] = fma(-G.J[j], P[j + 1], xuP);
+        }
+        double pj = c.PJ, pj2 = c.PJ2;
+#pragma unroll
+        for (int j = 0; j < N; j++) {
+            c.G0 = fma(pj, g0[j], c.G0);
+            c.GG = fma(pj, gP[j], c.GG);
+            c.Lc = fma(pj2, G.L[j], c.Lc);
+            pj *= G.J[j];
+            pj2 *= G.J[j] * G.J[j];
+        }
+        c.PJ = pj;
+        c.PJ2 = pj2;
+        c.q = q[N];
+        c.P = P[N];
+        c.Vq = G.Vnext;
+        c.dprod *= G.dend;
+        {
+            const int e = ((__double2hiint(c.dprod) >> 20) & 0x7ff) - 1023;
+            c.dprod *= __hiloint2double((1023 - e) << 20, 0);
+            c.shift += e;
+        }
+    }
+};
 template <int PQ, int UW, int N>
 __device__ __forceinline__ void forward_unit_basis(const Theta<PQ> &th, const SplitConst<PQ, UW> &k, unsigned bits,
                                                    const double *__restrict__ yseg, const double *__restrict__ useg,
                                                    const double *__restrict__ vseg, PieceFwd &c) {
-    double Bu[N], ymd[N], yo[N];
-    {
-        double ur[N * PQ], vr[N * PQ];
-        unit_inputs<PQ, N>(th, bits, yseg, useg, vseg, Bu, ymd, yo, ur, vr);
-    }
-    UnitGains<N> G;
-    unit_gains<PQ, UW, N>(th, k, bits, c.Vq, G);
-    double q[N + 1], P[N + 1];
-    q[0] = c.q;
-    P[0] = c.P;
-#pragma unroll
-    for (int j = 0; j < N; j++) {
-        const double beta = fma(k.A * G.K[j], ymd[j], Bu[j]);
-        q[j + 1] = fma(G.alpha[j], q[j], beta);
-        P[j + 1] = G.alpha[j] * P[j];
-    }
-    double g0[N], gP[N];
-#pragma unroll
-    for (int j = 0; j < N; j++) {
-        const double d0 = fma(-th.C, q[j], ymd[j]);
-        const double w0 = G.rS[j] * d0;
-        c.l0 = fma(w0, d0, c.l0);
-        c.l1 = fma(w0, P[j], c.l1);
-        c.l2 = fma(G.rS[j] * P[j], P[j], c.l2);
-        const double xu0 = fma(G.K[j], d0, q[j]);
-        const double xuP = P[j] * fma(-G.K[j], th.C, 1.0);
-        g0[j] = fma(-G.J[j], q[j + 1], xu0);
-        gP[j] = fma(-G.J[j], P[j + 1], xuP);
-    }
-    double pj = c.PJ, pj2 = c.PJ2;
-#pragma unroll
-    for (int j = 0; j < N; j++) {
-        c.G0 = fma(pj, g0[j], c.G0);
-        c.GG = fma(pj, gP[j], c.GG);
-        c.Lc = fma(pj2, G.L[j], c.Lc);
-        pj *= G.J[j];
-        pj2 *= G.J[j] * G.J[j];
-    }
-    c.PJ = pj;
-    c.PJ2 = pj2;
-    c.q = q[N];
-    c.P = P[N];
-    c.Vq = G.Vnext;
-    c.dprod *= G.dend;
-    {
-        const int e = ((__double2hiint(c.dprod) >> 20) & 0x7ff) - 1023;
-        c.dprod *= __hiloint2double((1023 - e) << 20, 0);
-        c.shift += e;
-    }
-}
-
+    FwdUnit<PQ, UW, N> f;
+    f.inputs(th, bits, yseg, useg, vseg);
+    f.gains(th, k, bits, c);
+    f.mean(k, c);
+    f.finish(th, c);
+}
+
+template <int PQ, int UW> struct FwdWord {
+    static constexpr bool KEEP_W = split_w_in_smem(PQ);
+    double A4, hh;
+    double W[KEEP_W ? PQ : 1];
+    __device__ __forceinline__ void begin(const SplitConst<PQ, UW> &k) {
+        A4 = k.A2 * k.A2;
+        hh = 0.0;
+        if (KEEP_W) {
+#pragma unroll
+            for (int i = 0; i < PQ; i++) W[i] = 0.0;
+        }
+    }
+    template <class Mid>
+    __device__ __forceinline__ void block(const Theta<PQ> &th, const SplitConst<PQ, UW> &k,
+                                          const double *__restrict__ blk, Mid mid) {
+        double ur[8 * PQ];
+        load_vec<8 * PQ>(blk, ur);
+        mid();
+        if (KEEP_W) {
+#pragma unroll
+            for (int i = 0; i < PQ; i++) {
+                double lo = ur[i], hi = ur[4 * PQ + i];
+#pragma unroll
+                for (int j = 1; j < 4; j++) {
+                    lo = fma(k.A, lo, ur[j * PQ + i]);
+                    hi = fma(k.A, hi, ur[(4 + j) * PQ + i]);
+                }
+                W[i] = fma(W[i], k.A8, fma(lo, A4, hi));
+            }
+        } else {
+            double Bu[8];
+#pragma unroll
+            for (int j = 0; j < 8; j++) {
+                double acc = 0.0;
+#pragma unroll
+                for (int i = 0; i < PQ; i++) acc = fma(th.b(i), ur[j * PQ + i], acc);
+                Bu[j] = acc;
+            }
+            double lo = Bu[0], hi = Bu[4];
+#pragma unroll
+            for (int j = 1; j < 4; j++) {
+                lo = fma(k.A, lo, Bu[j]);
+                hi = fma(k.A, hi, Bu[4 + j]);
+            }
+            hh = fma(hh, k.A8, fma(lo, A4, hi));
+        }
+    }
+    __device__ __forceinline__ void finish(const Theta<PQ> &th, const SplitConst<PQ, UW> &k, double *__restrict__ wk,
+                                           PieceFwd &c) {
+        if (KEEP_W) {
+#pragma unroll
+            for (int i = 0; i < PQ; i++) {
+                hh = fma(th.b(i), W[i], hh);
+                wk[i * 32] = W[i];
+            }
+        }
+        const double AW = k.AW();
+        const double qn = fma(AW, c.q, hh);
+        const double Pn = AW * c.P;
+        const double Vn = fma(k.aVW, c.Vq, k.bVW);
+        const double Jc = AW * c.Vq * fast_rcp(Vn);
+        const double g0 = fma(-Jc, qn, c.q);
+        const double gP = fma(-Jc, Pn, c.P);
+        const double L = c.Vq * fma(-AW, Jc, 1.0);
+        c.G0 = fma(c.PJ, g0, c.G0);
+        c.GG = fma(c.PJ, gP, c.GG);
+        c.Lc = fma(c.PJ2, L, c.Lc);
+        c.PJ *= Jc;
+        c.PJ2 *= Jc * Jc;
+        c.q = qn;
+        c.P = Pn;
+        c.Vq = Vn;
+    }
+};
 template <int PQ, int UW>
 __device__ __forceinline__ void forward_word_basis(const Theta<PQ> &th, const SplitConst<PQ, UW> &k,
                                                    const double *__restrict__ useg, double *__restrict__ wk,
                                                    PieceFwd &c) {
-    constexpr bool KEEP_W = split_w_in_smem(PQ);
-    const double A4 = k.A2 * k.A2;
-    double hh = 0.0;
-    double W[KEEP_W ? PQ : 1];
-    if (KEEP_W) {
-#pragma unroll
-        for (int i = 0; i < PQ; i++) W[i] = 0.0;
-    }
+    FwdWord<PQ, UW> f;
+    f.begin(k);
 #pragma unroll 1
-    for (int b = 0; b < UW / 8; b++) {
-        double ur[8 * PQ];
-        load_vec<8 * PQ>(useg + b * 8 * PQ, ur);
-        if (KEEP_W) {
-#pragma unroll
-            for (int i = 0; i < PQ; i++) {
-                double lo = ur[i], hi = ur[4 * PQ + i];
-#pragma unroll
-                for (int j = 1; j < 4; j++) {
-                    lo = fma(k.A, lo, ur[j * PQ + i]);
-                    hi = fma(k.A, hi, ur[(4 + j) * PQ + i]);
-                }
-                W[i] = fma(W[i], k.A8, fma(lo, A4, hi));
-            }
-        } else {
-            double Bu[8];
-#pragma unroll
-            for (int j = 0; j < 8; j++) {
-                double acc = 0.0;
-#pragma unroll
-                for (int i = 0; i < PQ; i++) acc = fma(th.b(i), ur[j * PQ + i], acc);
-                Bu[j] = acc;
-            }
-            double lo = Bu[0], hi = Bu[4];
-#pragma unroll
-            for (int j = 1; j < 4; j++) {
-                lo = fma(k.A, lo, Bu[j]);
-                hi = fma(k.A, hi, Bu[4 + j]);
-            }
-            hh = fma(hh, k.A8, fma(lo, A4, hi));
-        }
-    }
-    if (KEEP_W) {
-#pragma unroll
-        for (int i = 0; i < PQ; i++) {
-            hh = fma(th.b(i), W[i], hh);
-            wk[i * 32] = W[i];
-        }
-    }
-    const double AW = k.AW();
-    const double qn = fma(AW, c.q, hh);
-    const double Pn = AW * c.P;
-    const double Vn = fma(k.aVW, c.Vq, k.bVW);
-    const double Jc = AW * c.Vq * fast_rcp(Vn);
-    const double g0 = fma(-Jc, qn, c.q);
-    const double gP = fma(-Jc, Pn, c.P);
-    const double L = c.Vq * fma(-AW, Jc, 1.0);
-    c.G0 = fma(c.PJ, g0, c.G0);
-    c.GG = fma(c.PJ, gP, c.GG);
-    c.Lc = fma(c.PJ2, L, c.Lc);
-    c.PJ *= Jc;
-    c.PJ2 *= Jc * Jc;
-    c.q = qn;
-    c.P = Pn;
-    c.Vq = Vn;
-}
-
+    for (int b = 0; b < UW / 8; b++) f.block(th, k, useg + b * 8 * PQ, [] {});
+    f.finish(th, k, wk, c);
+}
+
+template <int PQ, int UW, int N, bool KEEP_ROWS> struct SmoothUnit {
+    double Bu[N], ymd[N], yo[N];
+    double ur[N * PQ], vr[N * PQ];
+    UnitGains<N> G;
+    double xq[N + 1], g[N];
+    double Xs[N + 1], Vs[N + 1];
+    __device__ __forceinline__ void inputs(const Theta<PQ> &th, unsigned bits, const double *__restrict__ yseg,
+                                           const double *__restrict__ useg, const double *__restrict__ vseg) {
+        unit_inputs<PQ, N>(th, bits, yseg, useg, vseg, Bu, ymd, yo, ur, vr);
+    }
+    __device__ __forceinline__ void gains(const Theta<PQ> &th, const SplitConst<PQ, UW> &k, unsigned bits, double Vq) {
+        unit_gains<PQ, UW, N>(th, k, bits, Vq, G);
+    }
+    __device__ __forceinline__ void filter(const Theta<PQ> &th, const SplitConst<PQ, UW> &k, double Xq) {
+        xq[0] = Xq;
+#pragma unroll
+        for (int j = 0; j < N; j++) xq[j + 1] = fma(G.alpha[j], xq[j], fma(k.A * G.K[j], ymd[j], Bu[j]));
+#pragma unroll
+        for (int j = 0; j < N; j++) {
+            const double delta = fma(-th.C, xq[j], ymd[j]);
+            const double xu = fma(G.K[j], delta, xq[j]);
+            g[j] = fma(-G.J[j], xq[j + 1], xu);
+        }
+    }
+    __device__ __forceinline__ void backward(double &Xs1, double &Vs1) {
+        Xs[N] = Xs1;
+        Vs[N] = Vs1;
+#pragma unroll
+        for (int j = N - 1; j >= 0; j--) {
+            Xs[j] = fma(G.J[j], Xs[j + 1], g[j]);
+            Vs[j] = fma(G.J[j] * G.J[j], Vs[j + 1], G.L[j]);
+        }
+        Xs1 = Xs[0];
+        Vs1 = Vs[0];
+    }
+    __device__ __forceinline__ void sums(unsigned bits, bool last, const double *__restrict__ useg,
+                                         const double *__restrict__ vseg, Stats<PQ> &st) {
+        if (!KEEP_ROWS) {
+            load_vec<N * PQ>(useg, ur);
+            load_vec<N * PQ>(vseg, vr);
+        }
+#pragma unroll
+        for (int j = 0; j < N; j++) {
+            if (N == 1 && last) {
+                st.XT = Xs[j];
+                st.VT = Vs[j];
+            } else {
+                st.Tx1x = fma(Xs[j + 1], Xs[j], st.Tx1x);
+                st.Tx1xv = fma(Vs[j + 1], G.J[j], st.Tx1xv);
+                st.Txx = fma(Xs[j], Xs[j], st.Txx);
+                st.Txxv += Vs[j];
+#pragma unroll
+                for (int i = 0; i < PQ; i++) {
+                    st.Tx1u[i] = fma(Xs[j + 1], ur[j * PQ + i], st.Tx1u[i]);
+                    st.Tux[i] = fma(ur[j * PQ + i], Xs[j], st.Tux[i]);
+                }
+            }
+            const bool obs = (bits >> j) & 1u;
+            const double xo = obs ? Xs[j] : 0.0;
+            st.Syx = fma(yo[j], xo, st.Syx);
+            st.Sxx = fma(xo, xo, st.Sxx);
+            st.Sxxv += obs ? Vs[j] : 0.0;
+#pragma unroll
+            for (int i = 0; i < PQ; i++) st.Sxv[i] = fma(xo, vr[j * PQ + i], st.Sxv[i]);
+        }
+    }
+};
 template <int PQ, int UW, int N>
 __device__ __forceinline__ void smooth_unit(const Theta<PQ> &th, const SplitConst<PQ, UW> &k, unsigned bits, bool last,
                                             const double *__restrict__ yseg, const double *__restrict__ useg,
                                             const double *__restrict__ vseg, double Xq, double Vq, double &Xs1,
                                             double &Vs1, Stats<PQ> &st) {
-    constexpr bool KEEP_ROWS = N * PQ <= 16;
-    double Bu[N], ymd[N], yo[N];
-    double ur[N * PQ], vr[N * PQ];
-    unit_inputs<PQ, N>(th, bits, yseg, useg, vseg, Bu, ymd, yo, ur, vr);
-    UnitGains<N> G;
-    unit_gains<PQ, UW, N>(th, k, bits, Vq, G);
-    double xq[N + 1], g[N];
-    xq[0] = Xq;
-#pragma unroll
-    for (int j = 0; j < N; j++) xq[j + 1] = fma(G.alpha[j], xq[j], fma(k.A * G.K[j], ymd[j], Bu[j]));
-#pragma unroll
-    for (int j = 0; j < N; j++) {
-        const double delta = fma(-th.C, xq[j], ymd[j]);
-        const double xu = fma(G.K[j], delta, xq[j]);
-        g[j] = fma(-G.J[j], xq[j + 1], xu);
-    }
-    double Xs[N + 1], Vs[N + 1];
-    Xs[N] = Xs1;
-    Vs[N] = Vs1;
-#pragma unroll
-    for (int j = N - 1; j >= 0; j--) {
-        Xs[j] = fma(G.J[j], Xs[j + 1], g[j]);
-        Vs[j] = fma(G.J[j] * G.J[j], Vs[j + 1], G.L[j]);
-    }
-    if (!KEEP_ROWS) {
-        load_vec<N * PQ>(useg, ur);
-        load_vec<N * PQ>(vseg, vr);
-    }
-#pragma unroll
-    for (int j = 0; j < N; j++) {
-        if (N == 1 && last) {
-            st.XT = Xs[j];
-            st.VT = Vs[j];
-        } else {
-            st.Tx1x = fma(Xs[j + 1], Xs[j], st.Tx1x);
-            st.Tx1xv = fma(Vs[j + 1], G.J[j], st.Tx1xv);
-            st.Txx = fma(Xs[j], Xs[j], st.Txx);
-            st.Txxv += Vs[j];
-#pragma unroll
-            for (int i = 0; i < PQ; i++) {
-                st.Tx1u[i] = fma(Xs[j + 1], ur[j * PQ + i], st.Tx1u[i]);
-                st.Tux[i] = fma(ur[j * PQ + i], Xs[j], st.Tux[i]);
-            }
-        }
-        const bool obs = (bits >> j) & 1u;
-        const double xo = obs ? Xs[j] : 0.0;
-        st.Syx = fma(yo[j], xo, st.Syx);
-        st.Sxx = fma(xo, xo, st.Sxx);
-        st.Sxxv += obs ? Vs[j] : 0.0;
-#pragma unroll
-        for (int i = 0; i < PQ; i++) st.Sxv[i] = fma(xo, vr[j * PQ + i], st.Sxv[i]);
-    }
-    Xs1 = Xs[0];
-    Vs1 = Vs[0];
+    SmoothUnit<PQ, UW, N, N * PQ <= 16> m;
+    m.inputs(th, bits, yseg, useg, vseg);
+    m.gains(th, k, bits, Vq);
+    m.filter(th, k, Xq);
+    m.backward(Xs1, Vs1);
+    m.sums(bits, last, useg, vseg, st);
 }
 
 template <int N> struct ShortConst {
@@ -489,86 +547,151 @@
     o[6 * 32] = Q2 * Z;
 }
 
+template <int PQ, int UW> struct SmoothWord {
+    static constexpr int NB = UW / 8;
+    static constexpr bool KEEP_W = split_w_in_smem(PQ);
+    double qg0, g1, g2, g3, G0, H0, Xfirst, Vfirst;
+    double Xs;
+    double tux[KEEP_W ? PQ : 1];
+    __device__ __forceinline__ void begin(const SplitConst<PQ, UW> &k, const double *__restrict__ uv, double Xq,
+                                          double Vq, double cG, double cH, Stats<PQ> &st) {
+        qg0 = k.Q * cG;
+        g1 = k.A8 * qg0;
+        g2 = k.A16 * qg0;
+        g3 = k.A8 * g2;
+        G0 = (NB == 4 ? k.A8 * k.A16 * k.A8 : k.A16) * cG;
+        H0 = k.aVW * cH;
+        Xfirst = fma(Vq, G0, Xq);
+        Vfirst = fma(Vq, Vq * H0, Vq);
+        {
+            const double sumVp = fma(uv[0 * 32], Vq, uv[1 * 32]);
+            const double qa = uv[2 * 32] * Vq;
+            st.Txxv += fma(cH, fma(Vq, qa + uv[3 * 32], uv[4 * 32]), sumVp);
+            st.Tx1xv = fma(k.A, fma(cH, fma(Vq, qa + uv[5 * 32], uv[6 * 32]), sumVp), st.Tx1xv);
+        }
+        Xs = Xfirst;
+        if (KEEP_W) {
+#pragma unroll
+            for (int i = 0; i < PQ; i++) tux[i] = 0.0;
+        }
+    }
+    template <class Mid>
+    __device__ __forceinline__ void block(const Theta<PQ> &th, const SplitConst<PQ, UW> &k,
+                                          const double *__restrict__ useg, int b, Stats<PQ> &st, Mid mid) {
+        const int r = NB - 1 - b;
+        const double Gb = r == 0 ? qg0 : (r == 1 ? g1 : (r == 2 ? g2 : g3));
+        const double *__restrict__ blk = useg + b * 8 * PQ;
+        constexpr bool KEEP_U = PQ <= 4;
+        double uk[8 * PQ];
+        load_vec<8 * PQ>(blk, uk);
+        mid();
+        double Gs[8];
+        Gs[7] = Gb;
+#pragma unroll
+        for (int j = 6; j >= 0; j--) Gs[j] = k.A * Gs[j + 1];
+        double inp[8];
+#pragma unroll
+        for (int j = 0; j < 8; j++) {
+            double acc = Gs[j];
+#pragma unroll
+            for (int i = 0; i < PQ; i++) acc = fma(th.b(i), uk[j * PQ + i], acc);
+            inp[j] = acc;
+        }
+        double Xn[9];
+        Xn[0] = Xs;
+#pragma unroll
+        for (int j = 0; j < 8; j++) Xn[j + 1] = fma(k.A, Xn[j], inp[j]);
+        if (!KEEP_U) load_vec<8 * PQ>(blk, uk);
+#pragma unroll
+        for (int j = 0; j < 8; j++) {
+            st.Tx1x = fma(Xn[j + 1], Xn[j], st.Tx1x);
+            st.Txx = fma(Xn[j], Xn[j], st.Txx);
+#pragma unroll
+            for (int i = 0; i < PQ; i++) {
+                if (KEEP_W) {
+                    tux[i] = fma(uk[j * PQ + i], Xn[j], tux[i]);
+                } else {
+                    st.Tx1u[i] = fma(Xn[j + 1], uk[j * PQ + i], st.Tx1u[i]);
+                    st.Tux[i] = fma(uk[j * PQ + i], Xn[j], st.Tux[i]);
+                }
+            }
+        }
+        Xs = Xn[8];
+    }
+    __device__ __forceinline__ void finish(const Theta<PQ> &th, const SplitConst<PQ, UW> &k,
+                                           const double *__restrict__ wk, const double *__restrict__ tuu_w, double &cG,
+                                           double &cH, double &Xs1, double &Vs1, Stats<PQ> &st) {
+        if (KEEP_W) {
+#pragma unroll
+            for (int i = 0; i < PQ; i++) {
+                double acc = fma(qg0, wk[i * 32], k.A * tux[i]);
+#pragma unroll
+                for (int j = 0; j < PQ; j++) acc = fma(th.b(j), tuu_w[j * PQ + i], acc);
+                st.Tx1u[i] += acc;
+                st.Tux[i] += tux[i];
+            }
+        }
+        Xs1 = Xfirst;
+        Vs1 = Vfirst;
+        cG = G0;
+        cH = H0;
+    }
+};
 template <int PQ, int UW>
 __device__ __forceinline__ void smooth_word(const Theta<PQ> &th, const SplitConst<PQ, UW> &k,
                                             const double *__restrict__ useg, const double *__restrict__ uv,
                                             const double *__restrict__ wk, const double *__restrict__ tuu_w,
                                             double Xq, double Vq, double &cG, double &cH, double &Xs1, double &Vs1,
                                             Stats<PQ> &st) {
+    SmoothWord<PQ, UW> w;
+    w.begin(k, uv, Xq, Vq, cG, cH, st);
+#pragma unroll 1
+    for (int b = 0; b < SmoothWord<PQ, UW>::NB; b++) w.block(th, k, useg, b, st, [] {});
+    w.finish(th, k, wk, tuu_w, cG, cH, Xs1, Vs1, st);
+}
+
+template <int PQ, int UW, int N>
+__device__ __forceinline__ void forward_pair(const Theta<PQ> &th, const SplitConst<PQ, UW> &k,
+                                             const double *__restrict__ useg_w, double *__restrict__ wk, PieceFwd &cw,
+                                             unsigned bits, const double *__restrict__ yseg,
+                                             const double *__restrict__ useg_m, const double *__restrict__ vseg_m,
+                                             PieceFwd &cm) {
     constexpr int NB = UW / 8;
-    constexpr bool KEEP_W = split_w_in_smem(PQ);
-    const double qg0 = k.Q * cG;
-    const double g1 = k.A8 * qg0, g2 = k.A16 * qg0, g3 = k.A8 * g2;
-    const double G0 = (NB == 4 ? k.A8 * k.A16 * k.A8 : k.A16) * cG;
-    const double H0 = k.aVW * cH;
-    const double Xfirst = fma(Vq, G0, Xq), Vfirst = fma(Vq, Vq * H0, Vq);
-    {
-        const double sumVp = fma(uv[0 * 32], Vq, uv[1 * 32]);
-        const double qa = uv[2 * 32] * Vq;
-        st.Txxv += fma(cH, fma(Vq, qa + uv[3 * 32], uv[4 * 32]), sumVp);
-        st.Tx1xv = fma(k.A, fma(cH, fma(Vq, qa + uv[5 * 32], uv[6 * 32]), sumVp), st.Tx1xv);
-    }
-    double Xs = Xfirst;
-    double tux[KEEP_W ? PQ : 1];
-    if (KEEP_W) {
-#pragma unroll
-        for (int i = 0; i < PQ; i++) tux[i] = 0.0;
-    }
-#pragma unroll 1
-    for (int b = 0; b < NB; b++) {
-        const int r = NB - 1 - b;
-        const double Gb = r == 0 ? qg0 : (r == 1 ? g1 : (r == 2 ? g2 : g3));
-        const double *__restrict__ blk = useg + b * 8 * PQ;
-        constexpr bool KEEP_U = PQ <= 4;
-        double uk[8 * PQ];
-        load_vec<8 * PQ>(blk, uk);
-        double Gs[8];
-        Gs[7] = Gb;
-#pragma unroll
-        for (int j = 6; j >= 0; j--) Gs[j] = k.A * Gs[j + 1];
-        double inp[8];
-#pragma unroll
-        for (int j = 0; j < 8; j++) {
-            double acc = Gs[j];
-#pragma unroll
-            for (int i = 0; i < PQ; i++) acc = fma(th.b(i), uk[j * PQ + i], acc);
-            inp[j] = acc;
-        }
-        double Xn[9];
-        Xn[0] = Xs;
-#pragma unroll
-        for (int j = 0; j < 8; j++) Xn[j + 1] = fma(k.A, Xn[j], inp[j]);
-        if (!KEEP_U) load_vec<8 * PQ>(blk, uk);
-#pragma unroll
-        for (int j = 0; j < 8; j++) {
-            st.Tx1x = fma(Xn[j + 1], Xn[j], st.Tx1x);
-            st.Txx = fma(Xn[j], Xn[j], st.Txx);
-#pragma unroll
-            for (int i = 0; i < PQ; i++) {
-                if (KEEP_W) {
-                    tux[i] = fma(uk[j * PQ + i], Xn[j], tux[i]);
-                } else {
-                    st.Tx1u[i] = fma(Xn[j + 1], uk[j * PQ + i], st.Tx1u[i]);
-                    st.Tux[i] = fma(uk[j * PQ + i], Xn[j], st.Tux[i]);
-                }
-            }
-        }
-        Xs = Xn[8];
-    }
-    if (KEEP_W) {
-#pragma unroll
-        for (int i = 0; i < PQ; i++) {
-            double acc = fma(qg0, wk[i * 32], k.A * tux[i]);
-#pragma unroll
-            for (int j = 0; j < PQ; j++) acc = fma(th.b(j), tuu_w[j * PQ + i], acc);
-            st.Tx1u[i] += acc;
-            st.Tux[i] += tux[i];
-        }
-    }
-    Xs1 = Xfirst;
-    Vs1 = Vfirst;
-    cG = G0;
-    cH = H0;
+    FwdWord<PQ, UW> w;
+    FwdUnit<PQ, UW, N> m;
+    w.begin(k);
+    m.inputs(th, bits, yseg, useg_m, vseg_m);
+#pragma unroll
+    for (int b = 0; b < NB; b++)
+        w.block(th, k, useg_w + b * 8 * PQ, [&] {
+            if (b == 0) m.gains(th, k, bits, cm);
+            if (b == NB / 4) m.mean(k, cm);
+            if (b == (2 * NB) / 4) m.finish(th, cm);
+        });
+    w.finish(th, k, wk, cw);
+}
+template <int PQ, int UW, int N>
+__device__ __forceinline__ void smooth_pair(const Theta<PQ> &th, const SplitConst<PQ, UW> &k,
+                                            const double *__restrict__ useg_w, const double *__restrict__ uv,
+                                            const double *__restrict__ wk, const double *__restrict__ tuu_w, double XqW,
+                                            double VqW, double &cG, double &cH, double &Xs1W, double &Vs1W,
+                                            unsigned bits, const double *__restrict__ yseg,
+                                            const double *__restrict__ useg_m, const double *__restrict__ vseg_m,
+                                            double XqM, double VqM, double &Xs1M, double &Vs1M, Stats<PQ> &st) {
+    constexpr int NB = SmoothWord<PQ, UW>::NB;
+    SmoothWord<PQ, UW> w;
+    SmoothUnit<PQ, UW, N, false> m;
+    w.begin(k, uv, XqW, VqW, cG, cH, st);
+    m.inputs(th, bits, yseg, useg_m, vseg_m);
+#pragma unroll
+    for (int b = 0; b < NB; b++)
+        w.block(th, k, useg_w, b, st, [&] {
+            if (b == 0) m.gains(th, k, bits, VqM);
+            if (b == NB / 4) m.filter(th, k, XqM);
+            if (b == (2 * NB) / 4) m.backward(Xs1M, Vs1M);
+            if (b == (3 * NB) / 4) m.sums(bits, false, useg_m, vseg_m, st);
+        });
+    w.finish(th, k, wk, tuu_w, cG, cH, Xs1W, Vs1W, st);
 }
 
 template <int PQ> __device__ __forceinline__ void stats_store(const Stats<PQ> &st, double *o) {
@@ -627,6 +750,7 @@
     int *ctl;
     const int *order;
     int n_sm;
+    int pair_walk = 1;
 #ifdef LDSR_PHASE_CLOCKS
     long long *clk;
 #endif
@@ -640,6 +764,7 @@
     } while (0)
 #define LDSR_UNIT_BEGIN() const long long ub_ = clock64()
 #define LDSR_UNIT_END(base, u0) pc[(base) + (((u0) & UNIT_M) ? 1 : ((u0) & UNIT_M1) ? 2 : ((u0) & UNIT_US) ? 3 : 0)] += clock64() - ub_
+#define LDSR_PAIR_END(kk) pc[kk] += clock64() - ub_
 #else
 #define LDSR_PHASE_MARK(kk) \
     do {                    \
@@ -650,7 +775,30 @@
 #define LDSR_UNIT_END(base, u0) \
     do {                        \
     } while (0)
+#define LDSR_PAIR_END(kk) \
+    do {                  \
+    } while (0)
 #endif
+constexpr int SPLIT_NCLK = 23;
+
+template <class V> __device__ __forceinline__ void swap_vals(V &a, V &b) {
+    const V t = a;
+    a = b;
+    b = t;
+}
+struct SplitBwd {
+    double xin, Xs1, Vs1, Xr, Vr, cG, cH;
+    int un, ua;
+    bool first, in_run;
+    __device__ __forceinline__ void enter_run() {
+        if (!in_run) {
+            const double rv = fast_rcp(Vr);
+            cG = (Xs1 - Xr) * rv;
+            cH = (Vs1 - Vr) * rv * rv;
+            in_run = true;
+        }
+    }
+};
 
 __device__ __forceinline__ int unit_cost(int u, int cost_u, int cost_m, int mseg) {
     if (u & UNIT_US) return cost_m / 5;
@@ -685,6 +833,7 @@
     constexpr int NST = split_nstat<PQ>();
     constexpr int NP = 2 * NW;
     constexpr bool PAIR = split_pairwise<PQ, NW>();
+    constexpr bool PAIR_WALK = LDSR_SPLIT_PAIR && MINB == 2 && !PAIR;
     constexpr int ST_SLOTS = split_st_slots<PQ, NW>();
     constexpr size_t CH_DOUBLES = (size_t)NP * SPLIT_NCH * 32, ST_DOUBLES = (size_t)ST_SLOTS * NST * 32;
 
@@ -856,7 +1005,7 @@
     __syncthreads();
 
 #ifdef LDSR_PHASE_CLOCKS
-    long long pc[21] = {0, 0, 0, 0, 0, 0, 0, 0, 0, 0, 0, 0, 0, 0, 0, 0, 0, 0, 0, 0, 0}, tprev = clock64();
+    long long pc[SPLIT_NCLK] = {}, tprev = clock64();
 #endif
     bool counted = false;
     for (int it = 0;; ++it) {
@@ -924,31 +1073,30 @@
         }
 
         LDSR_PHASE_MARK(10);
-#pragma unroll 1
-        for (int h = 0; h < 2; ++h) {
-            const int pj = h * NW + warp;
-            const int ua = pbound[pj], ue = pbound[pj + 1];
-            PieceFwd c;
-            c.Vq = h ? VinB : VinA;
-            c.P = 1.0;
-            c.q = 0.0;
-            c.l0 = c.l1 = c.l2 = 0.0;
-            c.dprod = 1.0;
-            c.shift = 0;
-            c.PJ = c.PJ2 = 1.0;
-            c.G0 = c.GG = c.Lc = 0.0;
-            bool any_m = false;
-            for (int un = ua; un < ue; ++un) {
-                const int u0 = units[un];
-                const int t0 = u0 & UNIT_T0;
+        if constexpr (PAIR_WALK) {
+            const auto fwd_init = [&](PieceFwd &c, double Vin) {
+                c.Vq = Vin;
+                c.P = 1.0;
+                c.q = 0.0;
+                c.l0 = c.l1 = c.l2 = 0.0;
+                c.dprod = 1.0;
+                c.shift = 0;
+                c.PJ = c.PJ2 = 1.0;
+                c.G0 = c.GG = c.Lc = 0.0;
+            };
+            const auto fwd_checkpoint = [&](int un, const PieceFwd &c) {
                 ck[(un * 3 + 0) * 32] = c.Vq;
                 ck[(un * 3 + 1) * 32] = c.q;
                 ck[(un * 3 + 2) * 32] = c.P;
+            };
+            const auto fwd_unit = [&](int un, PieceFwd &c, bool &any_m) {
+                const int u0 = units[un];
+                const int t0 = u0 & UNIT_T0;
+                fwd_checkpoint(un, c);
                 LDSR_UNIT_BEGIN();
                 if (u0 & UNIT_M) {
                     any_m = true;
-                    forward_unit_basis<PQ, UW, MSEG>(th, k, seg_bits(mw, t0, MSEG), ys + t0, us + t0 * PQ,
-                                                     vs + t0 * PQ, c);
+                    forward_unit_basis<PQ, UW, MSEG>(th, k, seg_bits(mw, t0, MSEG), ys + t0, us + t0 * PQ, vs + t0 * PQ, c);
                 } else if (u0 & UNIT_M1) {
                     any_m = true;
                     forward_unit_basis<PQ, UW, 1>(th, k, seg_bits(mw, t0, 1), ys + t0, us + t0 * PQ, vs + t0 * PQ, c);
@@ -958,20 +1106,108 @@
                     forward_word_basis<PQ, UW>(th, k, us + t0 * PQ, WK + (size_t)(t0 / UW) * PQ * 32, c);
                 }
                 LDSR_UNIT_END(13, u0);
-            }
-            double ld = 0.0;
-            if (any_m) ld = fma((double)c.shift, 0.693147180559945309417, log(c.dprod));
-            double *o = CH + (size_t)pj * SPLIT_NCH * 32;
-            o[0 * 32] = c.P;
-            o[1 * 32] = c.q;
-            o[2 * 32] = c.l0 + ld;
-            o[3 * 32] = c.l1;
-            o[4 * 32] = c.l2;
-            o[5 * 32] = c.PJ;
-            o[6 * 32] = c.G0;
-            o[7 * 32] = c.GG;
-            o[8 * 32] = c.Lc;
-            o[9 * 32] = c.Vq;
+            };
+            const auto fwd_publish = [&](int pj, const PieceFwd &c, bool any_m) {
+                double ld = 0.0;
+                if (any_m) ld = fma((double)c.shift, 0.693147180559945309417, log(c.dprod));
+                double *o = CH + (size_t)pj * SPLIT_NCH * 32;
+                o[0 * 32] = c.P;
+                o[1 * 32] = c.q;
+                o[2 * 32] = c.l0 + ld;
+                o[3 * 32] = c.l1;
+                o[4 * 32] = c.l2;
+                o[5 * 32] = c.PJ;
+                o[6 * 32] = c.G0;
+                o[7 * 32] = c.GG;
+                o[8 * 32] = c.Lc;
+                o[9 * 32] = c.Vq;
+            };
+            int pa = warp, pb = NW + warp;
+            int a = pbound[pa], ae = pbound[pa + 1], b = pbound[pb], be = pbound[pb + 1];
+            PieceFwd cA, cB;
+            fwd_init(cA, VinA);
+            fwd_init(cB, VinB);
+            bool mA = false, mB = false;
+            const auto swap_ab = [&] {
+                swap_vals(pa, pb);
+                swap_vals(a, b);
+                swap_vals(ae, be);
+                swap_vals(cA, cB);
+                swap_vals(mA, mB);
+            };
+            for (;;) {
+                const int uA = a < ae ? units[a] : -1, uB = b < be ? units[b] : -1;
+                if (uA < 0 && uB < 0) break;
+                if (SP.pair_walk && split_pairable(uA, uB)) {
+                    if (uA & UNIT_M) swap_ab();
+                    const int tw = units[a] & UNIT_T0, tm = units[b] & UNIT_T0;
+                    fwd_checkpoint(a, cA);
+                    fwd_checkpoint(b, cB);
+                    LDSR_UNIT_BEGIN();
+                    forward_pair<PQ, UW, MSEG>(th, k, us + tw * PQ, WK + (size_t)(tw / UW) * PQ * 32, cA,
+                                               seg_bits(mw, tm, MSEG), ys + tm, us + tm * PQ, vs + tm * PQ, cB);
+                    LDSR_PAIR_END(21);
+                    mB = true;
+                    a++;
+                    b++;
+                    continue;
+                }
+                if (uA < 0 || (SP.pair_walk && !split_is_short(uA) && split_is_short(uB))) swap_ab();
+                fwd_unit(a, cA, mA);
+                a++;
+            }
+            fwd_publish(pa, cA, mA);
+            fwd_publish(pb, cB, mB);
+        } else {
+#pragma unroll 1
+            for (int h = 0; h < 2; ++h) {
+                const int pj = h * NW + warp;
+                const int ua = pbound[pj], ue = pbound[pj + 1];
+                PieceFwd c;
+                c.Vq = h ? VinB : VinA;
+                c.P = 1.0;
+                c.q = 0.0;
+                c.l0 = c.l1 = c.l2 = 0.0;
+                c.dprod = 1.0;
+                c.shift = 0;
+                c.PJ = c.PJ2 = 1.0;
+                c.G0 = c.GG = c.Lc = 0.0;
+                bool any_m = false;
+                for (int un = ua; un < ue; ++un) {
+                    const int u0 = units[un];
+                    const int t0 = u0 & UNIT_T0;
+                    ck[(un * 3 + 0) * 32] = c.Vq;
+                    ck[(un * 3 + 1) * 32] = c.q;
+                    ck[(un * 3 + 2) * 32] = c.P;
+                    LDSR_UNIT_BEGIN();
+                    if (u0 & UNIT_M) {
+                        any_m = true;
+                        forward_unit_basis<PQ, UW, MSEG>(th, k, seg_bits(mw, t0, MSEG), ys + t0, us + t0 * PQ,
+                                                         vs + t0 * PQ, c);
+                    } else if (u0 & UNIT_M1) {
+                        any_m = true;
+                        forward_unit_basis<PQ, UW, 1>(th, k, seg_bits(mw, t0, 1), ys + t0, us + t0 * PQ, vs + t0 * PQ, c);
+                    } else if (u0 & UNIT_US) {
+                        forward_short_basis<PQ, MSEG>(th, k.A, k.A2, k.Q, us + t0 * PQ, c);
+                    } else {
+                        forward_word_basis<PQ, UW>(th, k, us + t0 * PQ, WK + (size_t)(t0 / UW) * PQ * 32, c);
+                    }
+                    LDSR_UNIT_END(13, u0);
+                }
+                double ld = 0.0;
+                if (any_m) ld = fma((double)c.shift, 0.693147180559945309417, log(c.dprod));
+                double *o = CH + (size_t)pj * SPLIT_NCH * 32;
+                o[0 * 32] = c.P;
+                o[1 * 32] = c.q;
+                o[2 * 32] = c.l0 + ld;
+                o[3 * 32] = c.l1;
+                o[4 * 32] = c.l2;
+                o[5 * 32] = c.PJ;
+                o[6 * 32] = c.G0;
+                o[7 * 32] = c.GG;
+                o[8 * 32] = c.Lc;
+                o[9 * 32] = c.Vq;
+            }
         }
         LDSR_PHASE_MARK(2);
         __syncthreads();
@@ -1040,49 +1276,134 @@
 
         Stats<PQ> st;
         st.zero();
-#pragma unroll 1
-        for (int h = 1; h >= 0; --h) {
-            const int pj = h * NW + warp;
-            const int ua = pbound[pj], ue = pbound[pj + 1];
-            const double xin = h ? xinB : xinA;
-            double Xs1 = h ? Xs1B : Xs1A, Vs1 = h ? Vs1B : Vs1A;
-            double Xr = h ? XrB : XrA, Vr = h ? VrB : VrA;
-            double cG = 0.0, cH = 0.0;
-            bool in_run = false;
-            for (int un = ue - 1; un >= ua; --un) {
+        if constexpr (PAIR_WALK) {
+            const auto bwd_unit = [&](SplitBwd &c) {
+                const int un = c.un;
                 const int u0 = units[un];
                 const int t0 = u0 & UNIT_T0;
                 const double Vq = ck[(un * 3 + 0) * 32];
-                const double Xq = fma(ck[(un * 3 + 2) * 32], xin, ck[(un * 3 + 1) * 32]);
+                const double Xq = fma(ck[(un * 3 + 2) * 32], c.xin, ck[(un * 3 + 1) * 32]);
                 LDSR_UNIT_BEGIN();
                 if (u0 & UNIT_M) {
-                    smooth_unit<PQ, UW, MSEG>(th, k, seg_bits(mw, t0, MSEG), false, ys + t0, us + t0 * PQ,
-                                              vs + t0 * PQ, Xq, Vq, Xs1, Vs1, st);
-                    in_run = false;
+                    smooth_unit<PQ, UW, MSEG>(th, k, seg_bits(mw, t0, MSEG), false, ys + t0, us + t0 * PQ, vs + t0 * PQ, Xq,
+                                              Vq, c.Xs1, c.Vs1, st);
+                    c.in_run = false;
                 } else if (u0 & UNIT_M1) {
-                    smooth_unit<PQ, UW, 1>(th, k, seg_bits(mw, t0, 1), t0 == T - 1, ys + t0, us + t0 * PQ,
-                                           vs + t0 * PQ, Xq, Vq, Xs1, Vs1, st);
-                    in_run = false;
+                    smooth_unit<PQ, UW, 1>(th, k, seg_bits(mw, t0, 1), t0 == T - 1, ys + t0, us + t0 * PQ, vs + t0 * PQ,
+                                           Xq, Vq, c.Xs1, c.Vs1, st);
+                    c.in_run = false;
                 } else {
-                    if (!in_run) {
-                        const double rv = fast_rcp(Vr);
-                        cG = (Xs1 - Xr) * rv;
-                        cH = (Vs1 - Vr) * rv * rv;
-                        in_run = true;
+                    c.enter_run();
+                    if (u0 & UNIT_US)
+                        smooth_short<PQ, MSEG>(th, k.A, k.A2, k.Q, us + t0 * PQ, Xq, Vq, c.cG, c.cH, c.Xs1, c.Vs1, st);
+                    else
+                        smooth_word<PQ, UW>(th, k, us + t0 * PQ, UV, WK + (size_t)(t0 / UW) * PQ * 32,
+                                            P.uwin + S.uwin_off + (size_t)(t0 / UW) * PQ * PQ, Xq, Vq, c.cG, c.cH, c.Xs1,
+                                            c.Vs1, st);
+                }
+                LDSR_UNIT_END(17, u0);
+                c.Xr = Xq;
+                c.Vr = Vq;
+                c.un = un - 1;
+            };
+            const auto bwd_init = [&](SplitBwd &c, int h) {
+                const int pj = h * NW + warp;
+                c.ua = pbound[pj];
+                c.un = pbound[pj + 1] - 1;
+                c.first = c.ua == 0 && c.un >= 0;
+                c.xin = h ? xinB : xinA;
+                c.Xs1 = h ? Xs1B : Xs1A;
+                c.Vs1 = h ? Vs1B : Vs1A;
+                c.Xr = h ? XrB : XrA;
+                c.Vr = h ? VrB : VrA;
+                c.cG = c.cH = 0.0;
+                c.in_run = false;
+            };
+            const auto bwd_done = [&](const SplitBwd &c) {
+                if (c.first) {
+                    st.X0 = c.Xs1;
+                    st.V0 = c.Vs1;
+                }
+            };
+            SplitBwd bA, bB;
+            bwd_init(bA, 1);
+            bwd_init(bB, 0);
+            for (;;) {
+                const int uA = bA.un >= bA.ua ? units[bA.un] : -1, uB = bB.un >= bB.ua ? units[bB.un] : -1;
+                if (uA < 0 && uB < 0) break;
+                if (SP.pair_walk && split_pairable(uA, uB)) {
+                    if (uA & UNIT_M) swap_vals(bA, bB);
+                    const int tw = units[bA.un] & UNIT_T0, tm = units[bB.un] & UNIT_T0;
+                    const double VqW = ck[(bA.un * 3 + 0) * 32];
+                    const double XqW = fma(ck[(bA.un * 3 + 2) * 32], bA.xin, ck[(bA.un * 3 + 1) * 32]);
+                    const double VqM = ck[(bB.un * 3 + 0) * 32];
+                    const double XqM = fma(ck[(bB.un * 3 + 2) * 32], bB.xin, ck[(bB.un * 3 + 1) * 32]);
+                    bA.enter_run();
+                    LDSR_UNIT_BEGIN();
+                    smooth_pair<PQ, UW, MSEG>(th, k, us + tw * PQ, UV, WK + (size_t)(tw / UW) * PQ * 32,
+                                              P.uwin + S.uwin_off + (size_t)(tw / UW) * PQ * PQ, XqW, VqW, bA.cG, bA.cH,
+                                              bA.Xs1, bA.Vs1, seg_bits(mw, tm, MSEG), ys + tm, us + tm * PQ,
+                                              vs + tm * PQ, XqM, VqM, bB.Xs1, bB.Vs1, st);
+                    LDSR_PAIR_END(22);
+                    bA.Xr = XqW;
+                    bA.Vr = VqW;
+                    bA.un--;
+                    bB.in_run = false;
+                    bB.Xr = XqM;
+                    bB.Vr = VqM;
+                    bB.un--;
+                    continue;
+                }
+                if (uA < 0 || (SP.pair_walk && !split_is_short(uA) && split_is_short(uB))) swap_vals(bA, bB);
+                bwd_unit(bA);
+            }
+            bwd_done(bA);
+            bwd_done(bB);
+        } else {
+#pragma unroll 1
+            for (int h = 1; h >= 0; --h) {
+                const int pj = h * NW + warp;
+                const int ua = pbound[pj], ue = pbound[pj + 1];
+                const double xin = h ? xinB : xinA;
+                double Xs1 = h ? Xs1B : Xs1A, Vs1 = h ? Vs1B : Vs1A;
+                double Xr = h ? XrB : XrA, Vr = h ? VrB : VrA;
+                double cG = 0.0, cH = 0.0;
+                bool in_run = false;
+                for (int un = ue - 1; un >= ua; --un) {
+                    const int u0 = units[un];
+                    const int t0 = u0 & UNIT_T0;
+                    const double Vq = ck[(un * 3 + 0) * 32];
+                    const double Xq = fma(ck[(un * 3 + 2) * 32], xin, ck[(un * 3 + 1) * 32]);
+                    LDSR_UNIT_BEGIN();
+                    if (u0 & UNIT_M) {
+                        smooth_unit<PQ, UW, MSEG>(th, k, seg_bits(mw, t0, MSEG), false, ys + t0, us + t0 * PQ,
+                                                  vs + t0 * PQ, Xq, Vq, Xs1, Vs1, st);
+                        in_run = false;
+                    } else if (u0 & UNIT_M1) {
+                        smooth_unit<PQ, UW, 1>(th, k, seg_bits(mw, t0, 1), t0 == T - 1, ys + t0, us + t0 * PQ,
+                                               vs + t0 * PQ, Xq, Vq, Xs1, Vs1, st);
+                        in_run = false;
+                    } else {
+                        if (!in_run) {
+                            const double rv = fast_rcp(Vr);
+                            cG = (Xs1 - Xr) * rv;
+                            cH = (Vs1 - Vr) * rv * rv;
+                            in_run = true;
+                        }
+                        if (u0 & UNIT_US)
+                            smooth_short<PQ, MSEG>(th, k.A, k.A2, k.Q, us + t0 * PQ, Xq, Vq, cG, cH, Xs1, Vs1, st);
+                        else
+                        smooth_word<PQ, UW>(th, k, us + t0 * PQ, UV, WK + (size_t)(t0 / UW) * PQ * 32,
+                                            P.uwin + S.uwin_off + (size_t)(t0 / UW) * PQ * PQ, Xq, Vq, cG, cH, Xs1, Vs1, st);
                     }
-                    if (u0 & UNIT_US)
-                        smooth_short<PQ, MSEG>(th, k.A, k.A2, k.Q, us + t0 * PQ, Xq, Vq, cG, cH, Xs1, Vs1, st);
-                    else
-                    smooth_word<PQ, UW>(th, k, us + t0 * PQ, UV, WK + (size_t)(t0 / UW) * PQ * 32,
-                                        P.uwin + S.uwin_off + (size_t)(t0 / UW) * PQ * PQ, Xq, Vq, cG, cH, Xs1, Vs1, st);
-                }
-                LDSR_UNIT_END(17, u0);
-                Xr = Xq;
-                Vr = Vq;
-            }
-            if (ua == 0 && ue > 0) {
-                st.X0 = Xs1;
-                st.V0 = Vs1;
+                    LDSR_UNIT_END(17, u0);
+                    Xr = Xq;
+                    Vr = Vq;
+                }
+                if (ua == 0 && ue > 0) {
+                    st.X0 = Xs1;
+                    st.V0 = Vs1;
+                }
             }
         }
         LDSR_PHASE_MARK(6);
@@ -1149,7 +1470,7 @@
     }
 #ifdef LDSR_PHASE_CLOCKS
     if (lane == 0 && SP.clk)
-        for (int i = 0; i < 21; i++) SP.clk[((size_t)blockIdx.x * NW + warp) * 21 + i] = pc[i];
+        for (int i = 0; i < SPLIT_NCLK; i++) SP.clk[((size_t)blockIdx.x * NW + warp) * SPLIT_NCLK + i] = pc[i];
 #endif
 
     if (ranked && !counted && threadIdx.x == 0) {
diff --git a/ldsr_b200/csrc/ldsr_abi.cu b/ldsr_b200/csrc/ldsr_abi.cu
--- a/ldsr_b200/csrc/ldsr_abi.cu
+++ b/ldsr_b200/csrc/ldsr_abi.cu
@@ -706,6 +706,7 @@
         grid0 += (P->h_series[s].fit_end - P->h_series[s].fit_begin + fits_per_cta - 1) / fits_per_cta;
     int share_slots = 0;
     bool share_ranked = false;
+    const bool no_pair = std::getenv("LDSR_NO_PAIR") != nullptr;
     if (use_split && P->kt->em_split_resident) {
         static const bool no_share = std::getenv("LDSR_NO_SHARE") != nullptr;
         int coop = 0, dev = 0;
@@ -834,6 +835,7 @@
             sp.ctl = share_ranked ? P->d_share_ctl : nullptr;
             sp.order = P->d_share_order;
             sp.n_sm = P->n_sm;
+            sp.pair_walk = no_pair ? 0 : 1;
             cudaError_t le = (grid <= 2 * P->n_sm || sp.flags) ? P->kt->em_split_wide(sp, grid, smem, st)
                                                                : P->kt->em_split(sp, grid, smem, st);
             if (le == cudaErrorCooperativeLaunchTooLarge && sp.flags) {
@@ -853,19 +855,20 @@
 #ifdef LDSR_PHASE_CLOCKS
         if (use_split && c == 1 && grid <= 4096) {
             const int nw = P->kt->split_nw;
-            std::vector<long long> h((size_t)grid * nw * 21);
+            std::vector<long long> h((size_t)grid * nw * SPLIT_NCLK);
             cudaStreamSynchronize(st);
             cudaMemcpy(h.data(), sp_clk_last, h.size() * sizeof(long long), cudaMemcpyDeviceToHost);
-            static const char *names[21] = {"P1 loops", "B1 wait", "P2", "B2 wait", "chain+stop", "B2' wait",
-                                            "P4", "B3 wait", "M-step", "constants", "prefix", "reduce",
-                                            "-", "P2 U words", "P2 M units", "P2 M1 units",
-                                            "P2 US units", "P4 U words", "P4 M units", "P4 M1 units", "P4 US units"};
+            static const char *names[SPLIT_NCLK] = {"P1 loops", "B1 wait", "P2", "B2 wait", "chain+stop", "B2' wait",
+                                                    "P4", "B3 wait", "M-step", "constants", "prefix", "reduce",
+                                                    "-", "P2 U words", "P2 M units", "P2 M1 units",
+                                                    "P2 US units", "P4 U words", "P4 M units", "P4 M1 units", "P4 US units",
+                                                    "P2 U+M pairs", "P4 U+M pairs"};
             std::fprintf(stderr, "[ldsr] phase clocks of launch 1 (cycles per iteration, mean over %d CTAs), per warp:\n", grid);
-            for (int i = 0; i < 21; i++) {
+            for (int i = 0; i < SPLIT_NCLK; i++) {
                 std::fprintf(stderr, "[ldsr]   %-14s", names[i]);
                 for (int w = 0; w < nw; w++) {
                     double sum = 0;
-                    for (int b = 0; b < grid; b++) sum += (double)h[((size_t)b * nw + w) * 21 + i];
+                    for (int b = 0; b < grid; b++) sum += (double)h[((size_t)b * nw + w) * SPLIT_NCLK + i];
                     std::fprintf(stderr, " %9.0f", sum / grid / chunk);
                 }
                 std::fprintf(stderr, "\n");
```

New measurement: 735,500 (median of 6 runs). About the same (+0.1%).
